# oxfordcontrol/Clarabel.jl

Measured on AMD Instinct MI355X. Metric: IPM iterations/sec + KKT factor+solve ms, 10k-var sparse QP, 1/2/4/8 GPU, higher is better.
Workload: dtype f64; 1 GPU; random sparse QP n=10000 m=20000 NN cone, uniform pattern (cfg 2a); N=30000, nnzK=99990, nnzL=16225495, supernodes=20125, levels=97, ordering=minimum degree, parallelism=1 independent problem(s), one per GPU

## Files before the change

### clarabel.jl_amd/csrc/device_plan.h

```cpp
#pragma once
#include <stdint.h>

#include "symbolic.h"

namespace hipkkt {

enum { SC_MAXDIAG = 0, SC_NORMB = 1, SC_NORME = 2, SC_COUNT = 8 };
enum { FL_NONFINITE = 0, FL_NREG = 1, FL_FRONTFAIL = 2, FL_FACFAIL = 3, FL_NPOLISH = 4, FL_COUNT = 8 };

struct __attribute__((aligned(16))) FrontSlot {
    double v;
    unsigned long long h;
};

struct RefineState {
    int32_t cur;
    int32_t steps;
    int32_t active;
    int32_t fail;
    double lastnorme, normb, norme;
};

struct GathPair {
    int64_t src;
    int32_t dj;
    int32_t r;
    int32_t K;
    int32_t dfirst;
};
struct DenseTriStrip {
    int c0, d, i0, pad;
    int64_t col0;
};
constexpr int kFbMax = 5;
struct FrontBatch {
    int64_t fp_off;
    int64_t scratch_off;
    int64_t stream_off;
    int32_t nb, nblk, r0;
    int32_t sync_off;
    int32_t i_base, i_end, tick, pad;
    int32_t x_begin, x_count;
};
constexpr int64_t kFbScratch = (int64_t)kFbMax * 4160 + (int64_t)(kFbMax * (kFbMax - 1) / 2) * 4096;
constexpr int kFbRec = 768;
constexpr int64_t kFbStream = (int64_t)kFbMax * 8 * kFbRec;
constexpr int kGathHeavy = 24;

constexpr int kSlvRows = 64;
constexpr int kSegSub = 8;
constexpr int kSegSubMin = 64;
constexpr int kSegRowTag = 0x40000000;
struct SegSyncLayout { int ftick, btick, fdone; int64_t err, words; };
constexpr SegSyncLayout seg_sync_layout(int nseg, int nsuper) {
    const int fdone = (2 * nseg + 31) & ~31;
    const int64_t err = fdone + (int64_t)kSegSub * nsuper;
    return {0, nseg, fdone, err, err + 16};
}
static_assert(seg_sync_layout(3, 5).btick == 3 && seg_sync_layout(3, 5).fdone == 32 && seg_sync_layout(3, 5).err == 32 + 8 * 5 &&
              seg_sync_layout(3, 5).words == 88, "seg_sync: tickets padded to 32 ints, then 8 * nsuper counters, then the error word");

struct DevPlan {
    const int *sn_first;
    const int64_t *sn_rowptr;
    const int *sn_rows;
    const int64_t *sn_panel;
    const int64_t *sn_diag;
    const int64_t *u_off;
    const int64_t *p_off;
    const int64_t *lt_off;
    const int *inv_list;
    const int *lvl_sn;
    const int *perm;
    const signed char *sgn_perm;
    const FacItem *fac_items;
    const FacRec *fac_recs;
    const FacItem *slv_items;
    const FacItem *bwd_items;
    const int *rel;
    const UpdTask *upd_tasks;
    const UpdGroup *upd_groups;
    const DenseGroup *dgroups;
    const int16_t *upd_tmap;
    const DenseTask *dtasks;
    const int64_t *gath_tgt;
    const int64_t *gath_pptr;
    const GathPair *gath_pairs;
    const int64_t *gath_heavy;
    const int64_t *g_ptr;
    const int *g_idx;
    const int64_t *kmap;
    const signed char *kdiag_sign;
    const int64_t *sym_rowptr;
    const int *sym_col;
    const int64_t *sym_q;
    const int *long_rows;
    int n_long_rows;
    const DenseTriStrip *dtri_strips;
    const int64_t *dtri_col;
    int n_dtri_strips;
    double *dense_acc;
    const FrontPanel *front_panels;
    const int64_t *front_gptr;
    const int *front_gidx;
    int *front_sync;
    const FacItem *pbwd_items;
    const int *dep_total;
    const int *sn_nitems;
    const int *sn_bparent;
    int *seg_sync;
    unsigned spin_limit;
    int *sn_polish;
    double polish_tau;
    int dbg;
    int nseg;
    double *kval;
    double *Lx;
    double *Ldiag;
    double *Linv;
    double *LinvT;
    double *LT;
    double *SbInv;
    double *D;
    double *Dinv;
    double *ubuf;
    FrontSlot *xseg, *pseg;
    int *seg_epoch;
    const int *rows_seg;
    double *pbuf;
    double *scal;
    int *flags;
};

}
```

### clarabel.jl_amd/csrc/hipkkt_internal.h

```cpp
#pragma once
#include "../../include/hipkkt.h"

#include <hip/hip_runtime.h>

#include <algorithm>
#include <atomic>
#include <chrono>
#include <cmath>
#include <cstdlib>
#include <cstring>
#include <deque>
#include <functional>
#include <future>
#include <memory>
#include <mutex>
#include <new>
#include <string>
#include <thread>
#include <vector>

#include "assemble.h"
#include "cone_layout.h"
#include "device_plan.h"
#include "hipkkt_cones.h"
#include "hipkkt_parts.h"
#include "kernels.h"
#include "runtime_pool.h"
#include "solve_schedule.h"
#include "symbolic.h"

namespace hipkkt { int box_probe(int device, double *out); }
namespace hipkkt_host {
using namespace hipkkt;

extern thread_local std::string g_create_error;

struct DeviceError {
    std::string msg;
};

#define HK_CHECK(expr)                                                                            \
    do {                                                                                          \
        hipError_t e_ = (expr);                                                                   \
        if (e_ != hipSuccess)                                                                     \
            throw DeviceError{std::string(#expr) + ": " + hipGetErrorString(e_)};                 \
    } while (0)

inline void copy_sync(hipStream_t st, void *dst, const void *src, size_t bytes, hipMemcpyKind kind) {
    if (!bytes) return;
    HK_CHECK(hipMemcpyAsync(dst, src, bytes, kind, st));
    HK_CHECK(hipStreamSynchronize(st));
}
inline void fill_async(hipStream_t st, void *dst, int value, size_t bytes) {
    if (bytes) HK_CHECK(hipMemsetAsync(dst, value, bytes, st));
}

struct DebugOpts {
    bool plan_cache = true;
    bool fb_extra = true;
    bool fb_stream = true;
    bool fb_v2 = true;
    bool force_twin = false;
    bool no_graph = false;
    bool no_persist = false;
    bool full_tiles = true;
    bool front_block = true;
    bool split_k = true;
    bool gather_overlap = true;
    bool gather_sort = true;
    int gather_side_blocks = 512;
    bool dense_tri = true;
    bool ordering_amd = false;
    bool no_front = false;
    bool host_assembly = false;
    int front_block_min_rows = -1;
    int superhop = -1;
    int debug_flags = 0;
    long long spin_limit = -1;
    long long persist_retry = -1;
    double accurate = 64.0;
    int fb_extra_pw = 1;
    double fb_pen1 = 10.0, fb_pen2 = 28.0;
    int psd_large_min = 65;
};
DebugOpts &debug_opts();
bool verbose();

struct GraphSlot {
    hipGraphExec_t exec = nullptr;
    bool valid = false;
    int static_enable = -1;
    double eps_const = 0, eps_prop = 0;
};

}

using namespace hipkkt;
using namespace hipkkt_host;

struct RefineOpts {
    int32_t enable; double reltol, abstol; int64_t max_iter; double stop_ratio;
    bool same_graph(const RefineOpts &o) const { return reltol == o.reltol && abstol == o.abstol && max_iter == o.max_iter && stop_ratio == o.stop_ratio; }
};

constexpr int kNumCtx = 2;
constexpr int kScalRedDoubles = 16;
struct SolveCtx {
    hipStream_t stream = nullptr;
    bool own_stream = false;
    DevPlan dp{};
    double *d_b = nullptr, *d_x0 = nullptr, *d_x1 = nullptr, *d_e = nullptr, *d_corr = nullptr;
    double *d_y = nullptr, *d_z = nullptr, *d_xp = nullptr;
    RefineState *d_rs = nullptr, *h_rs = nullptr;
    int *h_flags = nullptr;
    hipkkt_host::GraphSlot g_ldl, g_first, g_step;
    RefineOpts g_opts{-1, -1.0, -1.0, -1, -1.0};
    hipEvent_t ev_a = nullptr, ev_b = nullptr;
    double last_ms = 0;
    bool ir_used = false;
    bool extra_steps = false;
    const double *result() const { return (ir_used && h_rs->cur) ? d_x1 : d_x0; }
};

struct hipkkt_solver {
    int device = 0;
    SolveCtx ctx[kNumCtx];
    hipStream_t stream = nullptr;
    hipStream_t idle_stream = nullptr;
    hipkkt_opts opts{};
    bool l1 = false;
    KKTImage img;
    HostPlan plan;
    PlanOptions plan_opts;
    SolveSchedule sched;
    DevPlan dp{};
    std::vector<std::pair<void *, size_t>> allocs;
    std::string err;

    int N = 0;
    int64_t nnzK = 0;
    std::chrono::steady_clock::time_point t_created{};
    PersistState persist;
    FrontBatchState fb;
    UpdateSplit split;
    SocTables soc;
    ResidualBuffers res;
    ReducedSolve red;
    TwinState twin;
    SolverStats stats;
    ConeState cones;
    double accurate_threshold = 64.0;
    int last_npolish = 0;
    int inv_nsmall = 0, inv_wsmall = 1, inv_nwide = 0;
    int side_join_level = -1;
    hipEvent_t ev_fork = nullptr, ev_join = nullptr;

    int64_t *d_mapHs = nullptr, *d_mapP = nullptr, *d_mapA = nullptr, *d_diag_full = nullptr;
    std::vector<int64_t> cone_numel;
    std::vector<int32_t> cone_hs_dense, cone_sparse_kind;

    double *d_stage = nullptr;
    int64_t *d_stage_idx = nullptr;
    int64_t stage_cap = 0;
    double *h_scal = nullptr;
    double *h_scal_red = nullptr;
    int *h_flags = nullptr;

    hipkkt_host::GraphSlot g_factor;
    bool use_graph = true;
    bool runtime_ready = false;
    bool profiling = false;
    bool profiling_no_extra = false;
    hipEvent_t ev0 = nullptr, ev1 = nullptr, ev2 = nullptr, ev3 = nullptr;
    bool kval_event_pending = false;
    double last_eps = 0;
    int64_t last_nreg = 0;

    char *slab_cur = nullptr;
    size_t slab_left = 0;
    template <class T>
    T *dalloc(size_t n) {
        if (n == 0) n = 1;
        const size_t bytes = (n * sizeof(T) + 255) & ~(size_t)255;
        if (bytes > slab_left) {
            size_t slab = std::max<size_t>(bytes, (size_t)8 << 20);
            void *p = RuntimePool::get().dev_alloc(device, slab, &slab);
            if (!p) throw std::bad_alloc();
            allocs.push_back({p, slab});
            slab_cur = (char *)p;
            slab_left = slab;
        }
        void *p = slab_cur;
        slab_cur += bytes;
        slab_left -= bytes;
        return (T *)p;
    }
    template <class T>
    T *upload(const std::vector<T> &v) {
        T *p = dalloc<T>(v.size());
        if (!v.empty()) hipkkt_host::copy_sync(stream, p, v.data(), v.size() * sizeof(T), hipMemcpyHostToDevice);
        return p;
    }
    void ensure_stage(int64_t n) {
        if (n <= stage_cap) return;
        int64_t cap = std::max<int64_t>(n, 2 * stage_cap);
        d_stage = dalloc<double>(cap);
        d_stage_idx = dalloc<int64_t>(cap);
        stage_cap = cap;
    }
    template <class F>
    void for_each_graph_slot(F &&f) {
        f(g_factor); for (SolveCtx &C : ctx) { f(C.g_ldl); f(C.g_first); f(C.g_step); }
    }
    ~hipkkt_solver() {
        if (twin.cancel) twin.cancel->store(true);
        if (twin.go && twin.go->load() == 0) twin.go->store(2);
        if (twin.future.valid()) twin.future.wait();
        twin.pending.reset();
        delete twin.fallback;
        (void)hipSetDevice(device);
        RuntimePool &rp = RuntimePool::get();
        if (stream) (void)hipStreamSynchronize(stream);
        for (SolveCtx &C : ctx)
            if (C.own_stream && C.stream) (void)hipStreamSynchronize(C.stream);
        for_each_graph_slot([](hipkkt_host::GraphSlot &g) { if (g.exec) (void)hipGraphExecDestroy(g.exec); });
        for (SolveCtx &C : ctx) {
            rp.pinned_free(device, C.h_rs);
            rp.pinned_free(device, C.h_flags);
            for (hipEvent_t e : {C.ev_a, C.ev_b}) rp.event_put(device, e);
            if (C.own_stream) rp.stream_put(device, 2, C.stream);
        }
        for (auto &a : allocs) rp.dev_free(device, a.first, a.second);
        rp.pinned_free(device, h_scal);
        rp.pinned_free(device, h_flags);
        for (hipEvent_t e : {ev0, ev1, ev2, ev3, ev_fork, ev_join}) rp.event_put(device, e);
        rp.stream_put(device, 0, stream);
        rp.stream_put(device, 1, idle_stream);
    }
};

namespace hipkkt_host {

struct SyncWords { size_t seg, front; };
inline SyncWords sync_words(const hipkkt_solver *S) {
    return {(size_t)seg_sync_layout(S->sched.nseg, S->plan.nsuper).words, (size_t)std::max(S->plan.front_sync_ints, 16)};
}

void plan_cache_counts(int64_t *hits, int64_t *misses);
void init_runtime(hipkkt_solver *S);
void setup_device(hipkkt_solver *S);
int32_t finish_create(hipkkt_solver *S, const hipkkt_opts *opts, hipkkt_handle *out);
int32_t solve_many(hipkkt_solver *S, hipkkt_solver *T, int nrhs, const RefineOpts &ir, int64_t *ir_steps, double *const *out_dev, int nm,
                   const std::function<void(hipStream_t)> *after = nullptr);
hipkkt_solver *solve_target(hipkkt_solver *S);
struct ReducedIn {
    const double *rhs_x, *workz, *var_x, *in_dev;
    static ReducedIn host(const double *rhs_x, const double *workz, const double *var_x) { return {rhs_x, workz, var_x, nullptr}; }
    static ReducedIn device(const double *in_dev) { return {nullptr, nullptr, nullptr, in_dev}; }
};
struct ReducedScalars { const double *scal_in4; int32_t const_pending; };
struct ReducedOut {
    double *lhs_x = nullptr, *lhs_z = nullptr, *lhs_dev = nullptr, *scal_out = nullptr;
    int64_t *ir_steps = nullptr;
    const std::function<void(hipStream_t, const double *)> *after_reduce = nullptr;
};
int32_t kkt_solve_reduced_impl(hipkkt_solver *S, const ReducedIn &in, const ReducedScalars &sc, const ReducedOut &out, const RefineOpts &ir);

template <class F>
void run_graphed(hipkkt_solver *S, hipStream_t stream, GraphSlot &slot, bool reusable, F &&enqueue) {
    if (!S->use_graph) { enqueue(); return; }
    if (!(slot.valid && reusable)) {
        if (slot.exec) { (void)hipGraphExecDestroy(slot.exec); slot.exec = nullptr; slot.valid = false; }
        hipGraph_t graph = nullptr;
        HK_CHECK(hipStreamBeginCapture(stream, hipStreamCaptureModeRelaxed));
        try {
            enqueue();
        } catch (...) {
            (void)hipStreamEndCapture(stream, &graph);
            if (graph) (void)hipGraphDestroy(graph);
            throw;
        }
        HK_CHECK(hipStreamEndCapture(stream, &graph));
        hipError_t e = hipGraphInstantiate(&slot.exec, graph, nullptr, nullptr, 0);
        (void)hipGraphDestroy(graph);
        if (e != hipSuccess) { slot.exec = nullptr; S->use_graph = false; enqueue(); return; }
        slot.valid = true;
    }
    HK_CHECK(hipGraphLaunch(slot.exec, stream));
}

}

#define HK_ENTER(h)                                                      \
    if (!(h)) return HIPKKT_ERR_ARGUMENT;                                \
    hipkkt_solver *S = (h);                                              \
    try {                                                                \
        if (hipSetDevice(S->device) != hipSuccess) { S->err = "hipSetDevice failed"; return HIPKKT_ERR_DEVICE; }

#define HK_LEAVE                                                         \
    }                                                                    \
    catch (const DeviceError &e) { S->err = e.msg; return HIPKKT_ERR_DEVICE; } \
    catch (const std::bad_alloc &) { S->err = "out of memory"; return HIPKKT_ERR_ALLOC; } \
    catch (...) { S->err = "internal error"; return HIPKKT_ERR_INTERNAL; }
```

### clarabel.jl_amd/csrc/hipkkt_setup.cpp

```cpp
#include "hipkkt_internal.h"

using namespace hipkkt;
using namespace hipkkt_host;

namespace hipkkt_host {

namespace {
struct PlanCache {
    struct Entry {
        uint64_t key;
        std::string optkey;
        std::vector<int64_t> colptr, rowval;
        std::shared_ptr<const HostPlan> plan;
    };
    std::mutex mu;
    std::deque<Entry> entries;
    int64_t hits = 0, misses = 0;
    static constexpr size_t kMaxEntries = 8;
    static constexpr int64_t kMaxNnzL = 40000000;
    static PlanCache &get() { static PlanCache c; return c; }
    static bool enabled() { return debug_opts().plan_cache; }
    static uint64_t fnv(uint64_t h, const void *p, size_t n) {
        const unsigned char *b = (const unsigned char *)p;
        for (size_t i = 0; i < n; i++) { h ^= b[i]; h *= 1099511628211ull; }
        return h;
    }
    std::shared_ptr<const HostPlan> find(uint64_t key, const std::string &optkey, const KKTImage &K) {
        std::lock_guard<std::mutex> lk(mu);
        for (const Entry &e : entries)
            if (e.key == key && e.optkey == optkey && e.colptr == K.colptr && e.rowval == K.rowval) { hits++; return e.plan; }
        misses++;
        return nullptr;
    }
    void put(uint64_t key, const std::string &optkey, const KKTImage &K, const HostPlan &P) {
        if (P.nnzL > kMaxNnzL || P.ordering_used == 1) return;
        Entry e{key, optkey, K.colptr, K.rowval, std::make_shared<const HostPlan>(P)};
        std::lock_guard<std::mutex> lk(mu);
        entries.push_front(std::move(e));
        while (entries.size() > kMaxEntries) entries.pop_back();
    }
};
}
void plan_cache_counts(int64_t *hits, int64_t *misses) {
    PlanCache &c = PlanCache::get();
    std::lock_guard<std::mutex> lk(c.mu);
    *hits = c.hits; *misses = c.misses;
}

void init_runtime(hipkkt_solver *S) {
    HK_CHECK(hipSetDevice(S->device));
    RuntimePool &rp = RuntimePool::get();
    auto need = [&](void *p) { if (!p) throw DeviceError{"creating a stream / event / pinned buffer failed"}; return p; };
    S->stream = (hipStream_t)need(rp.stream_get(S->device, 0));
    S->idle_stream = (hipStream_t)need(rp.stream_get(S->device, 1));
    {
        const DebugOpts &o = debug_opts();
        S->fb.sw.extra = o.fb_extra;
        S->fb.sw.streamed = o.fb_stream;
        S->fb.sw.v2 = o.fb_v2 && S->fb.sw.streamed;
#ifndef HIPKKT_TESTING
        S->fb.sw.streamed = S->fb.sw.v2 = true;
#endif
        S->accurate_threshold = o.accurate;
        S->twin.force = o.force_twin;
    }
    static_assert(SC_COUNT * sizeof(double) <= RuntimePool::kPinned && sizeof(RefineState) <= RuntimePool::kPinned, "pinned chunk too small");
    for (hipEvent_t *e : {&S->ev0, &S->ev1, &S->ev2, &S->ev3, &S->ev_fork, &S->ev_join}) *e = (hipEvent_t)need(rp.event_get(S->device));
    S->h_scal = (double *)need(rp.pinned_alloc(S->device));
    S->h_flags = (int *)need(rp.pinned_alloc(S->device));
    S->h_scal_red = S->h_scal + 16;
    static_assert((16 + kScalRedDoubles) * sizeof(double) <= RuntimePool::kPinned, "pinned chunk too small for the reduced-solve scalars");
    memset(S->h_scal, 0, SC_COUNT * sizeof(double));
    memset(S->h_flags, 0, FL_COUNT * sizeof(int));
    if (debug_opts().no_graph) S->use_graph = false;
    for (int c = 0; c < kNumCtx; c++) {
        SolveCtx &C = S->ctx[c];
        if (c == 0) C.stream = S->stream;
        else { C.stream = (hipStream_t)need(rp.stream_get(S->device, 2)); C.own_stream = true; }
        C.ev_a = (hipEvent_t)need(rp.event_get(S->device));
        C.ev_b = (hipEvent_t)need(rp.event_get(S->device));
        C.h_rs = (RefineState *)need(rp.pinned_alloc(S->device));
        C.h_flags = (int *)need(rp.pinned_alloc(S->device));
        memset(C.h_rs, 0, sizeof(RefineState));
        memset(C.h_flags, 0, FL_COUNT * sizeof(int));
    }
}

template <class T>
static T *zeroed(hipkkt_solver *S, size_t n) {
    T *p = S->dalloc<T>(n);
    fill_async(S->stream, p, 0, std::max<size_t>(n, 1) * sizeof(T));
    return p;
}

static void order_far_stages(hipkkt_solver *S) {
    HostPlan &Pm = S->plan;
    const HostPlan &P = S->plan;
    const auto hb = front_batches(P, S->plan_opts.update_policy, kFbMax);
    const size_t nbh = hb.size();
    S->fb.next.assign(nbh, NextBatch());
    if (!S->fb.sw.extra || !debug_opts().front_block) return;
    std::vector<std::vector<int>> panel_batch(P.fronts.size());
    for (size_t fi = 0; fi < P.fronts.size(); fi++) panel_batch[fi].assign((size_t)P.fronts[fi].np, -1);
    for (size_t q = 0; q < nbh; q++)
        for (int t = 0; t < hb[q].nb; t++) panel_batch[(size_t)hb[q].front][(size_t)(hb[q].p0 + t)] = (int)q;
    for (size_t b = 0; b < nbh; b++) {
        const bool next = b + 1 < nbh && hb[b + 1].front == hb[b].front && hb[b + 1].p0 == hb[b].p0 + hb[b].nb;
        NextBatch &A = S->fb.next[b];
        const int l = hb[b].level_last, g0 = P.upd_stage_ptr[l], nd = P.upd_stage_ndense[l];
        const FrontDesc &F = P.fronts[(size_t)hb[b].front];
        auto near = [&](const UpdGroup &G) {
            if (!next || P.sn_front[G.tgt] != hb[b].front) return false;
            return panel_batch[(size_t)hb[b].front][(size_t)(G.tgt - F.s0)] == (int)b + 1;
        };
        auto gb = Pm.upd_groups.begin() + g0, ge = gb + nd;
        A.ncrit = (int)(std::stable_partition(gb, ge, near) - gb);
        A.has_next = next;
        A.next_blk = next ? (P.front_panels[P.fronts[(size_t)hb[b + 1].front].fp_off + hb[b + 1].p0].r + 63) / 64 : 0;
    }
}

constexpr int64_t kGatherSplitMin = 1000000;
constexpr int64_t kGatherSortMin = 50000;
static void split_gather_stages(hipkkt_solver *S) {
    HostPlan &P = S->plan;
    S->split.gath.assign(std::max(P.nlevels, 1), -1);
    const int B = P.update_batch_used;
    const bool may_split = S->plan_opts.update_policy == 2 && B >= 2 && debug_opts().gather_overlap;
    for (int l = 0; l < P.nlevels; l++) {
        const int64_t e0 = P.gath_stage_ptr[l], e1 = P.gath_stage_ptr[l + 1], ne = e1 - e0;
        if (ne < kGatherSortMin || !debug_opts().gather_sort) continue;
        std::vector<char> far((size_t)ne, 0);
        int64_t nfar = 0;
        if (may_split && ne >= kGatherSplitMin && l % B == B - 1 && l + B < P.nlevels) {
            for (int64_t e = e0; e < e1; e++) {
                const int t = (int)(std::upper_bound(P.sn_panel.begin(), P.sn_panel.begin() + P.nsuper, P.gath_tgt[e]) - P.sn_panel.begin()) - 1;
                far[(size_t)(e - e0)] = P.sn_level[t] > l + B;
                nfar += far[(size_t)(e - e0)];
            }
            if (nfar < kGatherSplitMin) { std::fill(far.begin(), far.end(), 0); nfar = 0; }
        }
        const size_t nkeys = (size_t)2 * (size_t)P.nsuper;
        std::vector<int64_t> cnt(nkeys + 1, 0);
        auto key = [&](int64_t e) { return (size_t)far[(size_t)(e - e0)] * (size_t)P.nsuper + (size_t)P.gath_sn[P.gath_pptr[e]]; };
        for (int64_t e = e0; e < e1; e++) cnt[key(e) + 1]++;
        for (size_t k = 0; k < nkeys; k++) cnt[k + 1] += cnt[k];
        std::vector<int64_t> ord((size_t)ne);
        for (int64_t e = e0; e < e1; e++) ord[(size_t)cnt[key(e)]++] = e;
        const int64_t p0 = P.gath_pptr[e0], p1 = P.gath_pptr[e1];
        std::vector<int64_t> tgt((size_t)ne), pptr((size_t)ne), src((size_t)(p1 - p0));
        std::vector<int32_t> dj((size_t)(p1 - p0)), sn((size_t)(p1 - p0));
        int64_t w = 0;
        for (int64_t q = 0; q < ne; q++) {
            const int64_t e = ord[(size_t)q];
            tgt[(size_t)q] = P.gath_tgt[e];
            for (int64_t pq = P.gath_pptr[e]; pq < P.gath_pptr[e + 1]; pq++, w++) { src[(size_t)w] = P.gath_src[pq]; dj[(size_t)w] = P.gath_dj[pq]; sn[(size_t)w] = P.gath_sn[pq]; }
            pptr[(size_t)q] = p0 + w;
        }
        std::copy(tgt.begin(), tgt.end(), P.gath_tgt.begin() + e0);
        std::copy(pptr.begin(), pptr.end(), P.gath_pptr.begin() + e0 + 1);
        std::copy(src.begin(), src.end(), P.gath_src.begin() + p0);
        std::copy(dj.begin(), dj.end(), P.gath_dj.begin() + p0);
        std::copy(sn.begin(), sn.end(), P.gath_sn.begin() + p0);
        if (nfar > 0) S->split.gath[l] = ne - nfar;
        if (verbose()) fprintf(stderr, "hipkkt: gather stage %d: %lld entries sorted by source, %lld of them deferred to the side stream (targets beyond level %d)\n", l, (long long)ne, (long long)nfar, l + B);
    }
}

static int64_t plan_split_k(hipkkt_solver *S, std::vector<DenseGroup> &dg) {
    const HostPlan &P = S->plan;
    S->split.group_begin.assign(std::max(P.nlevels, 1), 0);
    S->split.group_count.assign(std::max(P.nlevels, 1), 0);
    S->split.rec_ptr.assign(P.nlevels + 1, 0);
    std::vector<SplitRec> recs;
    int64_t scratch_max = 0;
    if (!debug_opts().split_k) { S->split.d_recs = S->upload(recs); return 0; }
    for (int l = 0; l < P.nlevels; l++) {
        S->split.rec_ptr[l + 1] = S->split.rec_ptr[l];
        const int g0 = P.upd_stage_ptr[l], nd = P.upd_stage_ndense[l];
        if (nd == 0 || S->fb.lvl[l] != -1) continue;
        int64_t ntasks = 0;
        for (int g = g0; g < g0 + nd; g++) ntasks += dg[g].task_end - dg[g].task_begin;
        const int chunk = std::max(4, (int)((ntasks + nd - 1) / nd));
        int max_nt = 0;
        for (int g = g0; g < g0 + nd; g++) max_nt = std::max(max_nt, dg[g].task_end - dg[g].task_begin);
        if (nd <= kDenseStripTiles || max_nt < 2 * chunk + 6) continue;
        int64_t scratch = 0;
        S->split.group_begin[l] = (int)dg.size();
        for (int g = g0; g < g0 + nd; g++) {
            const int nt = dg[g].task_end - dg[g].task_begin;
            const int parts = std::min(16, nt / chunk);
            if (nt < 2 * chunk || parts < 2) continue;
            recs.push_back({dg[g].tile_off, P.panel_doubles + scratch, dg[g].rt, dg[g].nrt, dg[g].wt, parts});
            for (int q = 0; q < parts; q++) {
                const int tb = dg[g].task_begin + (int)((int64_t)nt * q / parts), te = dg[g].task_begin + (int)((int64_t)nt * (q + 1) / parts);
                dg.push_back({P.panel_doubles + scratch, 64, dg[g].nrt, dg[g].wt, tb, te, dg[g].pad});
                scratch += 4096;
            }
            dg[g].wt = 0;
        }
        S->split.group_count[l] = (int)dg.size() - S->split.group_begin[l];
        S->split.rec_ptr[l + 1] = (int)recs.size();
        scratch_max = std::max(scratch_max, scratch);
    }
    S->split.d_recs = S->upload(recs);
    if (verbose() && !recs.empty())
        fprintf(stderr, "hipkkt: split-K: %zu target tiles cut into %zu chunks, %.1f MB of partial tiles\n", recs.size(), dg.size() - P.upd_groups.size(), scratch_max * 8e-6);
    return scratch_max;
}

static void build_front_batches(hipkkt_solver *S) {
    const HostPlan &P = S->plan;
    S->fb.lvl.assign(std::max(P.nlevels, 1), -1);
    if (!debug_opts().front_block) S->fb.sw.use = false;
    if (S->fb.sw.use)
        for (const FrontBatchHost &H : front_batches(P, S->plan_opts.update_policy, kFbMax)) {
            const FrontDesc &F = P.fronts[H.front];
            FrontBatch B;
            B.fp_off = F.fp_off + H.p0;
            B.nb = H.nb;
            B.r0 = P.front_panels[F.fp_off + H.p0].r;
            B.nblk = (B.r0 + 63) / 64;
            B.i_base = 0; B.i_end = B.nblk; B.tick = 0; B.pad = 0; B.x_begin = 0; B.x_count = 0;
            B.sync_off = 128 * (int)S->fb.batches.size();
            B.scratch_off = kFbScratch * (int64_t)S->fb.batches.size();
            B.stream_off = kFbStream * (int64_t)S->fb.batches.size();
            S->fb.lvl[H.level_first] = (int)S->fb.batches.size();
            for (int l = H.level_first + 1; l <= H.level_last; l++) S->fb.lvl[l] = -2;
            S->fb.batches.push_back(B);
            S->fb.last_level.push_back(H.level_last);
        }
    if (verbose()) fprintf(stderr, "hipkkt: %zu front batch(es) factored by one launch each (fronts %zu, update batch %d)\n", S->fb.batches.size(), P.fronts.size(), P.update_batch_used);
    const size_t nb_ = std::max<size_t>(S->fb.batches.size(), 1);
    S->fb.d_sync = zeroed<int>(S, 128 * nb_);
    S->fb.d_scratch = S->dalloc<double>((size_t)kFbScratch * nb_);
    S->fb.stream_doubles = (S->fb.sw.streamed || S->fb.sw.v2) ? (int64_t)kFbStream * (int64_t)nb_ : 0;
    S->fb.d_stream = S->dalloc<double>((size_t)std::max<int64_t>(S->fb.stream_doubles, 1));
    if (getenv("HIPKKT_FB_TRACE")) S->fb.d_trace = (long long *)zeroed<double>(S, nb_ * 128);
}

static void reset_device_state(hipkkt_solver *S) {
    S->for_each_graph_slot([](GraphSlot &g) { if (g.exec) (void)hipGraphExecDestroy(g.exec); g = GraphSlot(); });
    if (!S->allocs.empty() && S->stream) (void)hipStreamSynchronize(S->stream);
    for (auto &a : S->allocs) RuntimePool::get().dev_free(S->device, a.first, a.second);
    S->allocs.clear();
    S->slab_cur = nullptr; S->slab_left = 0;
    S->stage_cap = 0; S->d_stage = nullptr; S->d_stage_idx = nullptr;
    S->persist.rearm(!debug_opts().no_persist);
    S->fb.reset();
    S->split = UpdateSplit();
    S->soc = SocTables();
    S->res = ResidualBuffers();
    S->red = ReducedSolve();
    S->cones = ConeState();
}

static std::vector<int> inversion_list(hipkkt_solver *S) {
    const HostPlan &P = S->plan;
    std::vector<int> small, wide;
    S->inv_wsmall = 1;
    for (int s = 0; s < P.nsuper; s++) {
        const int w = P.sn_first[s + 1] - P.sn_first[s];
        if (w > 16 && w <= 64) wide.push_back(s);
        else { small.push_back(s); S->inv_wsmall = std::max(S->inv_wsmall, w); }
    }
    S->inv_nsmall = (int)small.size();
    S->inv_nwide = (int)wide.size();
    small.insert(small.end(), wide.begin(), wide.end());
    return small;
}

static std::vector<FacRec> fac_records(const HostPlan &P) {
    std::vector<FacRec> recs(P.fac_items.size());
    for (size_t q = 0; q < recs.size(); q++) {
        const int s = P.fac_items[q].sn;
        recs[q] = {P.sn_panel[s], P.sn_diag[s], P.lt_off[s], P.sn_first[s], P.sn_first[s + 1] - P.sn_first[s],
                   (int32_t)(P.sn_rowptr[s + 1] - P.sn_rowptr[s]), P.fac_items[q].blk};
    }
    return recs;
}

static std::vector<DenseGroup> dense_groups(const HostPlan &P) {
    std::vector<DenseGroup> dg(P.upd_groups.size());
    const bool no_full_tiles = !debug_opts().full_tiles;
    for (size_t q = 0; q < dg.size(); q++) {
        const UpdGroup &G = P.upd_groups[q];
        const int t = G.tgt;
        const int rt = (int)(P.sn_rowptr[t + 1] - P.sn_rowptr[t]);
        bool full = G.dense == 1 && rt - G.row_base >= kUpdRows && P.sn_first[t + 1] - P.sn_first[t] == 64 && !no_full_tiles;
        for (int u = G.task_begin; u < G.task_end && full; u++) {
            const UpdTask &T = P.upd_tasks[u];
            const int K = P.sn_first[T.src + 1] - P.sn_first[T.src];
            full = !(T.geom & (1 << 17)) && (T.geom & 0xFFFF) == 0 && T.nrows >= 64 && T.ncols >= 64 && K >= 8 && (K & 7) == 0;
        }
        dg[q] = {P.sn_panel[t] + G.row_base, rt, std::min(kUpdRows, rt - G.row_base), P.sn_first[t + 1] - P.sn_first[t],
                 G.task_begin, G.task_end, full ? 1 : 0};
    }
    return dg;
}

static std::vector<DenseTask> dense_tasks(const HostPlan &P) {
    std::vector<DenseTask> dt(P.upd_tasks.size());
    for (size_t q = 0; q < dt.size(); q++) {
        const UpdTask &T = P.upd_tasks[q];
        const int s = T.src;
        dt[q] = {P.sn_panel[s], (int32_t)((P.sn_rowptr[s + 1] - P.sn_rowptr[s]) * 8), P.sn_first[s + 1] - P.sn_first[s],
                 P.sn_first[s], T.row_lo, T.nrows, T.col_lo, T.ncols, T.geom, T.vt_begin, 0};
    }
    return dt;
}

static std::vector<GathPair> gather_pairs(const HostPlan &P) {
    std::vector<GathPair> gp(P.gath_src.size());
    for (size_t q = 0; q < gp.size(); q++) {
        const int s = P.gath_sn[q];
        gp[q] = {P.gath_src[q], P.gath_dj[q], (int32_t)(P.sn_rowptr[s + 1] - P.sn_rowptr[s]), P.sn_first[s + 1] - P.sn_first[s], P.sn_first[s]};
    }
    return gp;
}

static std::vector<int64_t> heavy_gathers(hipkkt_solver *S) {
    const HostPlan &P = S->plan;
    std::vector<int64_t> heavy;
    S->split.heavy_ptr.assign(P.nlevels + 1, 0);
    S->split.gath_heavy.assign(std::max(P.nlevels, 1), 0);
    for (int l = 0; l < P.nlevels; l++) {
        const int64_t e_split = S->split.gath[l] >= 0 ? P.gath_stage_ptr[l] + S->split.gath[l] : P.gath_stage_ptr[l + 1];
        for (int64_t e = P.gath_stage_ptr[l]; e < P.gath_stage_ptr[l + 1]; e++)
            if (P.gath_pptr[e + 1] - P.gath_pptr[e] > kGathHeavy) {
                heavy.push_back(e);
                if (e < e_split) S->split.gath_heavy[l]++;
            }
        S->split.heavy_ptr[l + 1] = (int64_t)heavy.size();
    }
    return heavy;
}

static void upload_plan(hipkkt_solver *S) {
    const HostPlan &P = S->plan;
    const SolveSchedule &H = S->sched;
    const int N = P.N;
    std::vector<signed char> sgn_perm(N), kdiag(S->nnzK, 0);
    for (int k = 0; k < N; k++) sgn_perm[k] = (signed char)(S->img.dsigns[P.perm[k]] >= 0 ? 1 : -1);
    for (int j = 0; j < N; j++)
        for (int64_t q = S->img.colptr[j]; q < S->img.colptr[j + 1]; q++)
            if (S->img.rowval[q] == j) kdiag[q] = (signed char)(S->img.dsigns[j] >= 0 ? 1 : -1);
    DevPlan &D = S->dp;
    D.sn_first = S->upload(P.sn_first);
    D.sn_rowptr = S->upload(P.sn_rowptr);
    D.sn_rows = S->upload(P.sn_rows);
    D.sn_panel = S->upload(P.sn_panel);
    D.sn_diag = S->upload(P.sn_diag);
    D.u_off = S->upload(P.u_off);
    D.p_off = S->upload(H.p_off);
    D.lt_off = S->upload(P.lt_off);
    D.bwd_items = S->upload(H.bwd_items);
    D.lvl_sn = S->upload(H.lvl_sn);
    D.perm = S->upload(P.perm);
    D.sgn_perm = S->upload(sgn_perm);
    D.inv_list = S->upload(inversion_list(S));
    D.fac_items = S->upload(P.fac_items);
    D.fac_recs = S->upload(fac_records(P));
    D.slv_items = S->upload(H.slv_items);
    D.rel = S->upload(P.rel);
    D.upd_tasks = S->upload(P.upd_tasks);
    D.upd_groups = S->upload(P.upd_groups);
    D.upd_tmap = P.upd_tmap.size() >= 128 ? S->upload(P.upd_tmap) : S->upload(std::vector<int16_t>(128, (int16_t)-1));
    D.dtasks = S->upload(dense_tasks(P));
    D.gath_tgt = S->upload(P.gath_tgt);
    D.gath_pptr = S->upload(P.gath_pptr);
    D.gath_pairs = S->upload(gather_pairs(P));
    D.gath_heavy = S->upload(heavy_gathers(S));
    D.g_ptr = S->upload(P.g_ptr);
    D.g_idx = S->upload(P.g_idx);
    D.kmap = S->upload(P.kmap);
    D.kdiag_sign = S->upload(kdiag);
    D.sym_rowptr = S->upload(P.sym_rowptr);
    D.sym_col = S->upload(P.sym_col);
    D.sym_q = S->upload(P.sym_q);
    std::vector<int> lr;
    const int thr = long_row_threshold();
    for (int i = 0; i < N; i++)
        if (P.sym_rowptr[i + 1] - P.sym_rowptr[i] > thr) lr.push_back(i);
    D.long_rows = S->upload(lr);
    D.n_long_rows = (int)lr.size();
    std::vector<DenseTriStrip> strips;
    for (const DenseTri &T : P.dtri)
        for (int i0 = 0; i0 < T.d; i0 += 64) strips.push_back(DenseTriStrip{T.c0, T.d, i0, 0, T.col0});
    D.dtri_strips = S->upload(strips);
    D.n_dtri_strips = (int)strips.size();
    D.dtri_col = S->upload(P.dtri_col);
    D.dense_acc = nullptr;
    D.front_panels = S->upload(P.front_panels);
    D.front_gptr = S->upload(P.front_gptr);
    D.front_gidx = S->upload(P.front_gidx);
    D.pbwd_items = S->upload(H.pbwd_items);
    D.dep_total = S->upload(H.dep_total);
    D.sn_nitems = S->upload(H.sn_nitems);
    D.sn_bparent = S->upload(H.sn_bparent);
    D.nseg = H.nseg;
    D.spin_limit = debug_opts().spin_limit >= 0 ? (unsigned)debug_opts().spin_limit : (1u << 20);
#ifdef HIPKKT_TESTING
    D.dbg = debug_opts().debug_flags;
    if (D.dbg) fprintf(stderr, "hipkkt: DEBUG_FLAGS = %d: timing experiment, the results of this handle are WRONG\n", D.dbg);
#else
    D.dbg = 0;
#endif
    D.sn_polish = zeroed<int>(S, (size_t)P.nsuper);
    D.polish_tau = S->accurate_threshold;
}

static void alloc_solve_scratch(hipkkt_solver *S, DevPlan &D) {
    const HostPlan &P = S->plan;
    const int64_t np0 = S->sched.p_off[P.nsuper];
    const size_t nx = (size_t)std::max(P.N, 1), np_ = (size_t)std::max<int64_t>(np0, 1);
    const SyncWords nw = sync_words(S);
    D.ubuf = S->dalloc<double>(P.ubuf_len);
    D.pbuf = S->dalloc<double>(np0);
    D.xseg = (FrontSlot *)zeroed<double>(S, 2 * nx);
    D.pseg = (FrontSlot *)zeroed<double>(S, 2 * np_);
    D.seg_epoch = zeroed<int>(S, 4);
    D.seg_sync = zeroed<int>(S, nw.seg);
    D.front_sync = zeroed<int>(S, nw.front);
    D.scal = zeroed<double>(S, SC_COUNT);
    D.flags = zeroed<int>(S, FL_COUNT);
}

static void alloc_factor_storage(hipkkt_solver *S) {
    const HostPlan &P = S->plan;
    DevPlan &D = S->dp;
    const int N = P.N;
    std::vector<DenseGroup> dg = dense_groups(P);
    build_front_batches(S);
    const int64_t split_scratch = S->split.scratch_doubles = plan_split_k(S, dg);
    D.dgroups = S->upload(dg);
    D.kval = S->upload(S->img.nzval);
    D.Lx = S->dalloc<double>(P.panel_doubles + split_scratch);
    if (split_scratch) fill_async(S->stream, D.Lx + P.panel_doubles, 0, (size_t)split_scratch * sizeof(double));
    D.Ldiag = zeroed<double>(S, (size_t)P.diag_doubles);
    D.Linv = S->dalloc<double>(P.diag_doubles);
    D.LinvT = S->dalloc<double>(P.diag_doubles);
    D.LT = S->dalloc<double>(P.lt_off[P.nsuper]);
    D.SbInv = zeroed<double>(S, (size_t)P.sbinv_doubles);
    D.D = S->dalloc<double>(N);
    D.Dinv = zeroed<double>(S, (size_t)N);
}

static void upload_value_maps(hipkkt_solver *S) {
    S->d_diag_full = S->upload(S->img.diag_full);
    if (!S->l1) return;
    SocTables &T = S->soc;
    S->d_mapHs = S->upload(S->img.mapHs);
    S->d_mapP = S->upload(S->img.mapP);
    S->d_mapA = S->upload(S->img.mapA);
    std::vector<int64_t> uidx, vidx, didx;
    std::vector<int> coneof;
    T.of_sparse.assign(S->img.smaps.size(), -1);
    for (size_t i = 0; i < S->img.smaps.size(); i++) {
        const SparseMap &sm = S->img.smaps[i];
        if (sm.kind != 1) continue;
        T.of_sparse[i] = T.n;
        T.off.push_back((int64_t)uidx.size());
        for (size_t q = 0; q < sm.vec[0].size(); q++) {
            uidx.push_back(sm.vec[0][q]);
            vidx.push_back(sm.vec[1][q]);
            coneof.push_back(T.n);
        }
        didx.push_back(sm.D[0]);
        didx.push_back(sm.D[1]);
        T.n++;
    }
    T.off.push_back((int64_t)uidx.size());
    T.total = (int64_t)uidx.size();
    T.d_uidx = S->upload(uidx);
    T.d_vidx = S->upload(vidx);
    T.d_didx = S->upload(didx);
    T.d_cone = S->upload(coneof);
    T.d_u = S->dalloc<double>(T.total);
    T.d_v = S->dalloc<double>(T.total);
    T.d_eta2 = S->dalloc<double>(T.n);
}

static void alloc_contexts(hipkkt_solver *S) {
    const int N = S->N;
    for (int c = 0; c < kNumCtx; c++) {
        SolveCtx &C = S->ctx[c];
        for (double **v : {&C.d_b, &C.d_x0, &C.d_x1, &C.d_e, &C.d_corr, &C.d_y, &C.d_z, &C.d_xp}) *v = zeroed<double>(S, (size_t)N);
        C.d_rs = (RefineState *)zeroed<double>(S, sizeof(RefineState) / sizeof(double) + 1);
        C.dp = S->dp;
        if (S->dp.n_dtri_strips > 0) C.dp.dense_acc = zeroed<double>(S, (size_t)N);
        if (c > 0) alloc_solve_scratch(S, C.dp);
        C.ir_used = false;
        C.h_rs->cur = 0;
    }
}

void setup_device(hipkkt_solver *S) {
    HK_CHECK(hipSetDevice(S->device));
    reset_device_state(S);
    order_far_stages(S);
    split_gather_stages(S);
    S->N = S->plan.N; S->nnzK = S->plan.nnzK;
    S->sched = build_solve_schedule(S->plan);
    upload_plan(S);
    alloc_factor_storage(S);
    S->dp.rows_seg = S->upload(S->sched.rows_seg);
    alloc_solve_scratch(S, S->dp);
    upload_value_maps(S);
    alloc_contexts(S);
    S->ensure_stage(std::max<int64_t>(1024, std::max<int64_t>(S->img.nHs, S->N)));
    HK_CHECK(hipStreamSynchronize(S->stream));
}

int32_t finish_create(hipkkt_solver *S, const hipkkt_opts *opts, hipkkt_handle *out) {
    PlanOptions po;
    po.max_width = opts->supernode_max_width > 0 ? opts->supernode_max_width : kMaxSnWidth;
    po.relax = opts->relax_supernodes != 0;
    po.update_policy = opts->update_policy;
    if (opts->update_batch > 0) po.update_batch = opts->update_batch;
    po.amd_dense_scale = opts->amd_dense_scale > 0 ? opts->amd_dense_scale : 1.5;
    po.front_min_panels = opts->front_min_panels == 0 ? 4 : std::max(0, opts->front_min_panels);
    po.n_hold = S->l1 ? (int)S->img.n : 0;
    po.dense_tri_first_col = (S->l1 && debug_opts().dense_tri) ? (int)S->img.n : -1;
    if (debug_opts().front_block_min_rows >= 0) po.front_block_min_width = debug_opts().front_block_min_rows;
    if (debug_opts().superhop >= 0) po.superhop = debug_opts().superhop;
    if (debug_opts().ordering_amd) po.n_hold = 0;
    if (debug_opts().no_front) po.front_min_panels = 0;
    std::vector<int64_t> up;
    const int64_t *uperm = nullptr;
    if (opts->user_perm) {
        up.resize(S->img.N);
        for (int64_t k = 0; k < S->img.N; k++) up[k] = opts->user_perm[k] - opts->index_base;
        uperm = up.data();
    }
    if (S->img.N >= ((int64_t)1 << 31)) { g_create_error = "N exceeds int32"; delete S; return HIPKKT_ERR_ARGUMENT; }
    {
        if (S->l1)
            po.on_alternative_order = [S, &po](const std::vector<int> &perm_md) {
                std::unique_ptr<hipkkt_solver> T(new hipkkt_solver());
                T->device = S->device;
                T->opts = S->opts;
                T->l1 = S->l1;
                T->img = S->img;
                PlanOptions po2 = po;
                po2.n_hold = 0;
                po2.on_alternative_order = nullptr;
                S->twin.cancel = std::make_shared<std::atomic<bool>>(false);
                po2.cancel = S->twin.cancel.get();
                T->plan_opts = po2;
                hipkkt_solver *Tp = T.get();
                std::vector<int64_t> pv(perm_md.begin(), perm_md.end());
                S->twin.pending = std::move(T);
                S->twin.go = std::make_shared<std::atomic<int>>(0);
                std::shared_ptr<std::atomic<int>> go = S->twin.go;
                S->twin.future = std::async(std::launch::async, [Tp, pv, po2, go]() {
                    std::string err = build_plan((int)Tp->img.N, Tp->img.colptr.data(), Tp->img.rowval.data(), pv.data(), po2, Tp->plan);
                    if (!err.empty()) return err;
                    if (Tp->plan.nnzL < 20000000) return err;
                    while (go->load(std::memory_order_acquire) == 0) std::this_thread::sleep_for(std::chrono::microseconds(200));
                    if (go->load(std::memory_order_acquire) != 1 || (po2.cancel && po2.cancel->load(std::memory_order_relaxed))) return std::string("cancelled");
                    try {
                        init_runtime(Tp);
                        setup_device(Tp);
                        Tp->twin.device_ready = true;
                    } catch (const DeviceError &e) {
                        return std::string("twin device set-up: ") + e.msg;
                    } catch (const std::bad_alloc &) {
                        return std::string("twin device set-up: out of memory");
                    }
                    return err;
                });
            };
    }
    const auto t_a = std::chrono::steady_clock::now();
    uint64_t ckey = 0;
    std::string optkey;
    std::shared_ptr<const HostPlan> cached;
    const bool plan_cache_on = PlanCache::enabled();
    if (plan_cache_on) {
        char buf[256];
        snprintf(buf, sizeof buf, "%d|%d|%d|%d|%.17g|%.17g|%d|%d|%d|%d|%d|%d|%d|%d|%d", po.max_width, (int)po.relax, po.update_policy, po.update_batch,
                 po.amd_dense_scale, po.dense_min_cover, po.n_hold, po.front_block_min_width, po.front_min_panels, po.superhop, po.nd_mode,
                 po.nd_leaf, uperm ? 1 : 0, po.dense_tri_first_col, po.dense_tri_min_dim);
        optkey = buf;
        ckey = PlanCache::fnv(1469598103934665603ull, S->img.colptr.data(), S->img.colptr.size() * sizeof(int64_t));
        ckey = PlanCache::fnv(ckey, S->img.rowval.data(), S->img.rowval.size() * sizeof(int64_t));
        if (uperm) ckey = PlanCache::fnv(ckey, uperm, (size_t)S->img.N * sizeof(int64_t));
        cached = PlanCache::get().find(ckey, optkey, S->img);
    }
    std::string err;
    if (cached) {
        S->plan = *cached;
        S->plan.timing_note = "plan cache hit";
    } else {
        err = build_plan((int)S->img.N, S->img.colptr.data(), S->img.rowval.data(), uperm, po, S->plan);
        if (err.empty() && plan_cache_on) PlanCache::get().put(ckey, optkey, S->img, S->plan);
    }
    po.on_alternative_order = nullptr;
    if (!err.empty()) { g_create_error = err; delete S; return HIPKKT_ERR_ARGUMENT; }
    if (S->plan.ordering_used != 1 && S->twin.cancel) S->twin.cancel->store(true);
    if (S->twin.go) S->twin.go->store((S->plan.ordering_used == 1 && err.empty()) ? 1 : 2, std::memory_order_release);
    S->plan_opts = po;
    const auto t_b = std::chrono::steady_clock::now();
    try {
        if (!S->runtime_ready) init_runtime(S);
        S->runtime_ready = true;
        setup_device(S);
        if (verbose())
            fprintf(stderr, "hipkkt: N %d nnzL %lld levels %d ordering %d: symbolic %.2f ms (%s), device set-up %.2f ms, runtime objects %.2f ms\n", S->plan.N, (long long)S->plan.nnzL,
                    S->plan.nlevels, S->plan.ordering_used, 1e3 * std::chrono::duration<double>(t_b - t_a).count(), S->plan.timing_note.c_str(),
                    1e3 * std::chrono::duration<double>(std::chrono::steady_clock::now() - t_b).count(), 1e3 * S->stats.t_init_runtime);
    } catch (const DeviceError &e) {
        g_create_error = e.msg; delete S; return HIPKKT_ERR_DEVICE;
    } catch (const std::bad_alloc &) {
        g_create_error = "out of (device) memory"; delete S; return HIPKKT_ERR_ALLOC;
    }
    *out = S;
    return HIPKKT_OK;
}

}
```

### clarabel.jl_amd/csrc/hipkkt_solve.cpp

```cpp
#include "hipkkt_internal.h"

using namespace hipkkt;
using namespace hipkkt_host;

namespace hipkkt_host {

static void enqueue_ldl_solve(hipkkt_solver *S, SolveCtx &C, const double *in, double *out, int *zero = nullptr, int nzero = 0) {
    const HostPlan &P = S->plan;
    const SolveSchedule &H = S->sched;
    hipStream_t st = C.stream;
    const DevPlan &D = C.dp;
    launch_permute_in(st, in, D.perm, C.d_y, S->N, D.seg_epoch, D.seg_sync, 2 * H.nseg, zero, nzero);
    const LevelLists &L = S->persist.use ? H.regular : H.all;
    auto fwd_level = [&](int l) {
        launch_fwd_narrow(st, D, L.reg_ptr[l], L.nnarrow[l], L.wnarrow[l], C.d_y, C.d_z);
        launch_fwd_level(st, D, L.slv_ptr[l], L.slv_ptr[l + 1] - L.slv_ptr[l], C.d_y, C.d_z);
    };
    auto bwd_level = [&](int l) {
        launch_bwd_partial(st, D, L.bwd_ptr[l], L.bwd_ptr[l + 1] - L.bwd_ptr[l], C.d_xp);
        launch_bwd_final(st, D, L.reg_ptr[l] + L.nnarrow[l], L.reg_ptr[l + 1] - L.reg_ptr[l] - L.nnarrow[l], C.d_z, C.d_xp, out);
        launch_bwd_narrow(st, D, L.reg_ptr[l], L.nnarrow[l], L.wnarrow[l], C.d_z, C.d_xp, out);
    };
    if (S->persist.use) {
        for (int g = 0; g < H.nseg; g++) {
            for (int l = H.seg_lo[g]; l < std::min(H.seg_lstar[g], H.seg_hi[g] + 1); l++) fwd_level(l);
            launch_fwd_seg(st, D, g, H.fseg_ptr[2 * g], H.fseg_ptr[2 * g + 1] - H.fseg_ptr[2 * g], P.nsuper, C.d_y, C.d_z);
            for (const FrontDesc &F : P.fronts)
                if (H.seg_of_level[F.level_last] == g) launch_front_fwd(st, D, F, C.d_y, C.d_z);
        }
        bool first = true;
        for (int g = H.nseg - 1; g >= 0; g--) {
            for (const FrontDesc &F : P.fronts)
                if (H.seg_of_level[F.level_last] == g) launch_front_bwd(st, D, F, C.d_z, C.d_xp, out);
            const int k = H.nseg - 1 - g;
            const int n = H.bseg_ptr[k + 1] - H.bseg_ptr[k];
            if (n > 0) { launch_bwd_seg(st, D, g, H.bseg_ptr[k], n, P.nsuper, first ? 1 : 0, C.d_z, C.d_xp, out); first = false; }
            for (int l = std::min(H.seg_lstar[g], H.seg_hi[g] + 1) - 1; l >= H.seg_lo[g]; l--) bwd_level(l);
        }
        return;
    }
    for (int l = 0; l < P.nlevels; l++) fwd_level(l);
    for (int l = P.nlevels - 1; l >= 0; l--) bwd_level(l);
}

static void invalidate_solve_graphs(SolveCtx &C) { C.g_ldl.valid = C.g_first.valid = C.g_step.valid = false; }

static void maybe_retry_persistent(hipkkt_solver *S) {
    PersistState &ps = S->persist;
    if (!ps.use && ps.allowed && ps.retry_at >= 0 && S->stats.n_ldlsolves >= ps.retry_at) {
        ps.use = true;
        ps.retry_at = -1;
        for (SolveCtx &C : S->ctx) invalidate_solve_graphs(C);
    }
}

static void enqueue_refine_step(hipkkt_solver *S, SolveCtx &C, const RefineOpts &ir) {
    hipStream_t st = C.stream;
    enqueue_ldl_solve(S, C, C.d_e, C.d_corr, (int *)(C.dp.scal + SC_NORME), 2);
    launch_refine_add(st, C.d_rs, C.d_x0, C.d_x1, C.d_corr, S->N);
    launch_spmv_residual(st, C.dp, C.d_b, C.d_rs, C.d_x0, C.d_x1, C.d_e, S->N, (unsigned long long *)C.dp.scal + SC_NORME);
    launch_refine_decide(st, C.d_rs, C.dp.scal, 1, ir.reltol, ir.abstol, (int)std::min<int64_t>(ir.max_iter, 1 << 30), ir.stop_ratio);
}

static inline bool sweep_failed(const SolveCtx &C) {
    if (C.h_flags[FL_FRONTFAIL] & ~7) {
        static bool told = false;
        if (!told)
            fprintf(stderr, "hipkkt: unexpected value in the flag words: %x %x %x %x\n", C.h_flags[0], C.h_flags[1], C.h_flags[2], C.h_flags[3]);
        told = true;
    }
    return (C.h_flags[FL_FRONTFAIL] & 7) != 0;
}

static bool recover_from_sweep_failure(hipkkt_solver *S) {
    PersistState &ps = S->persist;
    if (!ps.use) return false;
    for (SolveCtx &C : S->ctx) HK_CHECK(hipStreamSynchronize(C.stream));
    S->stats.n_sweep_timeouts++;
    const int64_t first = debug_opts().persist_retry >= 0 ? debug_opts().persist_retry : 64;
    ps.backoff = ps.backoff > 0 ? 2 * ps.backoff : first;
    ps.retry_at = first > 0 ? S->stats.n_ldlsolves + ps.backoff : -1;
    fprintf(stderr, "hipkkt: a persistent sweep kernel timed out (flags 0x%x 0x%x); per-level solve kernels for the next %lld LDL solves\n",
            S->ctx[0].h_flags[FL_FRONTFAIL], S->ctx[1].h_flags[FL_FRONTFAIL], (long long)(ps.retry_at >= 0 ? ps.backoff : -1));
    const SyncWords nw = sync_words(S);
    for (SolveCtx &C : S->ctx) {
        fill_async(S->stream, C.dp.seg_sync, 0, nw.seg * sizeof(int));
        fill_async(S->stream, C.dp.front_sync, 0, nw.front * sizeof(int));
        fill_async(S->stream, C.dp.flags + FL_FRONTFAIL, 0, sizeof(int));
        C.h_flags[FL_FRONTFAIL] = 0;
        invalidate_solve_graphs(C);
    }
    HK_CHECK(hipStreamSynchronize(S->stream));
    ps.use = false;
    return true;
}

template <class Body>
static bool with_sweep_retry(hipkkt_solver *T, Body &&body) {
    for (int attempt = 0; attempt < 2; attempt++) {
        maybe_retry_persistent(T);
        if (!body()) return false;
        if (!recover_from_sweep_failure(T)) return true;
    }
    return true;
}

static int32_t merge_rc(int32_t rc, int32_t r) { return (r < 0 || (r > 0 && rc == HIPKKT_OK)) ? (r < 0 ? r : (rc < 0 ? rc : r)) : rc; }

static void account_solve(hipkkt_solver *S, hipkkt_solver *T, double ms, int64_t nrhs) {
    for (hipkkt_solver *h : {T, S != T ? S : nullptr})
        if (h) { h->stats.t_last_solve = ms; h->stats.t_acc_solve += ms; h->stats.n_solvecalls++; h->stats.n_rhs_solved += nrhs; }
}

static void upload_rhs(SolveCtx &C, const double *rhsx, const double *rhsz, int64_t n, int64_t m, int64_t p) {
    if (n) HK_CHECK(hipMemcpyAsync(C.d_b, rhsx, n * sizeof(double), hipMemcpyHostToDevice, C.stream));
    if (m) HK_CHECK(hipMemcpyAsync(C.d_b + n, rhsz, m * sizeof(double), hipMemcpyHostToDevice, C.stream));
    if (p) HK_CHECK(hipMemsetAsync(C.d_b + n + m, 0, p * sizeof(double), C.stream));
}

static void solve_begin(hipkkt_solver *S, SolveCtx &C, const RefineOpts &ir) {
    hipStream_t st = C.stream;
    if (S->kval_event_pending && st != S->stream) HK_CHECK(hipStreamWaitEvent(st, S->ev3, 0));
    HK_CHECK(hipEventRecord(C.ev_a, st));
    C.ir_used = ir.enable != 0;
    if (ir.enable) {
        const bool same = C.g_opts.same_graph(ir);
        run_graphed(S, st, C.g_first, same, [&] {
            enqueue_ldl_solve(S, C, C.d_b, C.d_x0, (int *)(C.dp.scal + SC_NORMB), 4);
            launch_norm_inf(st, C.d_b, S->N, (unsigned long long *)C.dp.scal + SC_NORMB);
            launch_spmv_residual(st, C.dp, C.d_b, nullptr, C.d_x0, C.d_x0, C.d_e, S->N, (unsigned long long *)C.dp.scal + SC_NORME);
            launch_refine_decide(st, C.d_rs, C.dp.scal, 0, ir.reltol, ir.abstol, (int)std::min<int64_t>(ir.max_iter, 1 << 30), ir.stop_ratio);
            if (ir.max_iter > 0) enqueue_refine_step(S, C, ir);
        });
        if (!same) { C.g_step.valid = false; C.g_opts = ir; }
        S->stats.n_ldlsolves += ir.max_iter > 0 ? 2 : 1;
    } else {
        run_graphed(S, st, C.g_ldl, true, [&] {
            enqueue_ldl_solve(S, C, C.d_b, C.d_x0);
            launch_zero_words(st, C.dp.flags, 1);
            launch_check_finite(st, C.d_x0, S->N, C.dp.flags);
        });
        S->stats.n_ldlsolves += 1;
    }
}

static void solve_copy_out_dev(hipkkt_solver *S, SolveCtx &C, double *out_dev, int nm) {
    if (!out_dev) return;
    if (C.ir_used) launch_refine_copy_out(C.stream, C.d_rs, C.d_x0, C.d_x1, out_dev, nm);
    else HK_CHECK(hipMemcpyAsync(out_dev, C.d_x0, (size_t)nm * sizeof(double), hipMemcpyDeviceToDevice, C.stream));
}

static int32_t solve_finish(hipkkt_solver *S, SolveCtx &C, int64_t *ir_steps, double *out_dev, int nm) {
    hipStream_t st = C.stream;
    auto readback = [&] {
        if (C.ir_used) HK_CHECK(hipMemcpyAsync(C.h_rs, C.d_rs, sizeof(RefineState), hipMemcpyDeviceToHost, st));
        HK_CHECK(hipMemcpyAsync(C.h_flags, C.dp.flags, FL_COUNT * sizeof(int), hipMemcpyDeviceToHost, st));
        HK_CHECK(hipEventRecord(C.ev_b, st));
        HK_CHECK(hipStreamSynchronize(st));
    };
    readback();
    bool more = false;
    C.extra_steps = false;
    while (C.ir_used && C.h_rs->active && !sweep_failed(C)) {
        run_graphed(S, st, C.g_step, true, [&] { enqueue_refine_step(S, C, C.g_opts); });
        S->stats.n_ldlsolves += 1;
        more = true;
        readback();
    }
    C.extra_steps = more;
    if (more && out_dev) {
        solve_copy_out_dev(S, C, out_dev, nm);
        HK_CHECK(hipEventRecord(C.ev_b, st));
        HK_CHECK(hipStreamSynchronize(st));
    }
    float ms = 0;
    HK_CHECK(hipEventElapsedTime(&ms, C.ev_a, C.ev_b));
    C.last_ms = ms;
    if (ir_steps) *ir_steps = C.ir_used ? C.h_rs->steps : 0;
    if (sweep_failed(C)) { S->err = "persistent solve kernel timed out"; return HIPKKT_ERR_DEVICE; }
    const bool ok = C.ir_used ? C.h_rs->fail == 0 : C.h_flags[FL_NONFINITE] == 0;
    return ok ? HIPKKT_OK : HIPKKT_NUMERICAL_FAILURE;
}

hipkkt_solver *solve_target(hipkkt_solver *S) { return (S->twin.using_fallback && S->twin.fallback) ? S->twin.fallback : S; }

int32_t solve_many(hipkkt_solver *S, hipkkt_solver *T, int nrhs, const RefineOpts &ir, int64_t *ir_steps, double *const *out_dev, int nm,
                   const std::function<void(hipStream_t)> *after) {
    int32_t rc = HIPKKT_OK;
    double ms = 0;
    bool redo = false;
    auto run_after = [&] {
        for (int c = 1; c < nrhs; c++) {
            HK_CHECK(hipEventRecord(S->ev2, T->ctx[c].stream));
            HK_CHECK(hipStreamWaitEvent(T->ctx[0].stream, S->ev2, 0));
        }
        (*after)(T->ctx[0].stream);
    };
    const bool gave_up = with_sweep_retry(T, [&] {
        for (int c = 0; c < nrhs; c++) {
            solve_begin(T, T->ctx[c], ir);
            solve_copy_out_dev(T, T->ctx[c], out_dev ? out_dev[c] : nullptr, nm);
        }
        if (after) run_after();
        rc = HIPKKT_OK;
        ms = 0;
        redo = false;
        bool timed_out = false;
        for (int c = 0; c < nrhs; c++) {
            rc = merge_rc(rc, solve_finish(T, T->ctx[c], ir_steps ? ir_steps + c : nullptr, out_dev ? out_dev[c] : nullptr, nm));
            ms = std::max(ms, T->ctx[c].last_ms);
            timed_out = timed_out || sweep_failed(T->ctx[c]);
            redo = redo || T->ctx[c].extra_steps;
        }
        return timed_out;
    });
    if (after && !gave_up && rc == HIPKKT_OK) {
        if (redo) run_after();
        HK_CHECK(hipStreamSynchronize(T->ctx[0].stream));
    }
    account_solve(S, T, ms, nrhs);
    return rc;
}

int32_t kkt_solve_reduced_impl(hipkkt_solver *S, const ReducedIn &in, const ReducedScalars &sc, const ReducedOut &out, const RefineOpts &ir) {
    const int64_t n = S->img.n, m = S->img.m, p = S->img.p;
    const int nm = (int)(n + m);
    const int32_t const_pending = sc.const_pending;
    if (!S->red.d) {
        S->red.d = S->dalloc<double>(3 * (size_t)S->N + n + 16);
        S->red.d_part = S->dalloc<double>(8 * (size_t)residual_blocks((int)n, (int)m) + 8);
        S->red.have_const = false;
    }
    double *d_s1 = S->red.d, *d_s2 = d_s1 + S->N, *d_lhs = d_s2 + S->N, *d_xv = d_lhs + S->N, *d_sc = d_xv + n;
    if (!const_pending && !S->red.have_const) { S->err = "kkt_solve_reduced: no constant-rhs solution resident (pass const_pending = 1 after a refactorisation)"; return HIPKKT_ERR_ARGUMENT; }
    hipkkt_solver *T = solve_target(S);
    const double tau = sc.scal_in4[0], kappa = sc.scal_in4[1], rhs_tau = sc.scal_in4[2], rhs_kappa = sc.scal_in4[3];
    SolveCtx &A = T->ctx[0], &Bc = T->ctx[1];
    auto reduce = [&]() {
        launch_reduced(A.stream, S->dp, d_s1, d_s2, d_xv, S->res.d_qb, S->res.d_qb + n, tau, kappa, rhs_tau, rhs_kappa, S->red.d_part, d_sc,
                       d_lhs, (int)n, (int)m);
        if (out.lhs_dev) HK_CHECK(hipMemcpyAsync(out.lhs_dev, d_lhs, (size_t)nm * sizeof(double), hipMemcpyDeviceToDevice, A.stream));
        if (out.lhs_x && n) HK_CHECK(hipMemcpyAsync(out.lhs_x, d_lhs, n * sizeof(double), hipMemcpyDeviceToHost, A.stream));
        if (out.lhs_z && m) HK_CHECK(hipMemcpyAsync(out.lhs_z, d_lhs + n, m * sizeof(double), hipMemcpyDeviceToHost, A.stream));
        HK_CHECK(hipMemcpyAsync(S->h_scal_red, d_sc, 10 * sizeof(double), hipMemcpyDeviceToHost, A.stream));
        if (out.after_reduce) (*out.after_reduce)(A.stream, d_lhs);
    };
    auto join_const = [&]() { HK_CHECK(hipEventRecord(S->ev2, Bc.stream)); HK_CHECK(hipStreamWaitEvent(A.stream, S->ev2, 0)); };
    int64_t st1 = 0, st2 = 0;
    int32_t rc = HIPKKT_OK;
    bool redo = false;
    double ms = 0;
    const bool gave_up = with_sweep_retry(T, [&] {
        if (in.in_dev) {
            launch_set_rhs(A.stream, A.d_b, in.in_dev, nm, T->N);
            HK_CHECK(hipMemcpyAsync(d_xv, in.in_dev + nm, (size_t)n * sizeof(double), hipMemcpyDeviceToDevice, A.stream));
        } else {
            upload_rhs(A, in.rhs_x, in.workz, n, m, p);
            if (n) HK_CHECK(hipMemcpyAsync(d_xv, in.var_x, n * sizeof(double), hipMemcpyHostToDevice, A.stream));
        }
        solve_begin(T, A, ir);
        solve_copy_out_dev(T, A, d_s1, nm);
        if (const_pending) {
            launch_const_rhs(Bc.stream, Bc.d_b, S->res.d_qb, (int)n, nm, T->N);
            solve_begin(T, Bc, ir);
            solve_copy_out_dev(T, Bc, d_s2, nm);
            join_const();
        }
        reduce();
        st1 = st2 = 0;
        rc = solve_finish(T, A, &st1, d_s1, nm);
        redo = A.extra_steps;
        ms = A.last_ms;
        if (const_pending) {
            rc = merge_rc(rc, solve_finish(T, Bc, &st2, d_s2, nm));
            redo = redo || Bc.extra_steps;
            ms = std::max(ms, Bc.last_ms);
        }
        return sweep_failed(A) || (const_pending && sweep_failed(Bc));
    });
    if (gave_up) return HIPKKT_ERR_DEVICE;
    if (redo && rc == HIPKKT_OK) {
        if (const_pending) join_const();
        reduce();
    }
    HK_CHECK(hipStreamSynchronize(A.stream));
    account_solve(S, T, ms, const_pending ? 2 : 1);
    if (rc == HIPKKT_OK && const_pending) S->red.have_const = true;
    if (out.ir_steps) { out.ir_steps[0] = st1; out.ir_steps[1] = st2; }
    if (out.scal_out) memcpy(out.scal_out, S->h_scal_red, 10 * sizeof(double));
    return rc;
}

}

extern "C" {


int32_t hipkkt_setrhs(hipkkt_handle h, const double *rhsx, const double *rhsz) {
    HK_ENTER(h)
    const int64_t n = S->img.n, m = S->img.m;
    if (!S->l1 || (n && !rhsx) || (m && !rhsz)) return HIPKKT_ERR_ARGUMENT;
    upload_rhs(S->ctx[0], rhsx, rhsz, n, m, S->img.p);
    HK_CHECK(hipStreamSynchronize(S->stream));
    return HIPKKT_OK;
    HK_LEAVE
}

int32_t hipkkt_setrhs_dev(hipkkt_handle h, const double *rhs_dev) {
    HK_ENTER(h)
    if (!S->l1 || !rhs_dev) return HIPKKT_ERR_ARGUMENT;
    launch_set_rhs(S->stream, S->ctx[0].d_b, rhs_dev, (int)(S->img.n + S->img.m), S->N);
    return HIPKKT_OK;
    HK_LEAVE
}

static hipkkt_solver *target_with_rhs(hipkkt_solver *S) {
    hipkkt_solver *T = solve_target(S);
    if (T != S) copy_sync(S->stream, T->ctx[0].d_b, S->ctx[0].d_b, (size_t)S->N * sizeof(double), hipMemcpyDeviceToDevice);
    return T;
}

int32_t hipkkt_solve(hipkkt_handle h, double *lhsx, double *lhsz, int32_t ir_enable, double reltol, double abstol,
                     int64_t max_iter, double stop_ratio, int64_t *ir_steps) {
    HK_ENTER(h)
    if (!S->l1) return HIPKKT_ERR_ARGUMENT;
    hipkkt_solver *T = target_with_rhs(S);
    int32_t rc = solve_many(S, T, 1, RefineOpts{ir_enable, reltol, abstol, max_iter, stop_ratio}, ir_steps, nullptr, 0);
    if (rc == HIPKKT_OK) {
        const int64_t n = S->img.n, m = S->img.m;
        const double *x = T->ctx[0].result();
        if (lhsx && n) copy_sync(S->stream, lhsx, x, n * sizeof(double), hipMemcpyDeviceToHost);
        if (lhsz && m) copy_sync(S->stream, lhsz, x + n, m * sizeof(double), hipMemcpyDeviceToHost);
    }
    return rc;
    HK_LEAVE
}

int32_t hipkkt_solve_dev(hipkkt_handle h, double *lhs_dev, int32_t ir_enable, double reltol, double abstol,
                         int64_t max_iter, double stop_ratio, int64_t *ir_steps) {
    HK_ENTER(h)
    if (!S->l1) return HIPKKT_ERR_ARGUMENT;
    hipkkt_solver *T = target_with_rhs(S);
    double *outs[1] = {lhs_dev};
    return solve_many(S, T, 1, RefineOpts{ir_enable, reltol, abstol, max_iter, stop_ratio}, ir_steps, outs, (int)(S->img.n + S->img.m));
    HK_LEAVE
}

static int32_t solve_multi_impl(hipkkt_solver *S, int64_t nrhs, const double *rhsx, const double *rhsz, const double *rhs_dev,
                                double *lhsx, double *lhsz, double *lhs_dev, const RefineOpts &ir, int64_t *ir_steps) {
    const int64_t n = S->img.n, m = S->img.m, p = S->img.p;
    hipkkt_solver *T = solve_target(S);
    int32_t rc_all = HIPKKT_OK;
    for (int64_t r0 = 0; r0 < nrhs; r0 += kNumCtx) {
        const int k = (int)std::min<int64_t>(kNumCtx, nrhs - r0);
        double *outs[kNumCtx] = {nullptr, nullptr};
        for (int c = 0; c < k; c++) {
            SolveCtx &C = T->ctx[c];
            const int64_t r = r0 + c;
            if (rhs_dev) launch_set_rhs(C.stream, C.d_b, rhs_dev + r * (n + m), (int)(n + m), T->N);
            else upload_rhs(C, rhsx + r * n, rhsz + r * m, n, m, p);
            if (lhs_dev) outs[c] = lhs_dev + r * (n + m);
        }
        const int32_t rc = solve_many(S, T, k, ir, ir_steps ? ir_steps + r0 : nullptr, lhs_dev ? outs : nullptr, (int)(n + m));
        if (rc < 0) return rc;
        if (rc > 0) rc_all = rc;
        if (rc == HIPKKT_OK && (lhsx || lhsz))
            for (int c = 0; c < k; c++) {
                const double *x = T->ctx[c].result();
                const int64_t r = r0 + c;
                if (lhsx && n) copy_sync(S->stream, lhsx + r * n, x, n * sizeof(double), hipMemcpyDeviceToHost);
                if (lhsz && m) copy_sync(S->stream, lhsz + r * m, x + n, m * sizeof(double), hipMemcpyDeviceToHost);
            }
    }
    return rc_all;
}

int32_t hipkkt_solve_multi(hipkkt_handle h, int64_t nrhs, const double *rhsx, const double *rhsz, double *lhsx, double *lhsz,
                           int32_t ir_enable, double reltol, double abstol, int64_t max_iter, double stop_ratio, int64_t *ir_steps) {
    HK_ENTER(h)
    if (!S->l1 || nrhs < 0 || (nrhs && ((S->img.n && !rhsx) || (S->img.m && !rhsz)))) return HIPKKT_ERR_ARGUMENT;
    return solve_multi_impl(S, nrhs, rhsx, rhsz, nullptr, lhsx, lhsz, nullptr, RefineOpts{ir_enable, reltol, abstol, max_iter, stop_ratio}, ir_steps);
    HK_LEAVE
}

int32_t hipkkt_solve_multi_dev(hipkkt_handle h, int64_t nrhs, const double *rhs_dev, double *lhs_dev, int32_t ir_enable, double reltol,
                               double abstol, int64_t max_iter, double stop_ratio, int64_t *ir_steps) {
    HK_ENTER(h)
    if (!S->l1 || nrhs < 0 || (nrhs && !rhs_dev)) return HIPKKT_ERR_ARGUMENT;
    return solve_multi_impl(S, nrhs, nullptr, nullptr, rhs_dev, nullptr, nullptr, lhs_dev, RefineOpts{ir_enable, reltol, abstol, max_iter, stop_ratio}, ir_steps);
    HK_LEAVE
}

int32_t hipkkt_kkt_solve_reduced(hipkkt_handle h, const double *rhs_x, const double *workz, const double *var_x, const double *scal_in4,
                                 int32_t const_pending, double *lhs_x, double *lhs_z, double *scal_out10, int32_t ir_enable,
                                 double reltol, double abstol, int64_t max_iter, double stop_ratio, int64_t *ir_steps2) {
    HK_ENTER(h)
    const int64_t n = S->img.n, m = S->img.m;
    if (!S->l1 || !S->res.d_qb || !scal_in4 || !scal_out10 || (n && (!rhs_x || !var_x)) || (m && !workz)) {
        S->err = "kkt_solve_reduced: call hipkkt_set_qb first / bad arguments";
        return HIPKKT_ERR_ARGUMENT;
    }
    ReducedOut out;
    out.lhs_x = lhs_x; out.lhs_z = lhs_z; out.scal_out = scal_out10; out.ir_steps = ir_steps2;
    return kkt_solve_reduced_impl(S, ReducedIn::host(rhs_x, workz, var_x), {scal_in4, const_pending}, out, RefineOpts{ir_enable, reltol, abstol, max_iter, stop_ratio});
    HK_LEAVE
}

int32_t hipkkt_kkt_solve_reduced_dev(hipkkt_handle h, const double *in_dev, const double *scal_in4, int32_t const_pending,
                                     double *lhs_dev, double *scal_out10, int32_t ir_enable, double reltol, double abstol,
                                     int64_t max_iter, double stop_ratio, int64_t *ir_steps2) {
    HK_ENTER(h)
    if (!S->l1 || !S->res.d_qb || !scal_in4 || !scal_out10 || !in_dev) {
        S->err = "kkt_solve_reduced_dev: call hipkkt_set_qb first / bad arguments";
        return HIPKKT_ERR_ARGUMENT;
    }
    ReducedOut out;
    out.lhs_dev = lhs_dev; out.scal_out = scal_out10; out.ir_steps = ir_steps2;
    return kkt_solve_reduced_impl(S, ReducedIn::device(in_dev), {scal_in4, const_pending}, out, RefineOpts{ir_enable, reltol, abstol, max_iter, stop_ratio});
    HK_LEAVE
}

int32_t hipkkt_ldl_solve(hipkkt_handle h, double *x, const double *b) {
    if (h && h->twin.using_fallback && h->twin.fallback) return hipkkt_ldl_solve(h->twin.fallback, x, b);
    HK_ENTER(h)
    if (!x || !b) return HIPKKT_ERR_ARGUMENT;
    SolveCtx &C = S->ctx[0];
    HK_CHECK(hipMemcpyAsync(C.d_b, b, (size_t)S->N * sizeof(double), hipMemcpyHostToDevice, C.stream));
    int32_t rc = solve_many(S, S, 1, RefineOpts{0, 0.0, 0.0, 0, 0.0}, nullptr, nullptr, 0);
    if (rc < 0) return rc;
    copy_sync(S->stream, x, C.d_x0, (size_t)S->N * sizeof(double), hipMemcpyDeviceToHost);
    return HIPKKT_OK;
    HK_LEAVE
}

}
```

### clarabel.jl_amd/csrc/kernel_util.h

```cpp
#pragma once
#include <hip/hip_runtime.h>
#include <stdint.h>

namespace hipkkt {

static inline unsigned nblk(int64_t n, int bs = 256) { return (unsigned)((n + bs - 1) / bs); }

typedef double v4f64 __attribute__((ext_vector_type(4)));

__device__ __forceinline__ double readlane_f64(double x, int l) {
    const unsigned long long u = (unsigned long long)__double_as_longlong(x);
    const unsigned lo = __builtin_amdgcn_readlane((unsigned)u, l), hi = __builtin_amdgcn_readlane((unsigned)(u >> 32), l);
    return __longlong_as_double((long long)(((unsigned long long)hi << 32) | lo));
}
__device__ __forceinline__ int rfl(int v) { return __builtin_amdgcn_readfirstlane(v); }

template <class T>
__device__ __forceinline__ T *rfl_ptr(T *p) {
    const unsigned long long u = (unsigned long long)p;
    const unsigned lo = __builtin_amdgcn_readfirstlane((unsigned)u), hi = __builtin_amdgcn_readfirstlane((unsigned)(u >> 32));
    return (T *)(((unsigned long long)hi << 32) | lo);
}
#define HK_GLOBAL __attribute__((address_space(1)))
__device__ __forceinline__ double ld_off(const double *base, unsigned byte_off) {
    return *(const HK_GLOBAL double *)((const HK_GLOBAL char *)base + byte_off);
}
__device__ __forceinline__ void st_off(double *base, unsigned byte_off, double v) {
    *(HK_GLOBAL double *)((HK_GLOBAL char *)base + byte_off) = v;
}

__device__ __forceinline__ int ld_relaxed_i(const int *p) { return __hip_atomic_load(p, __ATOMIC_RELAXED, __HIP_MEMORY_SCOPE_AGENT); }
__device__ __forceinline__ double ld_relaxed(const double *p) { return __hip_atomic_load(p, __ATOMIC_RELAXED, __HIP_MEMORY_SCOPE_AGENT); }
__device__ __forceinline__ void st_relaxed(double *p, double v) { __hip_atomic_store(p, v, __ATOMIC_RELAXED, __HIP_MEMORY_SCOPE_AGENT); }

__device__ __forceinline__ double pivot_rcp(double d) {
    double r = __builtin_amdgcn_rcp(d);
    r = fma(fma(-d, r, 1.0), r, r);
    r = fma(fma(-d, r, 1.0), r, r);
    return r;
}

__device__ __forceinline__ double pivot_rcp3(double d) {
    const double r = __builtin_amdgcn_rcp(d);
    const double e = fma(-d, r, 1.0);
    const double e2 = fma(e, e, e);
    return fma(r, e2, r);
}

__device__ __forceinline__ void lds_barrier() { asm volatile("s_waitcnt lgkmcnt(0)\n\ts_barrier" ::: "memory"); }

__device__ __forceinline__ void mfma_settle() {
    __builtin_amdgcn_sched_barrier(0);
    asm volatile("s_nop 7\n\ts_nop 7\n\ts_nop 7" ::: "memory");
    __builtin_amdgcn_sched_barrier(0);
}

__device__ __forceinline__ void atomic_max_abs(unsigned long long *slot, double v) {
    unsigned long long bits = (unsigned long long)__double_as_longlong(fabs(v));
    atomicMax(slot, bits);
}

__device__ __forceinline__ double wave_max(double v) {
    for (int off = 32; off > 0; off >>= 1) {
        double o = __shfl_xor(v, off, 64);
        v = (o > v || o != o) ? o : v;
    }
    return v;
}

__device__ __forceinline__ void block_atomic_max_abs(unsigned long long *slot, double a) {
    __shared__ double wm_[16];
    a = wave_max(a);
    const int lane = threadIdx.x & 63, wave = threadIdx.x >> 6, nw = (blockDim.x + 63) >> 6;
    if (lane == 0) wm_[wave] = a;
    __syncthreads();
    if (threadIdx.x == 0) {
        double m = wm_[0];
        for (int i = 1; i < nw; i++) m = (wm_[i] > m || wm_[i] != wm_[i]) ? wm_[i] : m;
        atomic_max_abs(slot, m);
    }
}

}
```

### clarabel.jl_amd/csrc/kernels.h

```cpp
#pragma once
#include <hip/hip_runtime.h>

#include "device_plan.h"

namespace hipkkt {
void launch_scatter_values(hipStream_t st, double *kval, const int64_t *idx, const double *vals, int64_t n, double scale);
void launch_scale_values(hipStream_t st, double *kval, const int64_t *idx, int64_t n, double scale);
void launch_soc_batch(hipStream_t st, double *kval, const int64_t *uidx, const int64_t *vidx, const int *cone_of,
                      const double *u, const double *v, const double *eta2, int64_t n, const int64_t *didx, int nsoc);
void launch_psd_hs(hipStream_t st, double *kval, const int64_t *map_hs, int64_t hs_off, const double *W, int n, const int *skip = nullptr);
void launch_zero_words(hipStream_t st, void *p, int nwords);
void launch_maxabs_gather(hipStream_t st, const double *v, const int64_t *idx, int64_t n, unsigned long long *slot);
void launch_init_panels(hipStream_t st, const DevPlan &P, int64_t nnz, int static_enable, double eps_const, double eps_prop);
void launch_factor_level(hipStream_t st, const DevPlan &P, int item_begin, int nitems, int wmax, double dyn_eps, double dyn_delta);
void launch_factor_panel(hipStream_t st, const DevPlan &P, int item_begin, int nitems, double dyn_eps, double dyn_delta);
void launch_update_stage(hipStream_t st, const DevPlan &P, int group_begin, int ngroups);
constexpr int kDenseStripTiles = 384;
constexpr double kFullKFlopsPerTile = 1.5e6;
inline bool dense_full_k(int nd, double flops) { return nd > 0 && flops >= kFullKFlopsPerTile * nd; }
void launch_update_dense(hipStream_t st, const DevPlan &P, int group_begin, int ngroups, bool full_k = false);
void launch_split_reduce(hipStream_t st, const DevPlan &P, const SplitRec *recs, int n);
void launch_update_gather(hipStream_t st, const DevPlan &P, int64_t ebegin, int64_t n, int64_t hbegin, int64_t nheavy, int max_blocks = 0);
void launch_invert_diag(hipStream_t st, const DevPlan &P, int n_small, int wmax_small, int n_wide);
void launch_permute_in(hipStream_t st, const double *b, const int *perm, double *y, int n, int *epoch, int *ticks, int nticks, int *zero = nullptr,
                       int nzero = 0);
void launch_fwd_level(hipStream_t st, const DevPlan &P, int item_begin, int nitems, double *y, double *z);
void launch_bwd_partial(hipStream_t st, const DevPlan &P, int item_begin, int nitems, const double *x);
void launch_bwd_final(hipStream_t st, const DevPlan &P, int sn_begin, int nsn, const double *z, double *x, double *xout);
void launch_fwd_narrow(hipStream_t st, const DevPlan &P, int sn_begin, int n, int wmax, double *y, double *z);
void launch_bwd_narrow(hipStream_t st, const DevPlan &P, int sn_begin, int n, int wmax, const double *z, double *x, double *xout);
void launch_fwd_seg(hipStream_t st, const DevPlan &P, int seg, int item_begin, int nitems, int nsuper, double *y, double *z);
void launch_bwd_seg(hipStream_t st, const DevPlan &P, int seg, int item_begin, int nitems, int nsuper, int first, const double *z,
                    double *x, double *xout);
void launch_front_fwd(hipStream_t st, const DevPlan &P, const FrontDesc &F, double *y, double *z);
void launch_front_bwd(hipStream_t st, const DevPlan &P, const FrontDesc &F, const double *z, double *x, double *xout);
void launch_invert_super(hipStream_t st, const DevPlan &P, const FrontDesc &F);
void launch_spmv_residual(hipStream_t st, const DevPlan &P, const double *b, const RefineState *rs, const double *x0, const double *x1,
                          double *e, int n, unsigned long long *slot);
int long_row_threshold();
void launch_norm_inf(hipStream_t st, const double *v, int n, unsigned long long *slot);
void launch_refine_decide(hipStream_t st, RefineState *rs, const double *scal, int phase, double reltol, double abstol, int max_iter,
                          double stop_ratio);
void launch_refine_add(hipStream_t st, const RefineState *rs, double *x0, double *x1, const double *corr, int n);
void launch_refine_copy_out(hipStream_t st, const RefineState *rs, const double *x0, const double *x1, double *out, int nm);
void launch_set_rhs(hipStream_t st, double *b, const double *rhs, int nm, int n);
void launch_check_finite(hipStream_t st, const double *v, int n, int *flags);
void launch_block_products(hipStream_t st, const DevPlan &P, const double *x, const double *z, double *Px, double *ATz,
                           double *Ax, int n, int m);
int residual_blocks(int n, int m);
void launch_residuals(hipStream_t st, const DevPlan &P, const double *x, const double *z, const double *s, const double *q,
                      const double *b, double tau, double kappa, double *out, double *part, double *scal, int n, int m);
void launch_reduced(hipStream_t st, const DevPlan &P, const double *s1, const double *s2, const double *xv, const double *q,
                    const double *b, double tau, double kappa, double rhs_tau, double rhs_kappa, double *part, double *scal_out,
                    double *lhs, int n, int m);
void launch_const_rhs(hipStream_t st, double *dst, const double *qb, int n, int nm, int N);
void launch_mfma_probe(hipStream_t st, const double *A, const double *B, double *out);
void launch_front_block(hipStream_t st, const DevPlan &P, const FrontBatch &B, int *sync_all, double *scratch_all, double *stream_all,
                        double dyn_eps, double dyn_delta, bool streamed, long long *trace = nullptr);
void launch_front_block2(hipStream_t st, const DevPlan &P, const FrontBatch &B, int *sync_all, double *scratch_all, double *stream_all,
                         double dyn_eps, double dyn_delta, long long *trace = nullptr);
void launch_fb_reset(hipStream_t st, int *sync_all, int nsync, double *stream_all, int64_t nstream);
void launch_scaling_diag(hipStream_t st, const signed char *row_kind, const int64_t *row_hs, const int64_t *map_hs, const double *s,
                         const double *z, double *w, double *lam, double *kval, int64_t m);
void launch_scaling_soc(hipStream_t st, int nsoc, const int64_t *desc, const int64_t *map_hs, const double *s, const double *z,
                        double *w, double *lam, double *eta_out, double *soc_u, double *soc_v, double *soc_eta2, double *kval,
                        int *fail);
void launch_psd_rrt(hipStream_t st, const double *R, double *W, int n);
void launch_scaling_cone3(hipStream_t st, int nexp, int npow, const int64_t *row0, const int64_t *hs0, const int64_t *out0,
                          const double *alpha, const int64_t *map_hs, const double *s, const double *z, double mu, int strategy,
                          double *kval, double *out, int *trips, int *fail);
void launch_scaling_genpow(hipStream_t st, int ngenpow, const int64_t *desc, const double *alpha, const int64_t *idx,
                           const int64_t *map_hs, const double *z, double mu, double sqrtmu, double *kval, double *out, int *fail);
int64_t step_len_pairs(int64_t m, int nsoc);
int64_t step_norm_part_doubles();
void launch_step_affine_ds(hipStream_t st, const signed char *row_kind, int nsoc, const int64_t *desc, const double *lam, double *out,
                           int64_t m);
void launch_step_shift(hipStream_t st, const signed char *row_kind, int nsoc, const int64_t *desc, const double *w, const double *eta,
                       const double *dz, const double *ds, double sigma_mu, double *out, int64_t m);
void launch_step_offset(hipStream_t st, const signed char *row_kind, int nsoc, const int64_t *desc, const double *z, const double *w,
                        const double *lam, const double *eta, const double *ds, double *out, int64_t m);
void launch_step_mulhs(hipStream_t st, const signed char *row_kind, int nsoc, const int64_t *desc, const double *w, const double *eta,
                       const double *x, const double *addc, double *y, int64_t m);
void launch_step_length(hipStream_t st, const signed char *row_kind, int nsoc, const int64_t *desc, const double *z, const double *s,
                        const double *dz, const double *ds, double alpha_max, double *part, double *out2, int64_t m);
void launch_step_add_step(hipStream_t st, double *v, const double *dv, double alpha, int64_t len);
void launch_step_scale(hipStream_t st, double *out, const double *in, double f, int64_t len);
void launch_step_add(hipStream_t st, double *acc, const double *b, int64_t len);
void launch_step_rhs(hipStream_t st, double *in, const double *xzs, const double *res, const double *dsc, double f, int64_t n, int64_t m);
void launch_step_info_norms(hipStream_t st, const double *xzs, const double *res, const double *eq, double *part, double *out8, int64_t n,
                            int64_t m);
int step3_max_candidates();
int64_t step3_barrier_doubles(int64_t ncones);
void launch_step3_copy(hipStream_t st, int n3, const int64_t *row0, const double *src, double *out);
void launch_step3_mulhs(hipStream_t st, int n3, const int64_t *row0, const int64_t *out0, const double *nsout, const double *x,
                        const double *addc, double *y);
void launch_step3_shift(hipStream_t st, int nexp, int npow, const int64_t *row0, const int64_t *out0, const double *alpha,
                        const double *nsout, const double *z, const double *dz, const double *ds, double sigma_mu, double *out);
void launch_step3_length(hipStream_t st, int nexp, int npow, const int64_t *row0, const double *alpha, const double *z, const double *s,
                         const double *dz, const double *ds, const double *sym2, const double *dtau, double tau, double kappa,
                         double rhs_kappa, double alpha_max, double step, double alpha_min, int trips, double *part, double *out2,
                         int ngp = 0);
void launch_step3_barrier(hipStream_t st, const signed char *row_kind, int nsoc, const int64_t *desc, int nexp, int npow,
                          const int64_t *row0, const double *alpha, const double *z, const double *s, const double *dz, const double *ds,
                          const double *alphas, int nalpha, double *work, double *out, int64_t m, int ngp = 0);
int step3_length_parts(int nexp, int npow);
double *step3_barrier_gppart(double *work, int nsoc, int n3);
void launch_genpow_copy(hipStream_t st, int ngp, const int64_t *desc, const double *src, double *out);
void launch_genpow_shift(hipStream_t st, int ngp, const int64_t *desc, const double *nsout, double sigma_mu, double *out);
void launch_genpow_mulhs(hipStream_t st, int ngp, const int64_t *desc, const double *nsout, double mu, const double *x, const double *addc,
                         double *y);
void launch_genpow_length(hipStream_t st, int ngp, const int64_t *desc, const double *alpha, const double *z, const double *s,
                          const double *dz, const double *ds, const double *sym2, const double *dtau, double tau, double kappa,
                          double rhs_kappa, double alpha_max, double step, double alpha_min, int trips, double *part);
void launch_genpow_barrier(hipStream_t st, int ngp, const int64_t *desc, const double *alpha, const double *z, const double *s,
                           const double *dz, const double *ds, const double *alphas, int nalpha, double *cpart);
constexpr int kPsdLargeMaxN = 128;
constexpr int kPsdLargeMats = 4;
constexpr int kPsdLargeMatDoubles = kPsdLargeMaxN * kPsdLargeMaxN;
struct PsdLargeBatch { int nlarge = 0; const int *lidx = nullptr; int lmin = 65, max_n = 0; double *ws = nullptr; };
struct PsdView {
    int npsd = 0;
    const int64_t *tab = nullptr;
    const double *R = nullptr, *Rinv = nullptr, *lam = nullptr;
    PsdLargeBatch large;
};
int psd_step_max_dim();
void launch_psd_step_affine_ds(hipStream_t st, const PsdView &P, double *out);
void launch_psd_step_mulhs(hipStream_t st, const PsdView &P, const double *x, const double *addc, double *y);
void launch_psd_step_shift(hipStream_t st, const PsdView &P, const double *dz, const double *ds, double sigma_mu, double *out);
void launch_psd_step_offset(hipStream_t st, const PsdView &P, const double *ds, double *out);
void launch_psd_step_length_cones(hipStream_t st, const PsdView &P, const double *dz, const double *ds, double alpha_max, double *part);
void launch_psd_step_length_final(hipStream_t st, int npsd, const double *sym2, const double *part, double *out2);
void launch_psd_step_check(hipStream_t st, const double *lam, int64_t len, int *fail);
int psd_step_large_max_dim();
int64_t psd_large_ws_doubles(int nlarge);
void launch_psd_large_affine_ds(hipStream_t st, const PsdView &P, double *out);
void launch_psd_large_mulhs(hipStream_t st, const PsdView &P, const double *x, const double *addc, double *y);
void launch_psd_large_shift(hipStream_t st, const PsdView &P, const double *dz, const double *ds, double sigma_mu, double *out);
void launch_psd_large_offset(hipStream_t st, const PsdView &P, const double *ds, double *out);
void launch_psd_large_length(hipStream_t st, const PsdView &P, const double *dz, const double *ds, double alpha_max, double *part);
void launch_psd_nt_scaling(hipStream_t st, int npsd, const int64_t *tab, const double *s, const double *z, double *R, double *Rinv,
                           double *lam, int *bad, int *fail, int max_side);
void launch_psd_large_nt_scaling(hipStream_t st, const PsdView &P, const double *s, const double *z, double *R, double *Rinv,
                                 double *lam, int *bad, int *fail);
double *psd_barrier_slots(double *work, int nsoc, int n3, int ngp);
void launch_psd_barrier(hipStream_t st, const PsdView &P, const double *z, const double *s, const double *dz, const double *ds,
                        const double *alphas, int nalpha, double *slots);
void launch_psd_barrier_add(hipStream_t st, int npsd, const double *slots, int nalpha, double *out);
int64_t start_work_doubles(int64_t ncones);
double *start_decision(double *work, int64_t ncones);
void launch_start_identity(hipStream_t st, const signed char *row_kind, const int64_t *row_hs, const int64_t *map_hs, int nsoc,
                           const int64_t *desc, double *soc_u, double *soc_v, double *soc_eta2, const PsdView &P,
                           const int64_t *psd_hs0, int64_t psd_max_numel, double *kval, int64_t m);
void launch_start_margins(hipStream_t st, const signed char *row_kind, int nsoc, const int64_t *desc, const PsdView &P, const double *v0,
                          const double *v1, int nsides, double degree, double *work, int64_t ncones, int64_t m, bool psd_large);
void launch_start_shift(hipStream_t st, const signed char *row_kind, int nsoc, const int64_t *desc, const PsdView &P, const double *dec,
                        double *v0, int pd0, double *v1, int pd1, int nsides, int64_t m, bool psd_large);
void launch_start_rhs(hipStream_t st, double *dst, const double *qb, int n, int nm, int N, int mode);
void launch_start_assemble(hipStream_t st, double *xzs, const double *sa, const double *sb, int64_t n, int64_t m);
}
```

### clarabel.jl_amd/csrc/refine.hip

```cpp
#include <hip/hip_runtime.h>
#include <stdint.h>

#include "device_plan.h"
#include "kernel_util.h"
#include "kernels.h"

namespace hipkkt {

constexpr int kLongRow = 192;
__device__ __forceinline__ void spmv_short_rows(const int64_t *__restrict__ rowptr, const int *__restrict__ col,
                                                const int64_t *__restrict__ qidx, const double *__restrict__ kval,
                                                const double *__restrict__ b, const double *__restrict__ xi, double *__restrict__ e,
                                                int n, unsigned long long *__restrict__ norm_slot, const double *__restrict__ dacc) {
    const int gid = blockIdx.x * blockDim.x + threadIdx.x;
    const int row = gid >> 2, sub = gid & 3;
    double acc = 0.0;
    bool mine = false;
    if (row < n) {
        const int64_t p0 = rowptr[row], p1 = rowptr[row + 1];
        mine = p1 - p0 <= kLongRow;
        if (mine)
            for (int64_t p = p0 + sub; p < p1; p += 4) acc += kval[qidx[p]] * xi[col[p]];
    }
    acc += __shfl_xor(acc, 1, 64);
    acc += __shfl_xor(acc, 2, 64);
    double a = 0.0;
    if (mine && sub == 0) {
        if (dacc) acc += dacc[row];
        const double ev = b[row] - acc;
        e[row] = ev;
        a = fabs(ev);
    }
    block_atomic_max_abs(norm_slot, a);
}
__device__ __forceinline__ void spmv_long_row(int row, const int64_t *__restrict__ rowptr, const int *__restrict__ col,
                                              const int64_t *__restrict__ qidx, const double *__restrict__ kval,
                                              const double *__restrict__ b, const double *__restrict__ xi, double *__restrict__ e,
                                              unsigned long long *__restrict__ norm_slot, const double *__restrict__ dacc) {
    __shared__ double red[4];
    const int64_t p0 = rowptr[row], p1 = rowptr[row + 1];
    double acc = 0.0;
    for (int64_t p = p0 + threadIdx.x; p < p1; p += 256) acc += kval[qidx[p]] * xi[col[p]];
    for (int off = 32; off > 0; off >>= 1) acc += __shfl_down(acc, off, 64);
    if ((threadIdx.x & 63) == 0) red[threadIdx.x >> 6] = acc;
    __syncthreads();
    if (threadIdx.x == 0) {
        const double ev = b[row] - ((((red[0] + red[1]) + red[2]) + red[3]) + (dacc ? dacc[row] : 0.0));
        e[row] = ev;
        atomic_max_abs(norm_slot, ev);
    }
}
__device__ __forceinline__ const double *spmv_operand(const RefineState *st, const double *x0, const double *x1) {
    return st ? (st->cur ? x0 : x1) : x0;
}
__global__ void __launch_bounds__(256)
k_spmv_residual(const int64_t *__restrict__ rowptr, const int *__restrict__ col, const int64_t *__restrict__ qidx,
                const double *__restrict__ kval, const double *__restrict__ b, const RefineState *st,
                const double *__restrict__ x0, const double *__restrict__ x1, double *__restrict__ e, int n,
                unsigned long long *__restrict__ norm_slot, const double *__restrict__ dacc) {
    if (st && !st->active) return;
    spmv_short_rows(rowptr, col, qidx, kval, b, spmv_operand(st, x0, x1), e, n, norm_slot, dacc);
}
__global__ void __launch_bounds__(256)
k_spmv_long(const int *__restrict__ long_rows, const int64_t *__restrict__ rowptr, const int *__restrict__ col,
            const int64_t *__restrict__ qidx, const double *__restrict__ kval, const double *__restrict__ b,
            const RefineState *st, const double *__restrict__ x0, const double *__restrict__ x1, double *__restrict__ e,
            unsigned long long *__restrict__ norm_slot, const double *__restrict__ dacc) {
    if (st && !st->active) return;
    spmv_long_row(long_rows[blockIdx.x], rowptr, col, qidx, kval, b, spmv_operand(st, x0, x1), e, norm_slot, dacc);
}

__global__ void __launch_bounds__(512)
k_spmv_dense_tri(const DenseTriStrip *__restrict__ strips, const int64_t *__restrict__ col_off, const double *__restrict__ kval,
                 const RefineState *st, const double *__restrict__ x0, const double *__restrict__ x1, double *__restrict__ acc_out) {
    if (st && !st->active) return;
    const double *__restrict__ x = spmv_operand(st, x0, x1);
    __shared__ double part[8][64];
    __shared__ double csum[64];
    const DenseTriStrip T = strips[blockIdx.x];
    const int lane = threadIdx.x & 63, w = threadIdx.x >> 6;
    const int i = T.i0 + lane;
    const int64_t *__restrict__ co = col_off + T.col0;
    const double *__restrict__ xb = x + T.c0;
    double a = 0.0;
#pragma unroll 4
    for (int j = T.i0 + w; j < T.d; j += 8) {
        const double v = kval[co[j] + (i <= j ? i : j)];
        a = fma(i <= j ? v : 0.0, xb[j], a);
    }
    part[w][lane] = a;
    for (int c = 0; c < 8; c++) {
        const int ci = T.i0 + 8 * w + c;
        double s = 0.0;
        if (ci < T.d) {
            const double *__restrict__ colv = kval + co[ci];
#pragma unroll 4
            for (int r = lane; r < ci; r += 64) s = fma(colv[r], xb[r], s);
        }
        for (int off = 32; off > 0; off >>= 1) s += __shfl_xor(s, off, 64);
        if (lane == 0) csum[8 * w + c] = s;
    }
    __syncthreads();
    if (w == 0 && i < T.d) {
        double t = csum[lane];
#pragma unroll
        for (int q = 0; q < 8; q++) t += part[q][lane];
        acc_out[T.c0 + i] = t;
    }
}

template <int ND, int NQ>
__device__ __forceinline__ void block_dots(double (&d)[NQ], double *__restrict__ part) {
    __shared__ double red[4][NQ];
#pragma unroll
    for (int c = 0; c < ND; c++)
        for (int off = 32; off > 0; off >>= 1) d[c] += __shfl_down(d[c], off, 64);
    const int lane = threadIdx.x & 63, wave = threadIdx.x >> 6;
    if (lane == 0)
#pragma unroll
        for (int c = 0; c < NQ; c++) red[wave][c] = d[c];
    __syncthreads();
    if (threadIdx.x < NQ)
        part[(int64_t)blockIdx.x * NQ + threadIdx.x] = ((red[0][threadIdx.x] + red[1][threadIdx.x]) + red[2][threadIdx.x]) + red[3][threadIdx.x];
}
template <int NQ>
__device__ __forceinline__ void column_sums(const double *__restrict__ part, int nblocks, double (&tot)[NQ]) {
    constexpr int NS = 256 / NQ;
    __shared__ double buf[NQ][NS];
    const int which = threadIdx.x % NQ, slot = threadIdx.x / NQ;
    double a = 0.0;
    for (int bq = slot; bq < nblocks; bq += NS) a += part[(int64_t)bq * NQ + which];
    buf[which][slot] = a;
    __syncthreads();
    if (threadIdx.x < NQ) {
        double t = 0.0;
        for (int i = 0; i < NS; i++) t += buf[threadIdx.x][i];
        buf[threadIdx.x][0] = t;
    }
    __syncthreads();
#pragma unroll
    for (int c = 0; c < NQ; c++) tot[c] = threadIdx.x == 0 ? buf[c][0] : 0.0;
}

struct RowProducts { double ax, az; };
__device__ __forceinline__ RowProducts row_products(const int64_t *__restrict__ rowptr, const int *__restrict__ col,
                                                    const int64_t *__restrict__ qidx, const double *__restrict__ kval,
                                                    const double *__restrict__ x, const double *__restrict__ z, int row, int sub,
                                                    int n, int m) {
    double ax = 0.0, az = 0.0;
    if (row < n + m) {
        const int64_t p0 = rowptr[row], p1 = rowptr[row + 1];
        for (int64_t p = p0 + sub; p < p1; p += 4) {
            const int c = col[p];
            const double v = kval[qidx[p]];
            if (c < n) ax += v * x[c];
            else if (row < n && c < n + m) az += v * z[c - n];
        }
    }
    ax += __shfl_xor(ax, 1, 64);
    ax += __shfl_xor(ax, 2, 64);
    az += __shfl_xor(az, 1, 64);
    az += __shfl_xor(az, 2, 64);
    return {ax, az};
}
__global__ void __launch_bounds__(256)
k_block_products(const int64_t *__restrict__ rowptr, const int *__restrict__ col, const int64_t *__restrict__ qidx,
                 const double *__restrict__ kval, const double *__restrict__ x, const double *__restrict__ z,
                 double *__restrict__ Px, double *__restrict__ ATz, double *__restrict__ Ax, int n, int m) {
    const int gid = blockIdx.x * blockDim.x + threadIdx.x;
    const int row = gid >> 2, sub = gid & 3;
    const auto [ax, az] = row_products(rowptr, col, qidx, kval, x, z, row, sub, n, m);
    if (sub == 0 && row < n + m) {
        if (row < n) { Px[row] = ax; ATz[row] = az; }
        else Ax[row - n] = ax;
    }
}

__global__ void __launch_bounds__(256)
k_residuals(const int64_t *__restrict__ rowptr, const int *__restrict__ col, const int64_t *__restrict__ qidx,
            const double *__restrict__ kval, const double *__restrict__ x, const double *__restrict__ z,
            const double *__restrict__ sv, const double *__restrict__ q, const double *__restrict__ b, double tau,
            double *__restrict__ out, double *__restrict__ part, int n, int m) {
    const int gid = blockIdx.x * blockDim.x + threadIdx.x;
    const int row = gid >> 2, sub = gid & 3;
    const auto [ax, az] = row_products(rowptr, col, qidx, kval, x, z, row, sub, n, m);
    double d[4] = {0.0, 0.0, 0.0, 0.0};
    if (sub == 0 && row < n + m) {
        double *rx = out, *rz = out + n, *rxi = rz + m, *rzi = rxi + n, *Px = rzi + m;
        if (row < n) {
            const double xi = x[row], rinf = -az;
            Px[row] = ax;
            rxi[row] = rinf;
            rx[row] = (rinf - ax) - q[row] * tau;
            d[0] = q[row] * xi;
            d[3] = xi * ax;
        } else {
            const int j = row - n;
            const double rinf = sv[j] + ax;
            rzi[j] = rinf;
            rz[j] = rinf - b[j] * tau;
            d[1] = b[j] * z[j];
            d[2] = sv[j] * z[j];
        }
    }
    block_dots<4, 4>(d, part);
}
__global__ void __launch_bounds__(256)
k_residuals_finish(const double *__restrict__ part, int nblocks, double tau, double kappa, double *__restrict__ scal) {
    double t[4];
    column_sums<4>(part, nblocks, t);
    if (threadIdx.x == 0) {
        const double qx = t[0], bz = t[1], sz = t[2], xPx = t[3];
        scal[0] = qx; scal[1] = bz; scal[2] = sz; scal[3] = xPx;
        scal[4] = qx + bz + kappa + xPx / tau;
    }
}

__global__ void __launch_bounds__(256)
k_reduced_rows(const int64_t *__restrict__ rowptr, const int *__restrict__ col, const int64_t *__restrict__ qidx,
               const double *__restrict__ kval, const double *__restrict__ s1, const double *__restrict__ s2,
               const double *__restrict__ xv, const double *__restrict__ q, const double *__restrict__ b, double tau,
               double *__restrict__ part, int n, int m) {
    const int gid = blockIdx.x * blockDim.x + threadIdx.x;
    const int row = gid >> 2, sub = gid & 3;
    double a1 = 0.0, a2 = 0.0, a3 = 0.0;
    if (row < n) {
        const int64_t p0 = rowptr[row], p1 = rowptr[row + 1];
        for (int64_t p = p0 + sub; p < p1; p += 4) {
            const int c = col[p];
            if (c < n) {
                const double v = kval[qidx[p]];
                a1 += v * s1[c];
                a2 += v * s2[c];
                a3 += v * (xv[c] / tau);
            }
        }
    }
    a1 += __shfl_xor(a1, 1, 64); a1 += __shfl_xor(a1, 2, 64);
    a2 += __shfl_xor(a2, 1, 64); a2 += __shfl_xor(a2, 2, 64);
    a3 += __shfl_xor(a3, 1, 64); a3 += __shfl_xor(a3, 2, 64);
    double d[8] = {0.0, 0.0, 0.0, 0.0, 0.0, 0.0, 0.0, 0.0};
    if (sub == 0 && row < n + m) {
        if (row < n) {
            const double xi = xv[row] / tau, x1 = s1[row], x2 = s2[row];
            d[0] = q[row] * x1;
            d[2] = xi * a1;
            d[3] = q[row] * x2;
            d[5] = (xi - x2) * (a3 - a2);
            d[6] = x2 * a2;
        } else {
            const int j = row - n;
            d[1] = b[j] * s1[row];
            d[4] = b[j] * s2[row];
        }
    }
    block_dots<7, 8>(d, part);
}
__global__ void __launch_bounds__(256)
k_reduced_finish(const double *__restrict__ part, int nblocks, double tau, double kappa, double rhs_tau, double rhs_kappa,
                 double *__restrict__ scal_out) {
    double t[8];
    column_sums<8>(part, nblocks, t);
    if (threadIdx.x == 0) {
        const double qx1 = t[0], bz1 = t[1], xPx1 = t[2], qx2 = t[3], bz2 = t[4], dPd = t[5], x2Px2 = t[6];
        const double num = rhs_tau - rhs_kappa / tau + qx1 + bz1 + 2.0 * xPx1;
        double den = kappa / tau - qx2 - bz2;
        den += dPd - x2Px2;
        scal_out[0] = num / den; scal_out[1] = num; scal_out[2] = den;
        scal_out[3] = qx1; scal_out[4] = bz1; scal_out[5] = xPx1; scal_out[6] = qx2; scal_out[7] = bz2; scal_out[8] = dPd; scal_out[9] = x2Px2;
    }
}
__global__ void k_reduced_axpy(const double *__restrict__ s1, const double *__restrict__ s2, const double *__restrict__ scal,
                               double *__restrict__ lhs, int nm) {
    const int i = blockIdx.x * blockDim.x + threadIdx.x;
    if (i < nm) lhs[i] = s1[i] + scal[0] * s2[i];
}
__global__ void k_const_rhs(double *__restrict__ dst, const double *__restrict__ qb, int n, int nm, int N) {
    const int i = blockIdx.x * blockDim.x + threadIdx.x;
    if (i < N) dst[i] = i < n ? -qb[i] : (i < nm ? qb[i] : 0.0);
}

__global__ void __launch_bounds__(256)
k_norm_inf(const double *__restrict__ v, int n, unsigned long long *__restrict__ slot) {
    double a = 0.0;
    for (int i = blockIdx.x * blockDim.x + threadIdx.x; i < n; i += gridDim.x * blockDim.x) {
        const double t = fabs(v[i]);
        a = (t > a || t != t) ? t : a;
    }
    block_atomic_max_abs(slot, a);
}

__global__ void k_refine_decide(RefineState *st, const unsigned long long *scal, int phase, double reltol, double abstol,
                                int max_iter, double stop_ratio) {
    if (blockIdx.x || threadIdx.x) return;
    const double norme = __longlong_as_double((long long)scal[SC_NORME]);
    if (phase == 0) {
        const double normb = __longlong_as_double((long long)scal[SC_NORMB]);
        st->cur = 0;
        st->steps = 0;
        st->normb = normb;
        st->norme = norme;
        st->lastnorme = norme;
        st->fail = isfinite(norme) ? 0 : 1;
        st->active = (!st->fail && max_iter > 0 && !(norme <= abstol + reltol * normb)) ? 1 : 0;
        return;
    }
    if (!st->active) return;
    st->steps += 1;
    st->norme = norme;
    if (!isfinite(norme)) { st->fail = 1; st->active = 0; return; }
    const double improved = st->lastnorme / norme;
    if (improved < stop_ratio) {
        if (improved > 1.0) st->cur ^= 1;
        st->active = 0;
        return;
    }
    st->cur ^= 1;
    st->lastnorme = norme;
    st->active = (st->steps < max_iter && !(norme <= abstol + reltol * st->normb)) ? 1 : 0;
}
__global__ void k_refine_add(const RefineState *st, double *__restrict__ x0, double *__restrict__ x1,
                             const double *__restrict__ corr, int n) {
    if (!st->active) return;
    const int i = blockIdx.x * blockDim.x + threadIdx.x;
    const double *src = st->cur ? x1 : x0;
    double *dst = st->cur ? x0 : x1;
    if (i < n) dst[i] = src[i] + corr[i];
}
__global__ void k_refine_copy_out(const RefineState *st, const double *__restrict__ x0, const double *__restrict__ x1,
                                  double *__restrict__ out, int nm) {
    const int i = blockIdx.x * blockDim.x + threadIdx.x;
    const double *src = st->cur ? x1 : x0;
    if (i < nm) out[i] = src[i];
}

__global__ void k_set_rhs(double *__restrict__ b, const double *__restrict__ rhs, int nm, int n) {
    int i = blockIdx.x * blockDim.x + threadIdx.x;
    if (i < n) b[i] = i < nm ? rhs[i] : 0.0;
}

__global__ void k_check_finite(const double *__restrict__ v, int n, int *__restrict__ flags) {
    int i = blockIdx.x * blockDim.x + threadIdx.x;
    if (i < n && !isfinite(v[i])) atomicOr(flags + FL_NONFINITE, 1);
}

void launch_spmv_residual(hipStream_t st, const DevPlan &P, const double *b, const RefineState *rs, const double *x0, const double *x1,
                          double *e, int n, unsigned long long *slot) {
    const double *dacc = P.n_dtri_strips > 0 ? P.dense_acc : nullptr;
    if (dacc)
        hipLaunchKernelGGL(k_spmv_dense_tri, dim3(P.n_dtri_strips), dim3(512), 0, st, P.dtri_strips, P.dtri_col, P.kval, rs, x0, x1, P.dense_acc);
    if (n > 0)
        hipLaunchKernelGGL(k_spmv_residual, dim3(nblk((int64_t)n * 4)), dim3(256), 0, st, P.sym_rowptr, P.sym_col, P.sym_q,
                           P.kval, b, rs, x0, x1, e, n, slot, dacc);
    if (P.n_long_rows > 0)
        hipLaunchKernelGGL(k_spmv_long, dim3(P.n_long_rows), dim3(256), 0, st, P.long_rows, P.sym_rowptr, P.sym_col, P.sym_q, P.kval,
                           b, rs, x0, x1, e, slot, dacc);
}
void launch_block_products(hipStream_t st, const DevPlan &P, const double *x, const double *z, double *Px, double *ATz,
                           double *Ax, int n, int m) {
    if (n + m > 0)
        hipLaunchKernelGGL(k_block_products, dim3(nblk((int64_t)(n + m) * 4)), dim3(256), 0, st, P.sym_rowptr, P.sym_col, P.sym_q,
                           P.kval, x, z, Px, ATz, Ax, n, m);
}
void launch_refine_decide(hipStream_t st, RefineState *rs, const double *scal, int phase, double reltol, double abstol, int max_iter,
                          double stop_ratio) {
    hipLaunchKernelGGL(k_refine_decide, dim3(1), dim3(64), 0, st, rs, (const unsigned long long *)scal, phase, reltol, abstol, max_iter,
                       stop_ratio);
}
void launch_refine_add(hipStream_t st, const RefineState *rs, double *x0, double *x1, const double *corr, int n) {
    if (n > 0) hipLaunchKernelGGL(k_refine_add, dim3(nblk(n)), dim3(256), 0, st, rs, x0, x1, corr, n);
}
void launch_refine_copy_out(hipStream_t st, const RefineState *rs, const double *x0, const double *x1, double *out, int nm) {
    if (nm > 0) hipLaunchKernelGGL(k_refine_copy_out, dim3(nblk(nm)), dim3(256), 0, st, rs, x0, x1, out, nm);
}
int long_row_threshold() { return kLongRow; }
int residual_blocks(int n, int m) { return (int)nblk((int64_t)(n + m) * 4); }
void launch_residuals(hipStream_t st, const DevPlan &P, const double *x, const double *z, const double *s, const double *q,
                      const double *b, double tau, double kappa, double *out, double *part, double *scal, int n, int m) {
    if (n + m <= 0) return;
    const int nb = residual_blocks(n, m);
    hipLaunchKernelGGL(k_residuals, dim3(nb), dim3(256), 0, st, P.sym_rowptr, P.sym_col, P.sym_q, P.kval, x, z, s, q, b, tau, out, part, n, m);
    hipLaunchKernelGGL(k_residuals_finish, dim3(1), dim3(256), 0, st, part, nb, tau, kappa, scal);
}
void launch_reduced(hipStream_t st, const DevPlan &P, const double *s1, const double *s2, const double *xv, const double *q,
                    const double *b, double tau, double kappa, double rhs_tau, double rhs_kappa, double *part, double *scal_out,
                    double *lhs, int n, int m) {
    if (n + m <= 0) return;
    const int nb = residual_blocks(n, m);
    hipLaunchKernelGGL(k_reduced_rows, dim3(nb), dim3(256), 0, st, P.sym_rowptr, P.sym_col, P.sym_q, P.kval, s1, s2, xv, q, b, tau, part, n, m);
    hipLaunchKernelGGL(k_reduced_finish, dim3(1), dim3(256), 0, st, part, nb, tau, kappa, rhs_tau, rhs_kappa, scal_out);
    hipLaunchKernelGGL(k_reduced_axpy, dim3(nblk(n + m)), dim3(256), 0, st, s1, s2, scal_out, lhs, n + m);
}
void launch_const_rhs(hipStream_t st, double *dst, const double *qb, int n, int nm, int N) {
    if (N > 0) hipLaunchKernelGGL(k_const_rhs, dim3(nblk(N)), dim3(256), 0, st, dst, qb, n, nm, N);
}
void launch_norm_inf(hipStream_t st, const double *v, int n, unsigned long long *slot) {
    if (n > 0) hipLaunchKernelGGL(k_norm_inf, dim3(min(nblk(n), 64u)), dim3(256), 0, st, v, n, slot);
}
void launch_set_rhs(hipStream_t st, double *b, const double *rhs, int nm, int n) {
    if (n > 0) hipLaunchKernelGGL(k_set_rhs, dim3(nblk(n)), dim3(256), 0, st, b, rhs, nm, n);
}
void launch_check_finite(hipStream_t st, const double *v, int n, int *flags) {
    if (n > 0) hipLaunchKernelGGL(k_check_finite, dim3(nblk(n)), dim3(256), 0, st, v, n, flags);
}

}
```

### clarabel.jl_amd/csrc/solve_sweep.hip

```cpp
#include <hip/hip_runtime.h>
#include <stdint.h>

#include "device_plan.h"
#include "kernel_util.h"
#include "kernels.h"
#include "sweep_common.h"

namespace hipkkt {

__global__ void __launch_bounds__(256)
k_permute_in(const double *__restrict__ b, const int *__restrict__ perm, double *__restrict__ y, int n, int *epoch,
             int *ticks, int nticks, int *zero, int nzero) {
    if (blockIdx.x == 0 && threadIdx.x == 0 && epoch) ((unsigned *)epoch)[0] += 1u;
    if (blockIdx.x == 0) {
        for (int q = threadIdx.x; q < nticks; q += blockDim.x) ticks[q] = 0;
        for (int q = threadIdx.x; q < nzero; q += blockDim.x) zero[q] = 0;
    }
    int k = blockIdx.x * blockDim.x + threadIdx.x;
    if (k < n) y[k] = b[perm[k]];
}

__device__ __forceinline__ void polish_fwd(const DevPlan &P, int s, int w, const double *rhs, double *yv, double *scratch) {
    const double *ldg = P.Ldiag + P.sn_diag[s], *li = P.Linv + P.sn_diag[s];
    const int tid = threadIdx.x;
    if (tid < w) {
        double a = rhs[tid] - yv[tid];
        for (int k2 = 0; k2 < tid; k2++) a -= ldg[tid + k2 * w] * yv[k2];
        scratch[tid] = a;
    }
    __syncthreads();
    double c = 0.0;
    if (tid < w)
        for (int k2 = 0; k2 <= tid; k2++) c += li[tid + k2 * w] * scratch[k2];
    __syncthreads();
    if (tid < w) yv[tid] += c;
    __syncthreads();
}
__device__ __forceinline__ void polish_bwd(const DevPlan &P, int s, int w, const double *tv, double *xv, double *scratch) {
    const double *ldg = P.Ldiag + P.sn_diag[s], *lit = P.LinvT + P.sn_diag[s];
    const int tid = threadIdx.x;
    if (tid < w) {
        double a = tv[tid] - xv[tid];
        for (int i2 = tid + 1; i2 < w; i2++) a -= ldg[i2 + tid * w] * xv[i2];
        scratch[tid] = a;
    }
    __syncthreads();
    double c = 0.0;
    if (tid < w)
        for (int i2 = tid; i2 < w; i2++) c += lit[tid + i2 * w] * scratch[i2];
    __syncthreads();
    if (tid < w) xv[tid] += c;
    __syncthreads();
}


__global__ void __launch_bounds__(256)
k_fwd_level(DevPlan P, int item_begin, double *__restrict__ y, double *__restrict__ z) {
    __shared__ double rhs[kMaxSnWidth];
    __shared__ double part[4][kMaxSnWidth];
    __shared__ double yv[kMaxSnWidth];
    const FacItem it = P.slv_items[item_begin + blockIdx.x];
    const int s = it.sn;
    const int f = P.sn_first[s];
    const int w = P.sn_first[s + 1] - f;
    const int64_t slot0 = P.sn_rowptr[s];
    const int r = (int)(P.sn_rowptr[s + 1] - slot0);
    const double *pan = P.Lx + P.sn_panel[s];
    const double *li = P.Linv + P.sn_diag[s];
    const int tid = threadIdx.x;
    const int i = tid & 63, pq = tid >> 6;
    if (tid < w) {
        double acc = 0.0;
        const int64_t g0 = P.g_ptr[slot0 + tid], g1 = P.g_ptr[slot0 + tid + 1];
        for (int64_t g = g0; g < g1; g++) acc += P.ubuf[P.g_idx[g]];
        rhs[tid] = y[f + tid] - acc;
    }
    const int row = w + it.blk * kSlvRows + i;
    double pv[16];
    double gsum = 0.0;
    if (row < r) {
        const double *pr = pan + row;
#pragma unroll
        for (int t = 0; t < 16; t++) {
            const int k = pq + 4 * t;
            pv[t] = k < w ? pr[(int64_t)k * r] : 0.0;
        }
        if (pq == 0) {
            const int64_t g0 = P.g_ptr[slot0 + row], g1 = P.g_ptr[slot0 + row + 1];
            for (int64_t g = g0; g < g1; g++) gsum += P.ubuf[P.g_idx[g]];
        }
    }
    __syncthreads();
    {
        double a0 = 0.0, a1 = 0.0;
        if (i < w) {
            int k = pq;
            for (; k + 4 <= i; k += 8) {
                a0 += li[i + k * w] * rhs[k];
                a1 += li[i + (k + 4) * w] * rhs[k + 4];
            }
            if (k <= i) a0 += li[i + k * w] * rhs[k];
        }
        part[pq][i] = a0 + a1;
    }
    __syncthreads();
    if (tid < w) {
        yv[tid] = ((part[0][tid] + part[1][tid]) + part[2][tid]) + part[3][tid];
    } else if (tid < kMaxSnWidth) {
        yv[tid] = 0.0;
    }
    __syncthreads();
    if (P.sn_polish[s]) polish_fwd(P, s, w, rhs, yv, part[0]);
    if (tid < w && it.blk == 0) z[f + tid] = yv[tid] * P.Dinv[f + tid];
    {
        double a0 = 0.0, a1 = 0.0, a2 = 0.0, a3 = 0.0;
        if (row < r) {
#pragma unroll
            for (int t = 0; t < 16; t += 4) {
                a0 += pv[t] * yv[(pq + 4 * t) & 63];
                a1 += pv[t + 1] * yv[(pq + 4 * t + 4) & 63];
                a2 += pv[t + 2] * yv[(pq + 4 * t + 8) & 63];
                a3 += pv[t + 3] * yv[(pq + 4 * t + 12) & 63];
            }
        }
        __syncthreads();
        part[pq][i] = (a0 + a1) + (a2 + a3);
    }
    __syncthreads();
    if (pq == 0 && row < r)
        P.ubuf[P.u_off[s] + (row - w)] = gsum + (((part[0][i] + part[1][i]) + part[2][i]) + part[3][i]);
}

__device__ __forceinline__ double bwd_block_dot(const DevPlan &P, int s, int w, int r, int blk,
                                                const double *__restrict__ x, double (*red)[kMaxSnWidth]) {
    const int tid = threadIdx.x, lane = tid & 63, wave = tid >> 6;
    const int *rows = P.sn_rows + P.sn_rowptr[s];
    const double *lt = P.LT + P.lt_off[s];
    const int lo = w + blk * kSlvRows + wave * 16;
    const int hi = min(min(r, lo + 16), w + (blk + 1) * kSlvRows);
    double a0 = 0.0, a1 = 0.0, a2 = 0.0, a3 = 0.0;
    if (lane < w) {
        int i = lo;
        for (; i + 4 <= hi; i += 4) {
            a0 += lt[(int64_t)(i - w) * w + lane] * x[rows[i]];
            a1 += lt[(int64_t)(i + 1 - w) * w + lane] * x[rows[i + 1]];
            a2 += lt[(int64_t)(i + 2 - w) * w + lane] * x[rows[i + 2]];
            a3 += lt[(int64_t)(i + 3 - w) * w + lane] * x[rows[i + 3]];
        }
        for (; i < hi; i++) a0 += lt[(int64_t)(i - w) * w + lane] * x[rows[i]];
    }
    red[wave][lane] = (a0 + a1) + (a2 + a3);
    __syncthreads();
    return ((red[0][lane] + red[1][lane]) + red[2][lane]) + red[3][lane];
}

template <int NW>
__global__ void __launch_bounds__(256)
k_fwd_narrow(DevPlan P, int sn_begin, int n, double *__restrict__ y, double *__restrict__ z) {
    const int t = blockIdx.x * blockDim.x + threadIdx.x;
    if (t >= n) return;
    const int s = P.lvl_sn[sn_begin + t];
    const int f = P.sn_first[s];
    const int w = P.sn_first[s + 1] - f;
    const int64_t slot0 = P.sn_rowptr[s];
    const int r = (int)(P.sn_rowptr[s + 1] - slot0);
    const double *pan = P.Lx + P.sn_panel[s];
    const double *li = P.Linv + P.sn_diag[s];
    double rhs[NW], yv[NW];
#pragma unroll
    for (int k = 0; k < NW; k++) {
        rhs[k] = 0.0;
        if (k < w) {
            double acc = 0.0;
            for (int64_t g = P.g_ptr[slot0 + k]; g < P.g_ptr[slot0 + k + 1]; g++) acc += P.ubuf[P.g_idx[g]];
            rhs[k] = y[f + k] - acc;
        }
    }
#pragma unroll
    for (int i = 0; i < NW; i++) {
        double v = 0.0;
#pragma unroll
        for (int k = 0; k <= i; k++)
            if (i < w) v += li[i + k * w] * rhs[k];
        yv[i] = v;
        if (i < w) z[f + i] = v * P.Dinv[f + i];
    }
    double *u = P.ubuf + P.u_off[s];
    for (int row = w; row < r; row++) {
        double a = 0.0;
        for (int64_t g = P.g_ptr[slot0 + row]; g < P.g_ptr[slot0 + row + 1]; g++) a += P.ubuf[P.g_idx[g]];
#pragma unroll
        for (int k = 0; k < NW; k++)
            if (k < w) a += pan[row + (int64_t)k * r] * yv[k];
        u[row - w] = a;
    }
}

template <int NW>
__global__ void __launch_bounds__(256)
k_bwd_narrow(DevPlan P, int sn_begin, int n, const double *__restrict__ z, double *__restrict__ x, double *__restrict__ xout) {
    const int t = blockIdx.x * blockDim.x + threadIdx.x;
    if (t >= n) return;
    const int s = P.lvl_sn[sn_begin + t];
    const int f = P.sn_first[s];
    const int w = P.sn_first[s + 1] - f;
    const int64_t slot0 = P.sn_rowptr[s];
    const int r = (int)(P.sn_rowptr[s + 1] - slot0);
    const int *rows = P.sn_rows + slot0;
    const double *lt = P.LT + P.lt_off[s];
    const double *lit = P.LinvT + P.sn_diag[s];
    double tv[NW];
#pragma unroll
    for (int k = 0; k < NW; k++) tv[k] = k < w ? z[f + k] : 0.0;
    for (int i = w; i < r; i++) {
        const double xi = x[rows[i]];
#pragma unroll
        for (int k = 0; k < NW; k++)
            if (k < w) tv[k] -= lt[(int64_t)(i - w) * w + k] * xi;
    }
#pragma unroll
    for (int k = 0; k < NW; k++) {
        double v = 0.0;
#pragma unroll
        for (int i = k; i < NW; i++)
            if (i < w) v += lit[k + i * w] * tv[i];
        if (k < w) {
            x[f + k] = v;
            xout[P.perm[f + k]] = v;
        }
    }
}

__global__ void __launch_bounds__(256)
k_bwd_partial(DevPlan P, int item_begin, const double *__restrict__ x) {
    __shared__ double red[4][kMaxSnWidth];
    const FacItem it = P.bwd_items[item_begin + blockIdx.x];
    const int s = it.sn;
    const int w = P.sn_first[s + 1] - P.sn_first[s];
    const int r = (int)(P.sn_rowptr[s + 1] - P.sn_rowptr[s]);
    const double v = bwd_block_dot(P, s, w, r, it.blk, x, red);
    if (threadIdx.x < w) P.pbuf[P.p_off[s] + (int64_t)it.blk * w + threadIdx.x] = v;
}

__global__ void __launch_bounds__(256)
k_bwd_final(DevPlan P, int sn_begin, const double *__restrict__ z, double *__restrict__ x,
            double *__restrict__ xout) {
    __shared__ double red[4][kMaxSnWidth];
    __shared__ double tv[kMaxSnWidth];
    const int s = P.lvl_sn[sn_begin + blockIdx.x];
    const int f = P.sn_first[s];
    const int w = P.sn_first[s + 1] - f;
    const int r = (int)(P.sn_rowptr[s + 1] - P.sn_rowptr[s]);
    const double *lit = P.LinvT + P.sn_diag[s];
    const int tid = threadIdx.x;
    const int k = tid & 63, pq = tid >> 6;
    const int nblk = (r - w + kSlvRows - 1) / kSlvRows;
    double acc = 0.0;
    if (nblk == 1) {
        acc = bwd_block_dot(P, s, w, r, 0, x, red);
        __syncthreads();
    } else if (nblk > 1) {
        double a = 0.0;
        if (k < w) {
            const double *pb = P.pbuf + P.p_off[s] + k;
            for (int b = pq; b < nblk; b += 4) a += pb[(int64_t)b * w];
        }
        red[pq][k] = a;
        __syncthreads();
        acc = ((red[0][k] + red[1][k]) + red[2][k]) + red[3][k];
        __syncthreads();
    }
    if (tid < w) tv[tid] = z[f + tid] - acc;
    __syncthreads();
    {
        double a0 = 0.0, a1 = 0.0;
        if (k < w) {
            int i = k + pq;
            for (; i + 4 < w; i += 8) {
                a0 += lit[k + i * w] * tv[i];
                a1 += lit[k + (i + 4) * w] * tv[i + 4];
            }
            if (i < w) a0 += lit[k + i * w] * tv[i];
        }
        red[pq][k] = a0 + a1;
    }
    __syncthreads();
    if (P.sn_polish[s]) {
        __shared__ double xv[kMaxSnWidth];
        if (tid < w) xv[tid] = ((red[0][tid] + red[1][tid]) + red[2][tid]) + red[3][tid];
        __syncthreads();
        polish_bwd(P, s, w, tv, xv, red[0]);
        if (tid < w) {
            x[f + tid] = xv[tid];
            xout[P.perm[f + tid]] = xv[tid];
        }
        return;
    }
    if (tid < w) {
        const double v = ((red[0][tid] + red[1][tid]) + red[2][tid]) + red[3][tid];
        x[f + tid] = v;
        xout[P.perm[f + tid]] = v;
    }
}

struct SegSync {
    int *ftick, *btick, *fdone, *err;
};
__device__ __forceinline__ SegSync seg_sync(const DevPlan &P, int nsuper) {
    const SegSyncLayout L = seg_sync_layout(P.nseg, nsuper);
    return {P.seg_sync + L.ftick, P.seg_sync + L.btick, P.seg_sync + L.fdone, P.seg_sync + L.err};
}
__device__ __forceinline__ bool seg_wait_sum(int *ctr, int stride, int want, int *err, int *failflag, unsigned lim) {
    for (unsigned spins = 0;; spins++) {
        int v[kSegSub];
#pragma unroll
        for (int k = 0; k < kSegSub; k++) v[k] = front_ld_flag(ctr + (int64_t)k * stride);
        int sum = 0;
#pragma unroll
        for (int k = 0; k < kSegSub; k++) sum += v[k];
        if (sum >= want) return true;
        if (!spin_go_on(spins + 1u, spins, err, failflag, lim)) return false;
        __builtin_amdgcn_s_sleep(1);
    }
}
__device__ __forceinline__ bool seg_wait(int *ctr, int want, int *err, int *failflag, unsigned lim) {
    for (unsigned spins = 0;; spins++) {
        if (front_ld_flag(ctr) >= want) return true;
        if (!spin_go_on(spins + 1u, spins, err, failflag, lim)) return false;
        __builtin_amdgcn_s_sleep(1);
    }
}
__device__ __forceinline__ unsigned long long seg_key(const DevPlan &P) {
    return kSlotKey ^ ((unsigned long long)(((const unsigned *)P.seg_epoch)[0] + 1u) * 0x9E3779B97F4A7C15ull);
}
__device__ __forceinline__ void seg_slot_st(FrontSlot *p, double v, unsigned long long key) {
    typedef unsigned v4u __attribute__((ext_vector_type(4)));
    const unsigned long long b = (unsigned long long)__double_as_longlong(v), h = b ^ key;
    v4u r = {(unsigned)b, (unsigned)(b >> 32), (unsigned)h, (unsigned)(h >> 32)};
    asm volatile("global_store_dwordx4 %0, %1, off sc1\n\ts_nop 2" : : "v"(p), "v"(r) : "memory");
}

__global__ void __launch_bounds__(256)
k_fwd_seg(DevPlan P, int seg, int item_begin, int nitems, int nsuper, double *__restrict__ y, double *__restrict__ z) {
    __shared__ double rhs[kMaxSnWidth];
    __shared__ double part[4][kMaxSnWidth];
    __shared__ double yv[kMaxSnWidth];
    __shared__ int tick, sb;
    const SegSync Y = seg_sync(P, nsuper);
    const int tid = threadIdx.x;
    if (tid == 0) tick = atomicAdd(Y.ftick + seg, 1);
    __syncthreads();
    const int t = tick;
    if (t >= nitems) return;
    const FacItem it = P.slv_items[item_begin + t];
    const int s = it.sn;
    const int f = P.sn_first[s];
    const int w = P.sn_first[s + 1] - f;
    const int64_t slot0 = P.sn_rowptr[s];
    const int r = (int)(P.sn_rowptr[s + 1] - slot0);
    const double *pan = P.Lx + P.sn_panel[s];
    const double *li = P.Linv + P.sn_diag[s];
    const int i = tid & 63, pq = tid >> 6;
    const int row = w + it.blk * kSlvRows + i;
    double liv[16], pv[16];
#pragma unroll
    for (int t2 = 0; t2 < 16; t2++) {
        const int k = pq + 4 * t2;
        liv[t2] = (i < w && k <= i) ? li[i + k * w] : 0.0;
        pv[t2] = (row < r && k < w) ? pan[row + (int64_t)k * r] : 0.0;
    }
    constexpr int kSegGath = 12;
    int64_t ga0 = 0, ga1 = 0, gb0 = 0, gb1 = 0;
    int ia[kSegGath], ib[kSegGath];
#pragma unroll
    for (int q = 0; q < kSegGath; q++) { ia[q] = 0; ib[q] = 0; }
    double yin = 0.0, dinv_own = 0.0;
    if (tid < w) {
        dinv_own = P.Dinv[f + tid];
        ga0 = P.g_ptr[slot0 + tid];
        ga1 = P.g_ptr[slot0 + tid + 1];
#pragma unroll
        for (int q = 0; q < kSegGath; q++)
            if (ga0 + q < ga1) ia[q] = P.g_idx[ga0 + q];
        yin = y[f + tid];
    }
    if (pq == 0 && row < r) {
        gb0 = P.g_ptr[slot0 + row];
        gb1 = P.g_ptr[slot0 + row + 1];
#pragma unroll
        for (int q = 0; q < kSegGath; q++)
            if (gb0 + q < gb1) ib[q] = P.g_idx[gb0 + q];
    }
    const int want = P.dep_total[s], fpar = P.sn_bparent[s];
    const int fsub = (fpar >= 0 && P.dep_total[fpar] >= kSegSubMin) ? (it.blk & (kSegSub - 1)) : 0;
    if (tid == 0) {
        sb = (want == 0 || (want >= kSegSubMin ? seg_wait_sum(Y.fdone + s, nsuper, want, Y.err, P.flags + FL_FRONTFAIL, P.spin_limit)
                                               : seg_wait(Y.fdone + s, want, Y.err, P.flags + FL_FRONTFAIL, P.spin_limit))) ? 1 : 0;
        asm volatile("" ::: "memory");
    }
    __syncthreads();
    if (!sb) return;
    if (tid < w) {
        double u[kSegGath];
#pragma unroll
        for (int q = 0; q < kSegGath; q++) u[q] = ga0 + q < ga1 ? front_ld(P.ubuf + ia[q]) : 0.0;
        double acc = ((u[0] + u[1]) + u[2]) + u[3];
#pragma unroll
        for (int q = 4; q < kSegGath; q++)
            if (ga0 + q < ga1) acc += u[q];
        for (int64_t g = ga0 + kSegGath; g < ga1; g++) acc += front_ld(P.ubuf + P.g_idx[g]);
        rhs[tid] = yin - acc;
    } else if (tid < kMaxSnWidth) {
        rhs[tid] = 0.0;
    }
    double gsum = 0.0;
    if (pq == 0 && row < r) {
        double u[kSegGath];
#pragma unroll
        for (int q = 0; q < kSegGath; q++) u[q] = gb0 + q < gb1 ? front_ld(P.ubuf + ib[q]) : 0.0;
        gsum = ((u[0] + u[1]) + u[2]) + u[3];
#pragma unroll
        for (int q = 4; q < kSegGath; q++)
            if (gb0 + q < gb1) gsum += u[q];
        for (int64_t g = gb0 + kSegGath; g < gb1; g++) gsum += front_ld(P.ubuf + P.g_idx[g]);
    }
    __syncthreads();
    {
        double a0 = 0.0, a1 = 0.0;
#pragma unroll
        for (int t2 = 0; t2 < 16; t2 += 2) {
            a0 += liv[t2] * rhs[(pq + 4 * t2) & 63];
            a1 += liv[t2 + 1] * rhs[(pq + 4 * t2 + 4) & 63];
        }
        part[pq][i] = a0 + a1;
    }
    __syncthreads();
    if (tid < w) {
        yv[tid] = ((part[0][tid] + part[1][tid]) + part[2][tid]) + part[3][tid];
    } else if (tid < kMaxSnWidth) {
        yv[tid] = 0.0;
    }
    __syncthreads();
    if (P.sn_polish[s]) polish_fwd(P, s, w, rhs, yv, part[0]);
    if (tid < w && it.blk == 0) z[f + tid] = yv[tid] * dinv_own;
    {
        double a0 = 0.0, a1 = 0.0, a2 = 0.0, a3 = 0.0;
#pragma unroll
        for (int t2 = 0; t2 < 16; t2 += 4) {
            a0 += pv[t2] * yv[(pq + 4 * t2) & 63];
            a1 += pv[t2 + 1] * yv[(pq + 4 * t2 + 4) & 63];
            a2 += pv[t2 + 2] * yv[(pq + 4 * t2 + 8) & 63];
            a3 += pv[t2 + 3] * yv[(pq + 4 * t2 + 12) & 63];
        }
        __syncthreads();
        part[pq][i] = (a0 + a1) + (a2 + a3);
    }
    __syncthreads();
    if (pq == 0 && row < r)
        front_st(P.ubuf + P.u_off[s] + (row - w), gsum + (((part[0][i] + part[1][i]) + part[2][i]) + part[3][i]));
    if (pq == 0) asm volatile("s_waitcnt vmcnt(0)" ::: "memory");
    if (tid == 0 && fpar >= 0) atomicAdd(Y.fdone + (int64_t)fsub * nsuper + fpar, 1);
}

__global__ void __launch_bounds__(256)
k_bwd_seg(DevPlan P, int seg, int item_begin, int nitems, int nsuper, int first_launch, const double *__restrict__ z,
          double *__restrict__ x, double *__restrict__ xout) {
    __shared__ double red[4][kMaxSnWidth];
    __shared__ double tv[kMaxSnWidth];
    __shared__ int bad;
    const SegSync Y = seg_sync(P, nsuper);
    const int tid = threadIdx.x;
    __shared__ int tick;
    if (tid == 0) { bad = 0; tick = atomicAdd(Y.btick + seg, 1); }
    __syncthreads();
    const int t = tick;
    if (t >= nitems) return;
    if (first_launch) {
        for (int q = t * 256 + tid; q < kSegSub * nsuper; q += nitems * 256) Y.fdone[q] = 0;
    }
    const unsigned long long key = seg_key(P);
    const FacItem it = P.pbwd_items[item_begin + t];
    const int s = it.sn;
    const int f = P.sn_first[s];
    const int w = P.sn_first[s + 1] - f;
    const int r = (int)(P.sn_rowptr[s + 1] - P.sn_rowptr[s]);
    const int nblk = (r - w + kSlvRows - 1) / kSlvRows;
    const int lane = tid & 63, wave = tid >> 6;
    const int *rows = P.rows_seg + P.sn_rowptr[s];
    const double *lt = P.LT + P.lt_off[s];
    const bool dot_here = it.blk >= 0 || nblk == 1;
    const int blk = it.blk >= 0 ? it.blk : 0;
    const int lo = w + blk * kSlvRows + wave * 16;
    double lv[16], xv[16];
    int ri[16];
#pragma unroll
    for (int t2 = 0; t2 < 16; t2++) {
        const int i = lo + t2;
        const bool in = dot_here && i < r && i < w + (blk + 1) * kSlvRows;
        ri[t2] = in ? rows[i] : -1;
        lv[t2] = (in && lane < w) ? lt[(int64_t)(i - w) * w + lane] : 0.0;
        xv[t2] = (ri[t2] >= 0 && !(ri[t2] & kSegRowTag)) ? x[ri[t2]] : 0.0;
    }
    int ri_lane = -1;
    {
        const int i = lo + (lane & 15);
        if (dot_here && i < r && i < w + (blk + 1) * kSlvRows) ri_lane = rows[i];
    }
    double litv[16];
    double zin = 0.0;
    int perm_own = 0;
    if (it.blk < 0) {
        if (tid < w) perm_own = P.perm[f + tid];
        const double *lit = P.LinvT + P.sn_diag[s];
#pragma unroll
        for (int t2 = 0; t2 < 16; t2++) {
            const int i2 = wave + 4 * t2;
            litv[t2] = (lane < w && i2 >= lane && i2 < w) ? lit[lane + i2 * w] : 0.0;
        }
        if (tid < w) zin = z[f + tid];
    } else {
#pragma unroll
        for (int t2 = 0; t2 < 16; t2++) litv[t2] = 0.0;
    }
    bool ok = true;
    double dotv = 0.0;
    if (dot_here) {
        double a0 = 0.0, a1 = 0.0, a2 = 0.0, a3 = 0.0;
        {
            const int rl = ri_lane;
            const bool mine = lane < 16 && rl >= 0 && (rl & kSegRowTag);
            double myv = 0.0;
            bool got = !mine;
            unsigned spins = 0;
            while (ok) {
                if (!got) {
                    const FrontSlot sl = front_slot_ld(P.xseg + (rl & ~kSegRowTag));
                    if (((unsigned long long)__double_as_longlong(sl.v) ^ sl.h) == key) { myv = sl.v; got = true; }
                }
                if (__ballot(!got) == 0ull) break;
                ++spins;
                ok = spin_go_on(spins, spins, Y.err, P.flags + FL_FRONTFAIL, P.spin_limit);
            }
#pragma unroll
            for (int t2 = 0; t2 < 16; t2++) {
                const double bv = readlane_f64(myv, t2);
                if (ri[t2] >= 0 && (ri[t2] & kSegRowTag)) xv[t2] = bv;
            }
        }
        if (!ok) { bad = 1; atomicOr(P.flags + FL_FRONTFAIL, 4); }
#pragma unroll
        for (int t2 = 0; t2 < 16; t2 += 4) {
            a0 = fma(lv[t2], xv[t2], a0);
            a1 = fma(lv[t2 + 1], xv[t2 + 1], a1);
            a2 = fma(lv[t2 + 2], xv[t2 + 2], a2);
            a3 = fma(lv[t2 + 3], xv[t2 + 3], a3);
        }
        red[wave][lane] = (a0 + a1) + (a2 + a3);
        __syncthreads();
        if (bad) return;
        dotv = ((red[0][lane] + red[1][lane]) + red[2][lane]) + red[3][lane];
        __syncthreads();
    }
    if (it.blk >= 0) {
        if (tid < w) seg_slot_st(P.pseg + P.p_off[s] + (int64_t)it.blk * w + tid, dotv, key);
        return;
    }
    double acc = dotv;
    if (nblk > 1) {
        double a = 0.0;
        if (lane < w) {
            constexpr int kSegPoll = 8;
            const FrontSlot *pb = P.pseg + P.p_off[s] + lane;
            for (int b0 = wave; b0 < nblk && ok; b0 += 4 * kSegPoll) {
                double v[kSegPoll];
                bool got[kSegPoll];
#pragma unroll
                for (int u = 0; u < kSegPoll; u++) { v[u] = 0.0; got[u] = b0 + 4 * u >= nblk; }
                unsigned spins = 0;
                while (true) {
                    bool all = true;
#pragma unroll
                    for (int u = 0; u < kSegPoll; u++) {
                        if (!got[u]) {
                            const FrontSlot sl = front_slot_ld(pb + (int64_t)(b0 + 4 * u) * w);
                            if (((unsigned long long)__double_as_longlong(sl.v) ^ sl.h) == key) { v[u] = sl.v; got[u] = true; }
                            else all = false;
                        }
                    }
                    if (all) break;
                    ++spins;
                    ok = spin_go_on(spins, spins, Y.err, P.flags + FL_FRONTFAIL, P.spin_limit);
                    if (!ok) break;
                }
#pragma unroll
                for (int u = 0; u < kSegPoll; u++)
                    if (b0 + 4 * u < nblk) a += v[u];
            }
        }
        if (!ok) { bad = 1; atomicOr(P.flags + FL_FRONTFAIL, 4); }
        red[wave][lane] = a;
        __syncthreads();
        if (bad) return;
        acc = ((red[0][lane] + red[1][lane]) + red[2][lane]) + red[3][lane];
        __syncthreads();
    }
    if (tid < kMaxSnWidth) tv[tid] = tid < w ? zin - acc : 0.0;
    __syncthreads();
    {
        double s0 = 0.0, s1 = 0.0;
#pragma unroll
        for (int t2 = 0; t2 < 16; t2 += 2) {
            s0 = fma(litv[t2], tv[(wave + 4 * t2) & 63], s0);
            s1 = fma(litv[t2 + 1], tv[(wave + 4 * t2 + 4) & 63], s1);
        }
        red[wave][lane] = s0 + s1;
    }
    __syncthreads();
    if (P.sn_polish[s]) {
        __shared__ double xv[kMaxSnWidth];
        if (tid < w) xv[tid] = ((red[0][tid] + red[1][tid]) + red[2][tid]) + red[3][tid];
        __syncthreads();
        polish_bwd(P, s, w, tv, xv, red[0]);
        if (tid < w) {
            seg_slot_st(P.xseg + f + tid, xv[tid], key);
            x[f + tid] = xv[tid];
            xout[perm_own] = xv[tid];
        }
        return;
    }
    if (tid < w) {
        const double v = ((red[0][tid] + red[1][tid]) + red[2][tid]) + red[3][tid];
        seg_slot_st(P.xseg + f + tid, v, key);
        x[f + tid] = v;
        xout[perm_own] = v;
    }
}

void launch_fwd_narrow(hipStream_t st, const DevPlan &P, int sn_begin, int n, int wmax, double *y, double *z) {
    if (n <= 0) return;
    if (wmax <= 4) hipLaunchKernelGGL(k_fwd_narrow<4>, dim3(nblk(n)), dim3(256), 0, st, P, sn_begin, n, y, z);
    else hipLaunchKernelGGL(k_fwd_narrow<kNarrowW>, dim3(nblk(n)), dim3(256), 0, st, P, sn_begin, n, y, z);
}
void launch_bwd_narrow(hipStream_t st, const DevPlan &P, int sn_begin, int n, int wmax, const double *z, double *x, double *xout) {
    if (n <= 0) return;
    if (wmax <= 4) hipLaunchKernelGGL(k_bwd_narrow<4>, dim3(nblk(n)), dim3(256), 0, st, P, sn_begin, n, z, x, xout);
    else hipLaunchKernelGGL(k_bwd_narrow<kNarrowW>, dim3(nblk(n)), dim3(256), 0, st, P, sn_begin, n, z, x, xout);
}
void launch_permute_in(hipStream_t st, const double *b, const int *perm, double *y, int n, int *epoch, int *ticks, int nticks, int *zero, int nzero) {
    if (n > 0) hipLaunchKernelGGL(k_permute_in, dim3(nblk(n)), dim3(256), 0, st, b, perm, y, n, epoch, ticks, nticks, zero, nzero);
}
void launch_fwd_level(hipStream_t st, const DevPlan &P, int item_begin, int nitems, double *y, double *z) {
    if (nitems > 0) hipLaunchKernelGGL(k_fwd_level, dim3(nitems), dim3(256), 0, st, P, item_begin, y, z);
}
void launch_bwd_partial(hipStream_t st, const DevPlan &P, int item_begin, int nitems, const double *x) {
    if (nitems > 0) hipLaunchKernelGGL(k_bwd_partial, dim3(nitems), dim3(256), 0, st, P, item_begin, x);
}
void launch_bwd_final(hipStream_t st, const DevPlan &P, int sn_begin, int nsn, const double *z, double *x, double *xout) {
    if (nsn > 0) hipLaunchKernelGGL(k_bwd_final, dim3(nsn), dim3(256), 0, st, P, sn_begin, z, x, xout);
}
void launch_fwd_seg(hipStream_t st, const DevPlan &P, int seg, int item_begin, int nitems, int nsuper, double *y, double *z) {
    if (nitems > 0) hipLaunchKernelGGL(k_fwd_seg, dim3(nitems), dim3(256), 0, st, P, seg, item_begin, nitems, nsuper, y, z);
}
void launch_bwd_seg(hipStream_t st, const DevPlan &P, int seg, int item_begin, int nitems, int nsuper, int first, const double *z,
                    double *x, double *xout) {
    if (nitems > 0) hipLaunchKernelGGL(k_bwd_seg, dim3(nitems), dim3(256), 0, st, P, seg, item_begin, nitems, nsuper, first, z, x, xout);
}

}
```

Baseline: 212.0 IPM-iterations/s (KKT iteration units: 1 update + 1 factor + 3 refined solves [constant-rhs + affine concurrently, then combined], inputs in HBM).

## Fuse solve-level kernels, permute-in, norm and refine-decide into fewer launches

Merges the narrow and wide forward-level kernels into one launch and does the same for the backward narrow and final kernels. The input permutation and arming step are folded into the first forward level, and the norm-inf, refine-add and refine-decide kernels are folded into the SpMV residual kernel through a last-block-done pattern. Refine state and flags are packed into one struct so a single device-to-host copy reads both. The aim is to cut kernel launch count and graph node overhead in the latency-bound triangular solves, at the cost of larger, more divergent kernels and an extra atomic counter.

```diff
diff --git a/clarabel.jl_amd/csrc/device_plan.h b/clarabel.jl_amd/csrc/device_plan.h
--- a/clarabel.jl_amd/csrc/device_plan.h
+++ b/clarabel.jl_amd/csrc/device_plan.h
@@ -5,7 +5,7 @@
 
 namespace hipkkt {
 
-enum { SC_MAXDIAG = 0, SC_NORMB = 1, SC_NORME = 2, SC_COUNT = 8 };
+enum { SC_MAXDIAG = 0, SC_NORME = 2, SC_COUNT = 8, SC_NORMB = 16, SC_RCOUNT = 32, SC_ALLOC = 48 };
 enum { FL_NONFINITE = 0, FL_NREG = 1, FL_FRONTFAIL = 2, FL_FACFAIL = 3, FL_NPOLISH = 4, FL_COUNT = 8 };
 
 struct __attribute__((aligned(16))) FrontSlot {
@@ -19,6 +19,23 @@
     int32_t active;
     int32_t fail;
     double lastnorme, normb, norme;
+};
+struct SolveStatus {
+    int32_t flags[FL_COUNT];
+    RefineState rs;
+};
+struct SolveArm {
+    int *epoch, *ticks;
+    int nticks;
+    int *zero_norme, *zero_count;
+    unsigned long long *normb;
+};
+struct RefineDecide {
+    RefineState *st;
+    unsigned long long *scal;
+    unsigned *count;
+    int phase, max_iter;
+    double reltol, abstol, stop_ratio;
 };
 
 struct GathPair {
diff --git a/clarabel.jl_amd/csrc/hipkkt_internal.h b/clarabel.jl_amd/csrc/hipkkt_internal.h
--- a/clarabel.jl_amd/csrc/hipkkt_internal.h
+++ b/clarabel.jl_amd/csrc/hipkkt_internal.h
@@ -225,7 +225,6 @@
             if (C.own_stream && C.stream) (void)hipStreamSynchronize(C.stream);
         for_each_graph_slot([](hipkkt_host::GraphSlot &g) { if (g.exec) (void)hipGraphExecDestroy(g.exec); });
         for (SolveCtx &C : ctx) {
-            rp.pinned_free(device, C.h_rs);
             rp.pinned_free(device, C.h_flags);
             for (hipEvent_t e : {C.ev_a, C.ev_b}) rp.event_put(device, e);
             if (C.own_stream) rp.stream_put(device, 2, C.stream);
diff --git a/clarabel.jl_amd/csrc/hipkkt_setup.cpp b/clarabel.jl_amd/csrc/hipkkt_setup.cpp
--- a/clarabel.jl_amd/csrc/hipkkt_setup.cpp
+++ b/clarabel.jl_amd/csrc/hipkkt_setup.cpp
@@ -64,7 +64,7 @@
         S->accurate_threshold = o.accurate;
         S->twin.force = o.force_twin;
     }
-    static_assert(SC_COUNT * sizeof(double) <= RuntimePool::kPinned && sizeof(RefineState) <= RuntimePool::kPinned, "pinned chunk too small");
+    static_assert(SC_COUNT * sizeof(double) <= RuntimePool::kPinned && sizeof(SolveStatus) <= RuntimePool::kPinned, "pinned chunk too small");
     for (hipEvent_t *e : {&S->ev0, &S->ev1, &S->ev2, &S->ev3, &S->ev_fork, &S->ev_join}) *e = (hipEvent_t)need(rp.event_get(S->device));
     S->h_scal = (double *)need(rp.pinned_alloc(S->device));
     S->h_flags = (int *)need(rp.pinned_alloc(S->device));
@@ -79,10 +79,10 @@
         else { C.stream = (hipStream_t)need(rp.stream_get(S->device, 2)); C.own_stream = true; }
         C.ev_a = (hipEvent_t)need(rp.event_get(S->device));
         C.ev_b = (hipEvent_t)need(rp.event_get(S->device));
-        C.h_rs = (RefineState *)need(rp.pinned_alloc(S->device));
-        C.h_flags = (int *)need(rp.pinned_alloc(S->device));
-        memset(C.h_rs, 0, sizeof(RefineState));
-        memset(C.h_flags, 0, FL_COUNT * sizeof(int));
+        SolveStatus *hs = (SolveStatus *)need(rp.pinned_alloc(S->device));
+        memset(hs, 0, sizeof(SolveStatus));
+        C.h_flags = hs->flags;
+        C.h_rs = &hs->rs;
     }
 }
 
@@ -422,8 +422,8 @@
     D.seg_epoch = zeroed<int>(S, 4);
     D.seg_sync = zeroed<int>(S, nw.seg);
     D.front_sync = zeroed<int>(S, nw.front);
-    D.scal = zeroed<double>(S, SC_COUNT);
-    D.flags = zeroed<int>(S, FL_COUNT);
+    D.scal = zeroed<double>(S, SC_ALLOC);
+    D.flags = zeroed<SolveStatus>(S, 1)->flags;
 }
 
 static void alloc_factor_storage(hipkkt_solver *S) {
@@ -486,10 +486,10 @@
     for (int c = 0; c < kNumCtx; c++) {
         SolveCtx &C = S->ctx[c];
         for (double **v : {&C.d_b, &C.d_x0, &C.d_x1, &C.d_e, &C.d_corr, &C.d_y, &C.d_z, &C.d_xp}) *v = zeroed<double>(S, (size_t)N);
-        C.d_rs = (RefineState *)zeroed<double>(S, sizeof(RefineState) / sizeof(double) + 1);
         C.dp = S->dp;
         if (S->dp.n_dtri_strips > 0) C.dp.dense_acc = zeroed<double>(S, (size_t)N);
         if (c > 0) alloc_solve_scratch(S, C.dp);
+        C.d_rs = &((SolveStatus *)C.dp.flags)->rs;
         C.ir_used = false;
         C.h_rs->cur = 0;
     }
diff --git a/clarabel.jl_amd/csrc/hipkkt_solve.cpp b/clarabel.jl_amd/csrc/hipkkt_solve.cpp
--- a/clarabel.jl_amd/csrc/hipkkt_solve.cpp
+++ b/clarabel.jl_amd/csrc/hipkkt_solve.cpp
@@ -5,25 +5,35 @@
 
 namespace hipkkt_host {
 
-static void enqueue_ldl_solve(hipkkt_solver *S, SolveCtx &C, const double *in, double *out, int *zero = nullptr, int nzero = 0) {
+enum class ArmFor { plain, first_residual, step_residual };
+
+static void enqueue_ldl_solve(hipkkt_solver *S, SolveCtx &C, const double *in, double *out, ArmFor arm_for = ArmFor::plain) {
     const HostPlan &P = S->plan;
     const SolveSchedule &H = S->sched;
     hipStream_t st = C.stream;
     const DevPlan &D = C.dp;
-    launch_permute_in(st, in, D.perm, C.d_y, S->N, D.seg_epoch, D.seg_sync, 2 * H.nseg, zero, nzero);
+    SolveArm arm{D.seg_epoch, D.seg_sync, 2 * H.nseg, nullptr, nullptr, nullptr};
+    if (arm_for != ArmFor::plain) {
+        arm.zero_norme = (int *)(D.scal + SC_NORME);
+        arm.zero_count = (int *)(D.scal + SC_RCOUNT);
+    }
+    if (arm_for == ArmFor::first_residual) arm.normb = (unsigned long long *)D.scal + SC_NORMB;
     const LevelLists &L = S->persist.use ? H.regular : H.all;
-    auto fwd_level = [&](int l) {
-        launch_fwd_narrow(st, D, L.reg_ptr[l], L.nnarrow[l], L.wnarrow[l], C.d_y, C.d_z);
-        launch_fwd_level(st, D, L.slv_ptr[l], L.slv_ptr[l + 1] - L.slv_ptr[l], C.d_y, C.d_z);
+    auto fwd_blocks = [&](int l) { return fwd_bottom_blocks(L.nnarrow[l], L.slv_ptr[l + 1] - L.slv_ptr[l]); };
+    auto fwd_level = [&](int l, bool first) {
+        launch_fwd_bottom(st, D, L.reg_ptr[l], L.nnarrow[l], L.wnarrow[l], L.slv_ptr[l], L.slv_ptr[l + 1] - L.slv_ptr[l], first ? &arm : nullptr,
+                          in, S->N, C.d_y, C.d_z);
     };
     auto bwd_level = [&](int l) {
         launch_bwd_partial(st, D, L.bwd_ptr[l], L.bwd_ptr[l + 1] - L.bwd_ptr[l], C.d_xp);
-        launch_bwd_final(st, D, L.reg_ptr[l] + L.nnarrow[l], L.reg_ptr[l + 1] - L.reg_ptr[l] - L.nnarrow[l], C.d_z, C.d_xp, out);
-        launch_bwd_narrow(st, D, L.reg_ptr[l], L.nnarrow[l], L.wnarrow[l], C.d_z, C.d_xp, out);
+        launch_bwd_bottom(st, D, L.reg_ptr[l], L.nnarrow[l], L.wnarrow[l], L.reg_ptr[l + 1] - L.reg_ptr[l] - L.nnarrow[l], C.d_z, C.d_xp, out);
     };
+    const int l0 = S->persist.use ? H.seg_lo[0] : 0;
+    const bool level_first = l0 < (S->persist.use ? std::min(H.seg_lstar[0], H.seg_hi[0] + 1) : P.nlevels) && fwd_blocks(l0) > 0;
+    if (!level_first) launch_permute_in(st, arm, in, D.perm, C.d_y, S->N);
     if (S->persist.use) {
         for (int g = 0; g < H.nseg; g++) {
-            for (int l = H.seg_lo[g]; l < std::min(H.seg_lstar[g], H.seg_hi[g] + 1); l++) fwd_level(l);
+            for (int l = H.seg_lo[g]; l < std::min(H.seg_lstar[g], H.seg_hi[g] + 1); l++) fwd_level(l, level_first && l == l0);
             launch_fwd_seg(st, D, g, H.fseg_ptr[2 * g], H.fseg_ptr[2 * g + 1] - H.fseg_ptr[2 * g], P.nsuper, C.d_y, C.d_z);
             for (const FrontDesc &F : P.fronts)
                 if (H.seg_of_level[F.level_last] == g) launch_front_fwd(st, D, F, C.d_y, C.d_z);
@@ -39,7 +49,7 @@
         }
         return;
     }
-    for (int l = 0; l < P.nlevels; l++) fwd_level(l);
+    for (int l = 0; l < P.nlevels; l++) fwd_level(l, level_first && l == l0);
     for (int l = P.nlevels - 1; l >= 0; l--) bwd_level(l);
 }
 
@@ -54,12 +64,13 @@
     }
 }
 
+static RefineDecide decide_args(SolveCtx &C, int phase, const RefineOpts &ir) {
+    return {C.d_rs, (unsigned long long *)C.dp.scal, nullptr, phase, (int)std::min<int64_t>(ir.max_iter, 1 << 30), ir.reltol, ir.abstol, ir.stop_ratio};
+}
+
 static void enqueue_refine_step(hipkkt_solver *S, SolveCtx &C, const RefineOpts &ir) {
-    hipStream_t st = C.stream;
-    enqueue_ldl_solve(S, C, C.d_e, C.d_corr, (int *)(C.dp.scal + SC_NORME), 2);
-    launch_refine_add(st, C.d_rs, C.d_x0, C.d_x1, C.d_corr, S->N);
-    launch_spmv_residual(st, C.dp, C.d_b, C.d_rs, C.d_x0, C.d_x1, C.d_e, S->N, (unsigned long long *)C.dp.scal + SC_NORME);
-    launch_refine_decide(st, C.d_rs, C.dp.scal, 1, ir.reltol, ir.abstol, (int)std::min<int64_t>(ir.max_iter, 1 << 30), ir.stop_ratio);
+    enqueue_ldl_solve(S, C, C.d_e, C.d_corr, ArmFor::step_residual);
+    launch_spmv_residual(C.stream, C.dp, C.d_b, C.d_x0, C.d_x1, C.d_corr, C.d_e, S->N, decide_args(C, 1, ir));
 }
 
 static inline bool sweep_failed(const SolveCtx &C) {
@@ -87,6 +98,7 @@
         fill_async(S->stream, C.dp.seg_sync, 0, nw.seg * sizeof(int));
         fill_async(S->stream, C.dp.front_sync, 0, nw.front * sizeof(int));
         fill_async(S->stream, C.dp.flags + FL_FRONTFAIL, 0, sizeof(int));
+        fill_async(S->stream, C.dp.scal + SC_NORMB, 0, sizeof(double));
         C.h_flags[FL_FRONTFAIL] = 0;
         invalidate_solve_graphs(C);
     }
@@ -126,10 +138,8 @@
     if (ir.enable) {
         const bool same = C.g_opts.same_graph(ir);
         run_graphed(S, st, C.g_first, same, [&] {
-            enqueue_ldl_solve(S, C, C.d_b, C.d_x0, (int *)(C.dp.scal + SC_NORMB), 4);
-            launch_norm_inf(st, C.d_b, S->N, (unsigned long long *)C.dp.scal + SC_NORMB);
-            launch_spmv_residual(st, C.dp, C.d_b, nullptr, C.d_x0, C.d_x0, C.d_e, S->N, (unsigned long long *)C.dp.scal + SC_NORME);
-            launch_refine_decide(st, C.d_rs, C.dp.scal, 0, ir.reltol, ir.abstol, (int)std::min<int64_t>(ir.max_iter, 1 << 30), ir.stop_ratio);
+            enqueue_ldl_solve(S, C, C.d_b, C.d_x0, ArmFor::first_residual);
+            launch_spmv_residual(st, C.dp, C.d_b, C.d_x0, C.d_x0, nullptr, C.d_e, S->N, decide_args(C, 0, ir));
             if (ir.max_iter > 0) enqueue_refine_step(S, C, ir);
         });
         if (!same) { C.g_step.valid = false; C.g_opts = ir; }
@@ -153,8 +163,7 @@
 static int32_t solve_finish(hipkkt_solver *S, SolveCtx &C, int64_t *ir_steps, double *out_dev, int nm) {
     hipStream_t st = C.stream;
     auto readback = [&] {
-        if (C.ir_used) HK_CHECK(hipMemcpyAsync(C.h_rs, C.d_rs, sizeof(RefineState), hipMemcpyDeviceToHost, st));
-        HK_CHECK(hipMemcpyAsync(C.h_flags, C.dp.flags, FL_COUNT * sizeof(int), hipMemcpyDeviceToHost, st));
+        HK_CHECK(hipMemcpyAsync(C.h_flags, C.dp.flags, C.ir_used ? sizeof(SolveStatus) : FL_COUNT * sizeof(int), hipMemcpyDeviceToHost, st));
         HK_CHECK(hipEventRecord(C.ev_b, st));
         HK_CHECK(hipStreamSynchronize(st));
     };
diff --git a/clarabel.jl_amd/csrc/kernel_util.h b/clarabel.jl_amd/csrc/kernel_util.h
--- a/clarabel.jl_amd/csrc/kernel_util.h
+++ b/clarabel.jl_amd/csrc/kernel_util.h
@@ -68,17 +68,22 @@
     return v;
 }
 
-__device__ __forceinline__ void block_atomic_max_abs(unsigned long long *slot, double a) {
+__device__ __forceinline__ double block_max_abs(double a) {
     __shared__ double wm_[16];
     a = wave_max(a);
     const int lane = threadIdx.x & 63, wave = threadIdx.x >> 6, nw = (blockDim.x + 63) >> 6;
     if (lane == 0) wm_[wave] = a;
     __syncthreads();
+    double m = 0.0;
     if (threadIdx.x == 0) {
-        double m = wm_[0];
+        m = wm_[0];
         for (int i = 1; i < nw; i++) m = (wm_[i] > m || wm_[i] != wm_[i]) ? wm_[i] : m;
-        atomic_max_abs(slot, m);
     }
+    return m;
+}
+__device__ __forceinline__ void block_atomic_max_abs(unsigned long long *slot, double a) {
+    const double m = block_max_abs(a);
+    if (threadIdx.x == 0) atomic_max_abs(slot, m);
 }
 
 }
diff --git a/clarabel.jl_amd/csrc/kernels.h b/clarabel.jl_amd/csrc/kernels.h
--- a/clarabel.jl_amd/csrc/kernels.h
+++ b/clarabel.jl_amd/csrc/kernels.h
@@ -22,26 +22,21 @@
 void launch_split_reduce(hipStream_t st, const DevPlan &P, const SplitRec *recs, int n);
 void launch_update_gather(hipStream_t st, const DevPlan &P, int64_t ebegin, int64_t n, int64_t hbegin, int64_t nheavy, int max_blocks = 0);
 void launch_invert_diag(hipStream_t st, const DevPlan &P, int n_small, int wmax_small, int n_wide);
-void launch_permute_in(hipStream_t st, const double *b, const int *perm, double *y, int n, int *epoch, int *ticks, int nticks, int *zero = nullptr,
-                       int nzero = 0);
-void launch_fwd_level(hipStream_t st, const DevPlan &P, int item_begin, int nitems, double *y, double *z);
+void launch_permute_in(hipStream_t st, const SolveArm &arm, const double *b, const int *perm, double *y, int n);
+int fwd_bottom_blocks(int n_narrow, int nitems);
+void launch_fwd_bottom(hipStream_t st, const DevPlan &P, int sn_begin, int n_narrow, int wmax, int item_begin, int nitems, const SolveArm *arm,
+                       const double *b, int n, double *y, double *z);
 void launch_bwd_partial(hipStream_t st, const DevPlan &P, int item_begin, int nitems, const double *x);
-void launch_bwd_final(hipStream_t st, const DevPlan &P, int sn_begin, int nsn, const double *z, double *x, double *xout);
-void launch_fwd_narrow(hipStream_t st, const DevPlan &P, int sn_begin, int n, int wmax, double *y, double *z);
-void launch_bwd_narrow(hipStream_t st, const DevPlan &P, int sn_begin, int n, int wmax, const double *z, double *x, double *xout);
+void launch_bwd_bottom(hipStream_t st, const DevPlan &P, int sn_begin, int n_narrow, int wmax, int nsn, const double *z, double *x, double *xout);
 void launch_fwd_seg(hipStream_t st, const DevPlan &P, int seg, int item_begin, int nitems, int nsuper, double *y, double *z);
 void launch_bwd_seg(hipStream_t st, const DevPlan &P, int seg, int item_begin, int nitems, int nsuper, int first, const double *z,
                     double *x, double *xout);
 void launch_front_fwd(hipStream_t st, const DevPlan &P, const FrontDesc &F, double *y, double *z);
 void launch_front_bwd(hipStream_t st, const DevPlan &P, const FrontDesc &F, const double *z, double *x, double *xout);
 void launch_invert_super(hipStream_t st, const DevPlan &P, const FrontDesc &F);
-void launch_spmv_residual(hipStream_t st, const DevPlan &P, const double *b, const RefineState *rs, const double *x0, const double *x1,
-                          double *e, int n, unsigned long long *slot);
+void launch_spmv_residual(hipStream_t st, const DevPlan &P, const double *b, double *x0, double *x1, const double *corr, double *e, int n,
+                          const RefineDecide &d);
 int long_row_threshold();
-void launch_norm_inf(hipStream_t st, const double *v, int n, unsigned long long *slot);
-void launch_refine_decide(hipStream_t st, RefineState *rs, const double *scal, int phase, double reltol, double abstol, int max_iter,
-                          double stop_ratio);
-void launch_refine_add(hipStream_t st, const RefineState *rs, double *x0, double *x1, const double *corr, int n);
 void launch_refine_copy_out(hipStream_t st, const RefineState *rs, const double *x0, const double *x1, double *out, int nm);
 void launch_set_rhs(hipStream_t st, double *b, const double *rhs, int nm, int n);
 void launch_check_finite(hipStream_t st, const double *v, int n, int *flags);
diff --git a/clarabel.jl_amd/csrc/refine.hip b/clarabel.jl_amd/csrc/refine.hip
--- a/clarabel.jl_amd/csrc/refine.hip
+++ b/clarabel.jl_amd/csrc/refine.hip
@@ -8,9 +8,58 @@
 namespace hipkkt {
 
 constexpr int kLongRow = 192;
+template <bool STEP>
+struct SpmvOperand {
+    const double *src, *corr;
+    double *dst;
+    __device__ __forceinline__ SpmvOperand(const RefineState *st, double *x0, double *x1, const double *corr_)
+        : src(STEP && st->cur ? x1 : x0), corr(corr_), dst(STEP ? (st->cur ? x0 : x1) : nullptr) {}
+    __device__ __forceinline__ double operator[](int c) const { return STEP ? src[c] + corr[c] : src[c]; }
+};
+
+__device__ __forceinline__ void refine_decide(RefineState *st, double normb, double norme, int phase, double reltol, double abstol,
+                                              int max_iter, double stop_ratio) {
+    if (phase == 0) {
+        st->cur = 0;
+        st->steps = 0;
+        st->normb = normb;
+        st->norme = norme;
+        st->lastnorme = norme;
+        st->fail = isfinite(norme) ? 0 : 1;
+        st->active = (!st->fail && max_iter > 0 && !(norme <= abstol + reltol * normb)) ? 1 : 0;
+        return;
+    }
+    if (!st->active) return;
+    st->steps += 1;
+    st->norme = norme;
+    if (!isfinite(norme)) { st->fail = 1; st->active = 0; return; }
+    const double improved = st->lastnorme / norme;
+    if (improved < stop_ratio) {
+        if (improved > 1.0) st->cur ^= 1;
+        st->active = 0;
+        return;
+    }
+    st->cur ^= 1;
+    st->lastnorme = norme;
+    st->active = (st->steps < max_iter && !(norme <= abstol + reltol * st->normb)) ? 1 : 0;
+}
+__device__ __forceinline__ void refine_decide_last(const RefineDecide &d) {
+    if (!d.count) return;
+    if (atomicAdd(d.count, 1u) != gridDim.x - 1u) return;
+    const double norme = __longlong_as_double((long long)__hip_atomic_load(d.scal + SC_NORME, __ATOMIC_RELAXED, __HIP_MEMORY_SCOPE_AGENT));
+    const double normb = d.phase == 0 ? __longlong_as_double((long long)atomicExch(d.scal + SC_NORMB, 0ull)) : 0.0;
+    refine_decide(d.st, normb, norme, d.phase, d.reltol, d.abstol, d.max_iter, d.stop_ratio);
+    atomicExch(d.count, 0u);
+}
+
+__device__ __forceinline__ void max_abs_done(unsigned long long *slot, double v) {
+    const unsigned long long old = atomicMax(slot, (unsigned long long)__double_as_longlong(fabs(v)));
+    asm volatile("s_waitcnt vmcnt(0)" : : "v"(old) : "memory");
+}
+template <bool STEP>
 __device__ __forceinline__ void spmv_short_rows(const int64_t *__restrict__ rowptr, const int *__restrict__ col,
                                                 const int64_t *__restrict__ qidx, const double *__restrict__ kval,
-                                                const double *__restrict__ b, const double *__restrict__ xi, double *__restrict__ e,
+                                                const double *__restrict__ b, const SpmvOperand<STEP> xi, double *__restrict__ e,
                                                 int n, unsigned long long *__restrict__ norm_slot, const double *__restrict__ dacc) {
     const int gid = blockIdx.x * blockDim.x + threadIdx.x;
     const int row = gid >> 2, sub = gid & 3;
@@ -30,12 +79,15 @@
         const double ev = b[row] - acc;
         e[row] = ev;
         a = fabs(ev);
-    }
-    block_atomic_max_abs(norm_slot, a);
-}
+        if (STEP) xi.dst[row] = xi[row];
+    }
+    a = block_max_abs(a);
+    if (threadIdx.x == 0) max_abs_done(norm_slot, a);
+}
+template <bool STEP>
 __device__ __forceinline__ void spmv_long_row(int row, const int64_t *__restrict__ rowptr, const int *__restrict__ col,
                                               const int64_t *__restrict__ qidx, const double *__restrict__ kval,
-                                              const double *__restrict__ b, const double *__restrict__ xi, double *__restrict__ e,
+                                              const double *__restrict__ b, const SpmvOperand<STEP> xi, double *__restrict__ e,
                                               unsigned long long *__restrict__ norm_slot, const double *__restrict__ dacc) {
     __shared__ double red[4];
     const int64_t p0 = rowptr[row], p1 = rowptr[row + 1];
@@ -47,46 +99,47 @@
     if (threadIdx.x == 0) {
         const double ev = b[row] - ((((red[0] + red[1]) + red[2]) + red[3]) + (dacc ? dacc[row] : 0.0));
         e[row] = ev;
-        atomic_max_abs(norm_slot, ev);
-    }
-}
-__device__ __forceinline__ const double *spmv_operand(const RefineState *st, const double *x0, const double *x1) {
-    return st ? (st->cur ? x0 : x1) : x0;
-}
+        if (STEP) xi.dst[row] = xi[row];
+        max_abs_done(norm_slot, ev);
+    }
+}
+template <bool STEP>
 __global__ void __launch_bounds__(256)
 k_spmv_residual(const int64_t *__restrict__ rowptr, const int *__restrict__ col, const int64_t *__restrict__ qidx,
-                const double *__restrict__ kval, const double *__restrict__ b, const RefineState *st,
-                const double *__restrict__ x0, const double *__restrict__ x1, double *__restrict__ e, int n,
-                unsigned long long *__restrict__ norm_slot, const double *__restrict__ dacc) {
-    if (st && !st->active) return;
-    spmv_short_rows(rowptr, col, qidx, kval, b, spmv_operand(st, x0, x1), e, n, norm_slot, dacc);
-}
+                const double *__restrict__ kval, const double *__restrict__ b, double *x0, double *x1, const double *__restrict__ corr,
+                double *__restrict__ e, int n, unsigned long long *__restrict__ norm_slot, const double *__restrict__ dacc, RefineDecide d) {
+    if (STEP && !d.st->active) return;
+    spmv_short_rows<STEP>(rowptr, col, qidx, kval, b, SpmvOperand<STEP>(d.st, x0, x1, corr), e, n, norm_slot, dacc);
+    if (threadIdx.x == 0) refine_decide_last(d);
+}
+template <bool STEP>
 __global__ void __launch_bounds__(256)
 k_spmv_long(const int *__restrict__ long_rows, const int64_t *__restrict__ rowptr, const int *__restrict__ col,
-            const int64_t *__restrict__ qidx, const double *__restrict__ kval, const double *__restrict__ b,
-            const RefineState *st, const double *__restrict__ x0, const double *__restrict__ x1, double *__restrict__ e,
-            unsigned long long *__restrict__ norm_slot, const double *__restrict__ dacc) {
-    if (st && !st->active) return;
-    spmv_long_row(long_rows[blockIdx.x], rowptr, col, qidx, kval, b, spmv_operand(st, x0, x1), e, norm_slot, dacc);
-}
-
+            const int64_t *__restrict__ qidx, const double *__restrict__ kval, const double *__restrict__ b, double *x0, double *x1,
+            const double *__restrict__ corr, double *__restrict__ e, unsigned long long *__restrict__ norm_slot,
+            const double *__restrict__ dacc, RefineDecide d) {
+    if (STEP && !d.st->active) return;
+    spmv_long_row<STEP>(long_rows[blockIdx.x], rowptr, col, qidx, kval, b, SpmvOperand<STEP>(d.st, x0, x1, corr), e, norm_slot, dacc);
+    if (threadIdx.x == 0) refine_decide_last(d);
+}
+
+template <bool STEP>
 __global__ void __launch_bounds__(512)
 k_spmv_dense_tri(const DenseTriStrip *__restrict__ strips, const int64_t *__restrict__ col_off, const double *__restrict__ kval,
-                 const RefineState *st, const double *__restrict__ x0, const double *__restrict__ x1, double *__restrict__ acc_out) {
-    if (st && !st->active) return;
-    const double *__restrict__ x = spmv_operand(st, x0, x1);
+                 const RefineState *st, double *x0, double *x1, const double *__restrict__ corr, double *__restrict__ acc_out) {
+    if (STEP && !st->active) return;
+    const SpmvOperand<STEP> x(st, x0, x1, corr);
     __shared__ double part[8][64];
     __shared__ double csum[64];
     const DenseTriStrip T = strips[blockIdx.x];
     const int lane = threadIdx.x & 63, w = threadIdx.x >> 6;
     const int i = T.i0 + lane;
     const int64_t *__restrict__ co = col_off + T.col0;
-    const double *__restrict__ xb = x + T.c0;
     double a = 0.0;
 #pragma unroll 4
     for (int j = T.i0 + w; j < T.d; j += 8) {
         const double v = kval[co[j] + (i <= j ? i : j)];
-        a = fma(i <= j ? v : 0.0, xb[j], a);
+        a = fma(i <= j ? v : 0.0, x[T.c0 + j], a);
     }
     part[w][lane] = a;
     for (int c = 0; c < 8; c++) {
@@ -95,7 +148,7 @@
         if (ci < T.d) {
             const double *__restrict__ colv = kval + co[ci];
 #pragma unroll 4
-            for (int r = lane; r < ci; r += 64) s = fma(colv[r], xb[r], s);
+            for (int r = lane; r < ci; r += 64) s = fma(colv[r], x[T.c0 + r], s);
         }
         for (int off = 32; off > 0; off >>= 1) s += __shfl_xor(s, off, 64);
         if (lane == 0) csum[8 * w + c] = s;
@@ -280,53 +333,6 @@
     if (i < N) dst[i] = i < n ? -qb[i] : (i < nm ? qb[i] : 0.0);
 }
 
-__global__ void __launch_bounds__(256)
-k_norm_inf(const double *__restrict__ v, int n, unsigned long long *__restrict__ slot) {
-    double a = 0.0;
-    for (int i = blockIdx.x * blockDim.x + threadIdx.x; i < n; i += gridDim.x * blockDim.x) {
-        const double t = fabs(v[i]);
-        a = (t > a || t != t) ? t : a;
-    }
-    block_atomic_max_abs(slot, a);
-}
-
-__global__ void k_refine_decide(RefineState *st, const unsigned long long *scal, int phase, double reltol, double abstol,
-                                int max_iter, double stop_ratio) {
-    if (blockIdx.x || threadIdx.x) return;
-    const double norme = __longlong_as_double((long long)scal[SC_NORME]);
-    if (phase == 0) {
-        const double normb = __longlong_as_double((long long)scal[SC_NORMB]);
-        st->cur = 0;
-        st->steps = 0;
-        st->normb = normb;
-        st->norme = norme;
-        st->lastnorme = norme;
-        st->fail = isfinite(norme) ? 0 : 1;
-        st->active = (!st->fail && max_iter > 0 && !(norme <= abstol + reltol * normb)) ? 1 : 0;
-        return;
-    }
-    if (!st->active) return;
-    st->steps += 1;
-    st->norme = norme;
-    if (!isfinite(norme)) { st->fail = 1; st->active = 0; return; }
-    const double improved = st->lastnorme / norme;
-    if (improved < stop_ratio) {
-        if (improved > 1.0) st->cur ^= 1;
-        st->active = 0;
-        return;
-    }
-    st->cur ^= 1;
-    st->lastnorme = norme;
-    st->active = (st->steps < max_iter && !(norme <= abstol + reltol * st->normb)) ? 1 : 0;
-}
-__global__ void k_refine_add(const RefineState *st, double *__restrict__ x0, double *__restrict__ x1,
-                             const double *__restrict__ corr, int n) {
-    if (!st->active) return;
-    const int i = blockIdx.x * blockDim.x + threadIdx.x;
-    const double *src = st->cur ? x1 : x0;
-    double *dst = st->cur ? x0 : x1;
-    if (i < n) dst[i] = src[i] + corr[i];
-}
 __global__ void k_refine_copy_out(const RefineState *st, const double *__restrict__ x0, const double *__restrict__ x1,
                                   double *__restrict__ out, int nm) {
     const int i = blockIdx.x * blockDim.x + threadIdx.x;
@@ -344,31 +350,34 @@
     if (i < n && !isfinite(v[i])) atomicOr(flags + FL_NONFINITE, 1);
 }
 
-void launch_spmv_residual(hipStream_t st, const DevPlan &P, const double *b, const RefineState *rs, const double *x0, const double *x1,
-                          double *e, int n, unsigned long long *slot) {
+template <bool STEP>
+static void launch_spmv_residual_t(hipStream_t st, const DevPlan &P, const double *b, double *x0, double *x1, const double *corr, double *e,
+                                   int n, RefineDecide d) {
     const double *dacc = P.n_dtri_strips > 0 ? P.dense_acc : nullptr;
+    unsigned long long *slot = d.scal + SC_NORME;
+    unsigned *count = (unsigned *)(d.scal + SC_RCOUNT);
     if (dacc)
-        hipLaunchKernelGGL(k_spmv_dense_tri, dim3(P.n_dtri_strips), dim3(512), 0, st, P.dtri_strips, P.dtri_col, P.kval, rs, x0, x1, P.dense_acc);
-    if (n > 0)
-        hipLaunchKernelGGL(k_spmv_residual, dim3(nblk((int64_t)n * 4)), dim3(256), 0, st, P.sym_rowptr, P.sym_col, P.sym_q,
-                           P.kval, b, rs, x0, x1, e, n, slot, dacc);
+        hipLaunchKernelGGL(k_spmv_dense_tri<STEP>, dim3(P.n_dtri_strips), dim3(512), 0, st, P.dtri_strips, P.dtri_col, P.kval, d.st, x0, x1,
+                           corr, P.dense_acc);
+    d.count = P.n_long_rows > 0 ? nullptr : count;
+    hipLaunchKernelGGL(k_spmv_residual<STEP>, dim3(nblk((int64_t)n * 4)), dim3(256), 0, st, P.sym_rowptr, P.sym_col, P.sym_q, P.kval, b,
+                       x0, x1, corr, e, n, slot, dacc, d);
+    d.count = count;
     if (P.n_long_rows > 0)
-        hipLaunchKernelGGL(k_spmv_long, dim3(P.n_long_rows), dim3(256), 0, st, P.long_rows, P.sym_rowptr, P.sym_col, P.sym_q, P.kval,
-                           b, rs, x0, x1, e, slot, dacc);
+        hipLaunchKernelGGL(k_spmv_long<STEP>, dim3(P.n_long_rows), dim3(256), 0, st, P.long_rows, P.sym_rowptr, P.sym_col, P.sym_q, P.kval,
+                           b, x0, x1, corr, e, slot, dacc, d);
+}
+void launch_spmv_residual(hipStream_t st, const DevPlan &P, const double *b, double *x0, double *x1, const double *corr, double *e, int n,
+                          const RefineDecide &d) {
+    if (n <= 0) return;
+    if (d.phase == 0) launch_spmv_residual_t<false>(st, P, b, x0, x1, corr, e, n, d);
+    else launch_spmv_residual_t<true>(st, P, b, x0, x1, corr, e, n, d);
 }
 void launch_block_products(hipStream_t st, const DevPlan &P, const double *x, const double *z, double *Px, double *ATz,
                            double *Ax, int n, int m) {
     if (n + m > 0)
         hipLaunchKernelGGL(k_block_products, dim3(nblk((int64_t)(n + m) * 4)), dim3(256), 0, st, P.sym_rowptr, P.sym_col, P.sym_q,
                            P.kval, x, z, Px, ATz, Ax, n, m);
-}
-void launch_refine_decide(hipStream_t st, RefineState *rs, const double *scal, int phase, double reltol, double abstol, int max_iter,
-                          double stop_ratio) {
-    hipLaunchKernelGGL(k_refine_decide, dim3(1), dim3(64), 0, st, rs, (const unsigned long long *)scal, phase, reltol, abstol, max_iter,
-                       stop_ratio);
-}
-void launch_refine_add(hipStream_t st, const RefineState *rs, double *x0, double *x1, const double *corr, int n) {
-    if (n > 0) hipLaunchKernelGGL(k_refine_add, dim3(nblk(n)), dim3(256), 0, st, rs, x0, x1, corr, n);
 }
 void launch_refine_copy_out(hipStream_t st, const RefineState *rs, const double *x0, const double *x1, double *out, int nm) {
     if (nm > 0) hipLaunchKernelGGL(k_refine_copy_out, dim3(nblk(nm)), dim3(256), 0, st, rs, x0, x1, out, nm);
@@ -394,9 +403,6 @@
 void launch_const_rhs(hipStream_t st, double *dst, const double *qb, int n, int nm, int N) {
     if (N > 0) hipLaunchKernelGGL(k_const_rhs, dim3(nblk(N)), dim3(256), 0, st, dst, qb, n, nm, N);
 }
-void launch_norm_inf(hipStream_t st, const double *v, int n, unsigned long long *slot) {
-    if (n > 0) hipLaunchKernelGGL(k_norm_inf, dim3(min(nblk(n), 64u)), dim3(256), 0, st, v, n, slot);
-}
 void launch_set_rhs(hipStream_t st, double *b, const double *rhs, int nm, int n) {
     if (n > 0) hipLaunchKernelGGL(k_set_rhs, dim3(nblk(n)), dim3(256), 0, st, b, rhs, nm, n);
 }
diff --git a/clarabel.jl_amd/csrc/solve_sweep.hip b/clarabel.jl_amd/csrc/solve_sweep.hip
--- a/clarabel.jl_amd/csrc/solve_sweep.hip
+++ b/clarabel.jl_amd/csrc/solve_sweep.hip
@@ -1,5 +1,7 @@
 #include <hip/hip_runtime.h>
 #include <stdint.h>
+
+#include <algorithm>
 
 #include "device_plan.h"
 #include "kernel_util.h"
@@ -8,16 +10,29 @@
 
 namespace hipkkt {
 
+__device__ __forceinline__ void solve_arm(const SolveArm &A, const double *__restrict__ b, const int *__restrict__ perm,
+                                          double *__restrict__ y, int n, int nb) {
+    if ((int)blockIdx.x >= nb) return;
+    if (blockIdx.x == 0 && threadIdx.x == 0 && A.epoch) ((unsigned *)A.epoch)[0] += 1u;
+    if (blockIdx.x == 0) {
+        for (int q = threadIdx.x; q < A.nticks; q += blockDim.x) A.ticks[q] = 0;
+        if (threadIdx.x < 2) {
+            if (A.zero_norme) A.zero_norme[threadIdx.x] = 0;
+            if (A.zero_count) A.zero_count[threadIdx.x] = 0;
+        }
+    }
+    double a = 0.0;
+    for (int k = blockIdx.x * blockDim.x + threadIdx.x; k < n; k += nb * blockDim.x) {
+        const double v = b[perm[k]];
+        y[k] = v;
+        const double t = fabs(v);
+        a = (t > a || t != t) ? t : a;
+    }
+    if (A.normb) block_atomic_max_abs(A.normb, a);
+}
 __global__ void __launch_bounds__(256)
-k_permute_in(const double *__restrict__ b, const int *__restrict__ perm, double *__restrict__ y, int n, int *epoch,
-             int *ticks, int nticks, int *zero, int nzero) {
-    if (blockIdx.x == 0 && threadIdx.x == 0 && epoch) ((unsigned *)epoch)[0] += 1u;
-    if (blockIdx.x == 0) {
-        for (int q = threadIdx.x; q < nticks; q += blockDim.x) ticks[q] = 0;
-        for (int q = threadIdx.x; q < nzero; q += blockDim.x) zero[q] = 0;
-    }
-    int k = blockIdx.x * blockDim.x + threadIdx.x;
-    if (k < n) y[k] = b[perm[k]];
+k_permute_in(SolveArm A, const double *__restrict__ b, const int *__restrict__ perm, double *__restrict__ y, int n) {
+    solve_arm(A, b, perm, y, n, gridDim.x);
 }
 
 __device__ __forceinline__ void polish_fwd(const DevPlan &P, int s, int w, const double *rhs, double *yv, double *scratch) {
@@ -54,12 +69,13 @@
 }
 
 
-__global__ void __launch_bounds__(256)
-k_fwd_level(DevPlan P, int item_begin, double *__restrict__ y, double *__restrict__ z) {
+template <bool PERM>
+__device__ __forceinline__ void fwd_level(const DevPlan &P, int item, const double *__restrict__ y, const int *__restrict__ perm,
+                                          double *__restrict__ z) {
     __shared__ double rhs[kMaxSnWidth];
     __shared__ double part[4][kMaxSnWidth];
     __shared__ double yv[kMaxSnWidth];
-    const FacItem it = P.slv_items[item_begin + blockIdx.x];
+    const FacItem it = P.slv_items[item];
     const int s = it.sn;
     const int f = P.sn_first[s];
     const int w = P.sn_first[s + 1] - f;
@@ -73,7 +89,7 @@
         double acc = 0.0;
         const int64_t g0 = P.g_ptr[slot0 + tid], g1 = P.g_ptr[slot0 + tid + 1];
         for (int64_t g = g0; g < g1; g++) acc += P.ubuf[P.g_idx[g]];
-        rhs[tid] = y[f + tid] - acc;
+        rhs[tid] = y[PERM ? perm[f + tid] : f + tid] - acc;
     }
     const int row = w + it.blk * kSlvRows + i;
     double pv[16];
@@ -154,9 +170,9 @@
     return ((red[0][lane] + red[1][lane]) + red[2][lane]) + red[3][lane];
 }
 
-template <int NW>
-__global__ void __launch_bounds__(256)
-k_fwd_narrow(DevPlan P, int sn_begin, int n, double *__restrict__ y, double *__restrict__ z) {
+template <int NW, bool PERM>
+__device__ __forceinline__ void fwd_narrow(const DevPlan &P, int sn_begin, int n, const double *__restrict__ y,
+                                           const int *__restrict__ perm, double *__restrict__ z) {
     const int t = blockIdx.x * blockDim.x + threadIdx.x;
     if (t >= n) return;
     const int s = P.lvl_sn[sn_begin + t];
@@ -173,7 +189,7 @@
         if (k < w) {
             double acc = 0.0;
             for (int64_t g = P.g_ptr[slot0 + k]; g < P.g_ptr[slot0 + k + 1]; g++) acc += P.ubuf[P.g_idx[g]];
-            rhs[k] = y[f + k] - acc;
+            rhs[k] = y[PERM ? perm[f + k] : f + k] - acc;
         }
     }
 #pragma unroll
@@ -197,8 +213,8 @@
 }
 
 template <int NW>
-__global__ void __launch_bounds__(256)
-k_bwd_narrow(DevPlan P, int sn_begin, int n, const double *__restrict__ z, double *__restrict__ x, double *__restrict__ xout) {
+__device__ __forceinline__ void bwd_narrow(const DevPlan &P, int sn_begin, int n, const double *__restrict__ z, double *__restrict__ x,
+                                           double *__restrict__ xout) {
     const int t = blockIdx.x * blockDim.x + threadIdx.x;
     if (t >= n) return;
     const int s = P.lvl_sn[sn_begin + t];
@@ -242,12 +258,10 @@
     if (threadIdx.x < w) P.pbuf[P.p_off[s] + (int64_t)it.blk * w + threadIdx.x] = v;
 }
 
-__global__ void __launch_bounds__(256)
-k_bwd_final(DevPlan P, int sn_begin, const double *__restrict__ z, double *__restrict__ x,
-            double *__restrict__ xout) {
+__device__ __forceinline__ void bwd_final(const DevPlan &P, int s, const double *__restrict__ z, double *__restrict__ x,
+                                          double *__restrict__ xout) {
     __shared__ double red[4][kMaxSnWidth];
     __shared__ double tv[kMaxSnWidth];
-    const int s = P.lvl_sn[sn_begin + blockIdx.x];
     const int f = P.sn_first[s];
     const int w = P.sn_first[s + 1] - f;
     const int r = (int)(P.sn_rowptr[s + 1] - P.sn_rowptr[s]);
@@ -301,6 +315,22 @@
         x[f + tid] = v;
         xout[P.perm[f + tid]] = v;
     }
+}
+
+template <int NW, bool PERM>
+__global__ void __launch_bounds__(256)
+k_fwd_bottom(DevPlan P, int sn_begin, int n_narrow, int nb_narrow, int item_begin, SolveArm A, int nb_arm, const double *__restrict__ b,
+             int n, double *__restrict__ y, double *__restrict__ z) {
+    if (PERM) solve_arm(A, b, P.perm, y, n, nb_arm);
+    if ((int)blockIdx.x < nb_narrow) fwd_narrow<NW, PERM>(P, sn_begin, n_narrow, PERM ? b : y, P.perm, z);
+    else fwd_level<PERM>(P, item_begin + (int)blockIdx.x - nb_narrow, PERM ? b : y, P.perm, z);
+}
+template <int NW>
+__global__ void __launch_bounds__(256)
+k_bwd_bottom(DevPlan P, int sn_begin, int n_narrow, int nb_narrow, const double *__restrict__ z, double *__restrict__ x,
+             double *__restrict__ xout) {
+    if ((int)blockIdx.x < nb_narrow) bwd_narrow<NW>(P, sn_begin, n_narrow, z, x, xout);
+    else bwd_final(P, P.lvl_sn[sn_begin + n_narrow + (int)blockIdx.x - nb_narrow], z, x, xout);
 }
 
 struct SegSync {
@@ -636,27 +666,37 @@
     }
 }
 
-void launch_fwd_narrow(hipStream_t st, const DevPlan &P, int sn_begin, int n, int wmax, double *y, double *z) {
-    if (n <= 0) return;
-    if (wmax <= 4) hipLaunchKernelGGL(k_fwd_narrow<4>, dim3(nblk(n)), dim3(256), 0, st, P, sn_begin, n, y, z);
-    else hipLaunchKernelGGL(k_fwd_narrow<kNarrowW>, dim3(nblk(n)), dim3(256), 0, st, P, sn_begin, n, y, z);
-}
-void launch_bwd_narrow(hipStream_t st, const DevPlan &P, int sn_begin, int n, int wmax, const double *z, double *x, double *xout) {
-    if (n <= 0) return;
-    if (wmax <= 4) hipLaunchKernelGGL(k_bwd_narrow<4>, dim3(nblk(n)), dim3(256), 0, st, P, sn_begin, n, z, x, xout);
-    else hipLaunchKernelGGL(k_bwd_narrow<kNarrowW>, dim3(nblk(n)), dim3(256), 0, st, P, sn_begin, n, z, x, xout);
-}
-void launch_permute_in(hipStream_t st, const double *b, const int *perm, double *y, int n, int *epoch, int *ticks, int nticks, int *zero, int nzero) {
-    if (n > 0) hipLaunchKernelGGL(k_permute_in, dim3(nblk(n)), dim3(256), 0, st, b, perm, y, n, epoch, ticks, nticks, zero, nzero);
-}
-void launch_fwd_level(hipStream_t st, const DevPlan &P, int item_begin, int nitems, double *y, double *z) {
-    if (nitems > 0) hipLaunchKernelGGL(k_fwd_level, dim3(nitems), dim3(256), 0, st, P, item_begin, y, z);
+static inline int narrow_blocks(int n_narrow) { return (int)nblk(std::max(n_narrow, 0)); }
+int fwd_bottom_blocks(int n_narrow, int nitems) { return narrow_blocks(n_narrow) + std::max(nitems, 0); }
+constexpr int kArmBlocks = 128;
+template <int NW>
+static void launch_fwd_bottom_nw(hipStream_t st, const DevPlan &P, int sn_begin, int n_narrow, int item_begin, int nitems, const SolveArm *arm,
+                                 const double *b, int n, double *y, double *z) {
+    const int nbn = narrow_blocks(n_narrow), grid = nbn + nitems;
+    if (arm)
+        hipLaunchKernelGGL((k_fwd_bottom<NW, true>), dim3(grid), dim3(256), 0, st, P, sn_begin, n_narrow, nbn, item_begin, *arm,
+                           std::min(grid, kArmBlocks), b, n, y, z);
+    else
+        hipLaunchKernelGGL((k_fwd_bottom<NW, false>), dim3(grid), dim3(256), 0, st, P, sn_begin, n_narrow, nbn, item_begin, SolveArm{}, 0,
+                           (const double *)nullptr, n, y, z);
+}
+void launch_fwd_bottom(hipStream_t st, const DevPlan &P, int sn_begin, int n_narrow, int wmax, int item_begin, int nitems, const SolveArm *arm,
+                       const double *b, int n, double *y, double *z) {
+    if (fwd_bottom_blocks(n_narrow, nitems) <= 0) return;
+    if (wmax <= 4) launch_fwd_bottom_nw<4>(st, P, sn_begin, n_narrow, item_begin, nitems, arm, b, n, y, z);
+    else launch_fwd_bottom_nw<kNarrowW>(st, P, sn_begin, n_narrow, item_begin, nitems, arm, b, n, y, z);
+}
+void launch_bwd_bottom(hipStream_t st, const DevPlan &P, int sn_begin, int n_narrow, int wmax, int nsn, const double *z, double *x, double *xout) {
+    const int nbn = narrow_blocks(n_narrow), grid = nbn + std::max(nsn, 0);
+    if (grid <= 0) return;
+    if (wmax <= 4) hipLaunchKernelGGL(k_bwd_bottom<4>, dim3(grid), dim3(256), 0, st, P, sn_begin, n_narrow, nbn, z, x, xout);
+    else hipLaunchKernelGGL(k_bwd_bottom<kNarrowW>, dim3(grid), dim3(256), 0, st, P, sn_begin, n_narrow, nbn, z, x, xout);
+}
+void launch_permute_in(hipStream_t st, const SolveArm &arm, const double *b, const int *perm, double *y, int n) {
+    if (n > 0) hipLaunchKernelGGL(k_permute_in, dim3(nblk(n)), dim3(256), 0, st, arm, b, perm, y, n);
 }
 void launch_bwd_partial(hipStream_t st, const DevPlan &P, int item_begin, int nitems, const double *x) {
     if (nitems > 0) hipLaunchKernelGGL(k_bwd_partial, dim3(nitems), dim3(256), 0, st, P, item_begin, x);
-}
-void launch_bwd_final(hipStream_t st, const DevPlan &P, int sn_begin, int nsn, const double *z, double *x, double *xout) {
-    if (nsn > 0) hipLaunchKernelGGL(k_bwd_final, dim3(nsn), dim3(256), 0, st, P, sn_begin, z, x, xout);
 }
 void launch_fwd_seg(hipStream_t st, const DevPlan &P, int seg, int item_begin, int nitems, int nsuper, double *y, double *z) {
     if (nitems > 0) hipLaunchKernelGGL(k_fwd_seg, dim3(nitems), dim3(256), 0, st, P, seg, item_begin, nitems, nsuper, y, z);
```

After: 212.8 IPM-iterations/s (KKT iteration units: 1 update + 1 factor + 3 refined solves [constant-rhs + affine concurrently, then combined], inputs in HBM), median of 6. Within noise of the previous version (+0.4%).
